# jonnylaw/ComposableStateSpaceModels

Measured on AMD Instinct MI355X. Metric: particle-steps/sec (N x T) bootstrap filter, higher is better.
Workload: dtype f64

## Files before the change

composablestatespacemodels_amd/csrc/cssm_device.hip.h:

```cpp
#pragma once

#if !defined(__HIPCC_RTC__)
#include <hip/hip_runtime.h>
#include <stdint.h>
#endif

#include "cssm_records.h"

#define CSSM_BLOCK 256
#ifndef CSSM_PROP_IT_MID
#define CSSM_PROP_IT_MID 2
#endif
#define CSSM_ITEMS 4
#define CSSM_TILE (CSSM_BLOCK * CSSM_ITEMS)

#define CSSM_MAXSLOTS 64
#define CSSM_SLOT_STRIDE 16
#define CSSM_MAXSETS 3
#define CSSM_GRP_UNITS 32
#define CSSM_GRP_MAX 64
#define CSSM_GRP_SMALL 32
#define CSSM_GRP_LIMB 56
#define CSSM_GRP_MAX_UNIT (1u << 15)
struct Scalars {
  unsigned long long maxslot[CSSM_MAXSETS * CSSM_MAXSLOTS * CSSM_SLOT_STRIDE];
  unsigned long long grp[CSSM_MAXSETS * 2 * CSSM_GRP_MAX * CSSM_SLOT_STRIDE];
  unsigned long long grp2[CSSM_MAXSETS * 2 * CSSM_GRP_MAX * CSSM_SLOT_STRIDE];
  uint32_t err;
  int32_t ess;
  uint32_t fail_step;
  uint32_t pad_;
  double gmax;
  double ref;
  double next_ref;
  double ll;
  cssm_u128 S_local, S2_local;
  cssm_u128 S_off;
  cssm_u128 S_tot, S2_tot;
  uint32_t pend, pend_buf, pend_n, pend_idx, pend_gen;
  uint32_t wait_code;
  cssm_u128 pend_S;
  unsigned long long peer_wait_ticks;
  unsigned long long t_first;
  unsigned long long t_last;
  unsigned long long hdr_wait_ticks, xhdr_wait_ticks, rows_wait_ticks, xwaits;
};

struct ChainBase {
  double* state[2]; double* logw; uint32_t* anc; cssm_u128* tileS; cssm_u128* tileS2; Scalars* sc; StepRec* recs;
  cssm_u128* s2buf; double* ll_t; int32_t* ess_t; double* path; const double* m0; const double* sd0;
  Scalars* host_sc; double* host_ll_t; int32_t* host_ess_t; uint32_t* host_done;
  uint64_t seed; uint32_t gen, done_seq;
};


#define CSSM_DPP_ROW_SHR(n) (0x110 + (n))
#define CSSM_DPP_BCAST15 0x142
#define CSSM_DPP_BCAST31 0x143
template <int CTRL, int ROW_MASK>
__device__ __forceinline__ uint32_t dpp0(uint32_t v) {
  return (uint32_t)__builtin_amdgcn_update_dpp(0, (int)v, CTRL, ROW_MASK, 0xf, false);
}
template <int CTRL, int ROW_MASK>
__device__ __forceinline__ uint64_t dpp0_u64(uint64_t v) {
  return (uint64_t)dpp0<CTRL, ROW_MASK>((uint32_t)v) | ((uint64_t)dpp0<CTRL, ROW_MASK>((uint32_t)(v >> 32)) << 32);
}
template <int CTRL, int ROW_MASK>
__device__ __forceinline__ cssm_u128 dpp0_u128(cssm_u128 v) {
  cssm_u128 r;
  r.lo = dpp0_u64<CTRL, ROW_MASK>(v.lo);
  r.hi = dpp0_u64<CTRL, ROW_MASK>(v.hi);
  return r;
}
__device__ __forceinline__ uint64_t readlane_u64(uint64_t v, int lane) {
  return (uint64_t)(uint32_t)__builtin_amdgcn_readlane((int)(uint32_t)v, lane) |
         ((uint64_t)(uint32_t)__builtin_amdgcn_readlane((int)(uint32_t)(v >> 32), lane) << 32);
}

#define CSSM_SCAN_STEP(CTRL)                                  \
  "v_add_co_u32_dpp %0, vcc, %0, %0 " CTRL "\n\t"              \
  "v_addc_co_u32_dpp %1, vcc, %1, %1, vcc " CTRL "\n\t"        \
  "v_addc_co_u32_dpp %2, vcc, %2, %2, vcc " CTRL "\n\t"        \
  "v_addc_co_u32_dpp %3, vcc, %3, %3, vcc " CTRL "\n\t"
__device__ __forceinline__ cssm_u128 wave_scan_u128(cssm_u128 v, int lane) {
  (void)lane;
  uint32_t a0 = (uint32_t)v.lo, a1 = (uint32_t)(v.lo >> 32), a2 = (uint32_t)v.hi, a3 = (uint32_t)(v.hi >> 32);
  asm volatile("s_nop 1\n\t"
               CSSM_SCAN_STEP("row_shr:1 row_mask:0xf bank_mask:0xf bound_ctrl:0")
               CSSM_SCAN_STEP("row_shr:2 row_mask:0xf bank_mask:0xf bound_ctrl:0")
               CSSM_SCAN_STEP("row_shr:4 row_mask:0xf bank_mask:0xf bound_ctrl:0")
               CSSM_SCAN_STEP("row_shr:8 row_mask:0xf bank_mask:0xf bound_ctrl:0")
               CSSM_SCAN_STEP("row_bcast:15 row_mask:0xa bank_mask:0xf")
               CSSM_SCAN_STEP("row_bcast:31 row_mask:0xc bank_mask:0xf")
               "s_nop 0"
               : "+v"(a0), "+v"(a1), "+v"(a2), "+v"(a3) : : "vcc");
  cssm_u128 r;
  r.lo = (uint64_t)a0 | ((uint64_t)a1 << 32);
  r.hi = (uint64_t)a2 | ((uint64_t)a3 << 32);
  return r;
}
__device__ __forceinline__ cssm_u128 wave_excl_add_u128(cssm_u128 inc, cssm_u128 off) {
  uint32_t a0 = (uint32_t)inc.lo, a1 = (uint32_t)(inc.lo >> 32), a2 = (uint32_t)inc.hi, a3 = (uint32_t)(inc.hi >> 32);
  const uint32_t b0 = (uint32_t)off.lo, b1 = (uint32_t)(off.lo >> 32), b2 = (uint32_t)off.hi, b3 = (uint32_t)(off.hi >> 32);
  uint32_t r0, r1, r2, r3;
  asm volatile("s_nop 1\n\t"
               "v_add_co_u32_dpp %0, vcc, %4, %8 wave_shr:1 row_mask:0xf bank_mask:0xf bound_ctrl:0\n\t"
               "v_addc_co_u32_dpp %1, vcc, %5, %9, vcc wave_shr:1 row_mask:0xf bank_mask:0xf bound_ctrl:0\n\t"
               "v_addc_co_u32_dpp %2, vcc, %6, %10, vcc wave_shr:1 row_mask:0xf bank_mask:0xf bound_ctrl:0\n\t"
               "v_addc_co_u32_dpp %3, vcc, %7, %11, vcc wave_shr:1 row_mask:0xf bank_mask:0xf bound_ctrl:0"
               : "=&v"(r0), "=&v"(r1), "=&v"(r2), "=&v"(r3)
               : "v"(a0), "v"(a1), "v"(a2), "v"(a3), "v"(b0), "v"(b1), "v"(b2), "v"(b3) : "vcc");
  cssm_u128 r;
  r.lo = (uint64_t)r0 | ((uint64_t)r1 << 32);
  r.hi = (uint64_t)r2 | ((uint64_t)r3 << 32);
  return r;
}
__device__ __forceinline__ unsigned long long ld_sys_u64(const unsigned long long* p) { return __hip_atomic_load(p, __ATOMIC_RELAXED, __HIP_MEMORY_SCOPE_SYSTEM); }
__device__ __forceinline__ double ld_sys_f64(const double* p) { return cssm_u2d(ld_sys_u64(reinterpret_cast<const unsigned long long*>(p))); }

__device__ __forceinline__ double uniform_f64(double x) {
  const uint64_t b = cssm_d2u(x);
  const uint32_t lo = (uint32_t)__builtin_amdgcn_readfirstlane((int)(uint32_t)b), hi = (uint32_t)__builtin_amdgcn_readfirstlane((int)(uint32_t)(b >> 32));
  return cssm_u2d((uint64_t)lo | ((uint64_t)hi << 32));
}
__device__ __forceinline__ cssm_u128 uniform_u128(cssm_u128 v) {
  cssm_u128 r;
  r.lo = (uint64_t)(uint32_t)__builtin_amdgcn_readfirstlane((int)(uint32_t)v.lo) | ((uint64_t)(uint32_t)__builtin_amdgcn_readfirstlane((int)(uint32_t)(v.lo >> 32)) << 32);
  r.hi = (uint64_t)(uint32_t)__builtin_amdgcn_readfirstlane((int)(uint32_t)v.hi) | ((uint64_t)(uint32_t)__builtin_amdgcn_readfirstlane((int)(uint32_t)(v.hi >> 32)) << 32);
  return r;
}
__device__ __forceinline__ double cssm_fract_pos(double x) { return __builtin_amdgcn_fract(x); }
__device__ __forceinline__ cssm_u128 wave_sum_u128(cssm_u128 v) {
  v = wave_scan_u128(v, 0);
  cssm_u128 r;
  r.lo = readlane_u64(v.lo, 63);
  r.hi = readlane_u64(v.hi, 63);
  return r;
}
__device__ __forceinline__ uint32_t wave_max_u32(uint32_t v) {
#define CSSM_MAX_STEP(CTRL, RM) { const uint32_t o = dpp0<CTRL, RM>(v); v = (o > v) ? o : v; }
  CSSM_MAX_STEP(CSSM_DPP_ROW_SHR(1), 0xf) CSSM_MAX_STEP(CSSM_DPP_ROW_SHR(2), 0xf) CSSM_MAX_STEP(CSSM_DPP_ROW_SHR(4), 0xf)
  CSSM_MAX_STEP(CSSM_DPP_ROW_SHR(8), 0xf) CSSM_MAX_STEP(CSSM_DPP_BCAST15, 0xa) CSSM_MAX_STEP(CSSM_DPP_BCAST31, 0xc)
#undef CSSM_MAX_STEP
  return (uint32_t)__builtin_amdgcn_readlane((int)v, 63);
}
__device__ __forceinline__ uint64_t wave_max_u64(uint64_t k) {
  const uint32_t hi = (uint32_t)(k >> 32);
  const uint32_t mh = wave_max_u32(hi);
  const uint32_t ml = wave_max_u32((hi == mh) ? (uint32_t)k : 0u);
  return ((uint64_t)mh << 32) | (uint64_t)ml;
}
__device__ __forceinline__ double wave_max(double v) { return cssm_order_unkey(wave_max_u64(cssm_order_key(v))); }

__device__ __forceinline__ const double* stage_log_table(const double* __restrict__ tab_global) {
  __shared__ double s_logtab[CSSM_TAB_SIZE];
  for (int i = threadIdx.x; i < CSSM_TAB_SIZE; i += blockDim.x) s_logtab[i] = tab_global[i];
  __syncthreads();
  return s_logtab;
}
__device__ __forceinline__ const double* stage_log_table_finish(double v, double v1, double v2) {
  static_assert(CSSM_TAB_SIZE == 3 * 256, "three table entries per thread of a 256-thread block");
  __shared__ double s_logtab2[CSSM_TAB_SIZE];
  s_logtab2[threadIdx.x] = v; s_logtab2[256 + threadIdx.x] = v1; s_logtab2[512 + threadIdx.x] = v2;
  __syncthreads();
  return s_logtab2;
}

template <int NP>
__device__ __forceinline__ void stream_normals(uint64_t seed, uint64_t stream, uint32_t step, uint32_t tag, uint32_t b0, const double* tab,
                                               double (&E)[2 * NP]) {
#pragma unroll
  for (int B = 0; B < (NP + 1) / 2; ++B) {
    const cssm_u32x4 blk = cssm_philox_draw(seed, stream, step, tag, b0 + (uint32_t)B);
    cssm_normal_pair64(blk.v[0], blk.v[1], tab, &E[(4 * B) % (2 * NP)], &E[(4 * B + 1) % (2 * NP)]);
    if (2 * B + 1 < NP) cssm_normal_pair64(blk.v[2], blk.v[3], tab, &E[(4 * B + 2) % (2 * NP)], &E[(4 * B + 3) % (2 * NP)]);
// ... 332 lines not shown
```

composablestatespacemodels_amd/csrc/cssm_host.h:

```cpp
#pragma once

#include <hip/hip_runtime.h>
#include <stdint.h>

#include "cssm_device.hip.h"

struct PropLaunch {
  int grid;
  hipStream_t stream;
  int lgcp;
  int obs;
  int sums;
  const double* src; size_t src_stride; const uint32_t* anc;
  double* dst; size_t dst_stride; double* logw; uint64_t n; uint64_t gid0; uint64_t seed;
  const StepRec* rec; ModelK mk; Scalars* sc; int slot_set;
  const double* src2; size_t src2_stride; uint32_t n_split; const double* logtab;
  uint64_t chunk; int do_sums; cssm_u128* subS; cssm_u128* subS2; double* pick_out; uint32_t pick_slot;
  const double* fsub;
  int sharded;
  int shard_slim;
  uint32_t step;
  int one;
  int specialise;
  const void* chains;
  int nchains;
  int cur, anc_valid, want_pick; uint32_t rec_idx;
  int obs_kind;
};

bool cssm_rtc_launch(const PropLaunch& a, int kind, int D, int IT, int onev);

#define CSSM_PROP_LAUNCHED_GRP 1
#define CSSM_PROP_LAUNCHED_WS 2
#define CSSM_DECL_PROP(D) int cssm_prop_launch_d##D(const PropLaunch& a);
CSSM_DECL_PROP(1) CSSM_DECL_PROP(2) CSSM_DECL_PROP(3) CSSM_DECL_PROP(4) CSSM_DECL_PROP(5) CSSM_DECL_PROP(6) CSSM_DECL_PROP(7) CSSM_DECL_PROP(8)
CSSM_DECL_PROP(9) CSSM_DECL_PROP(10) CSSM_DECL_PROP(11) CSSM_DECL_PROP(12) CSSM_DECL_PROP(13) CSSM_DECL_PROP(14) CSSM_DECL_PROP(15) CSSM_DECL_PROP(16)
#undef CSSM_DECL_PROP
```

composablestatespacemodels_amd/csrc/cssm_internal.h:

```cpp
#pragma once

#include <hip/hip_runtime.h>

#include <cstddef>
#include <cstring>
#include <string>
#include <vector>

#include "cssm_host.h"

#define fail cssm_fail
#define HIP_TRY(expr)                                                                         \
  do {                                                                                        \
    hipError_t e__ = (expr);                                                                  \
    if (e__ != hipSuccess) return fail(CSSM_EHIP, "%s: %s (%s:%d)", #expr, hipGetErrorString(e__), __FILE__, __LINE__); \
  } while (0)

#define CSSM_NKERNELS CSSM_PROFILE_NKERNELS


struct cssm_pf : HostModel {
  int device = 0;
  int n_cus = 256;
  hipStream_t stream = nullptr;
  bool own_stream = true;
  uint64_t first = 0, n = 0;
  size_t stride = 0;
  uint32_t ntiles = 0;
  uint32_t sup = 1, nunits = 0;
  uint32_t split = 1;
  bool safe_sums = false;
  bool last_optimistic = false;
  bool wmode = false;
  bool have_level = false;
  bool sums_ready = false;
  cssm_u128* s2buf = nullptr;
  uint32_t s2_stride = 0;
  int s2_par = 0;
  uint32_t gen = 0;
  int32_t ess_host = 0;
  void* last_comm = nullptr;
  std::vector<double> h_fsub;
  double* d_fsub = nullptr; size_t fsub_cap = 0;
  bool sharded = false;
  double* state[2] = {nullptr, nullptr};
  int cur = 0;
  const double* src = nullptr;
  size_t src_stride = 0;
  const double* src2 = nullptr;
  size_t src2_stride = 0;
  uint32_t n_split = 0;
  double* logw = nullptr;
  uint32_t* endslot = nullptr;
  uint32_t* anc = nullptr;
  bool anc_valid = false;
  int wparity = 0;
  int opt_exact = 0;
  int opt_fused = 0;
  cssm_u128 *fineS = nullptr, *fineS2 = nullptr;
  size_t fine_cap = 0;
  int opt_whole = 0;
  int opt_grp = 1;
  uint32_t grp_min_units = 2u * CSSM_GRP_UNITS;
  int opt_spec = 1;
  bool last_grp = false;
  int grp_layout = 0;
  bool last_ws = false;
  int opt_wave = 1;
  cssm_u128* tileW = nullptr;
  int resampler = CSSM_RESAMPLE_SYSTEMATIC;
  double* cum = nullptr;
  const long long *send_first_dev = nullptr, *send_count_dev = nullptr;
  cssm_u128 *tileS = nullptr, *tileS2 = nullptr, *tileP = nullptr;
  cssm_u128* unitPre = nullptr;
  bool spec_pre = false;
  Scalars* sc = nullptr;
  double *d_m0 = nullptr, *d_sd0 = nullptr, *d_logtab = nullptr;
  StepRec* d_recs = nullptr;
  size_t recs_cap = 0;
  double* d_ll_t = nullptr;
  int32_t* d_ess_t = nullptr;
  double* h_ll_t = nullptr; double* hd_ll_t = nullptr;
  int32_t* h_ess_t = nullptr; int32_t* hd_ess_t = nullptr;
  Scalars* hd_sc = nullptr;
  double* d_path = nullptr;
  size_t path_cap = 0;
  double* cand = nullptr;
  size_t cand_cap = 0;
  uint32_t *cand_end = nullptr, *cand_idx = nullptr;
  size_t cidx_cap = 0;
  int64_t* d_bounds = nullptr;
  int64_t* d_xch = nullptr;
  uint32_t* d_need = nullptr;
  size_t need_cap = 0;
  bool series = false;
  unsigned long long* sm_keys = nullptr; double* sm_partial = nullptr; void* sm_st = nullptr; StepRec* sm_rec = nullptr;
  size_t sm_cap = 0; int sm_blocks = 0; double sm_time = 0.0;
  void* peer = nullptr; void* peer_tab = nullptr; unsigned int* peer_tickets = nullptr;
  unsigned long long peer_wait_ticks = 3000000000ull;
  uint32_t peer_seq = 0;
  uint32_t peer_probe_plain_bad = 0;
  bool peer_packed = false;
  bool peer_rows_packed = false;
  bool peer_all_rows = false;
  long long peer_eager = 4096;
  bool want_path = false;
  uint32_t rec_base = 0;
  struct Snap { int cur; const double* src; size_t src_stride; const double* src2; size_t src2_stride; uint32_t n_split; bool anc_valid, last_optimistic; uint32_t step; double t; bool have_level;
                int wparity; bool last_grp; };
  std::vector<Snap> snaps;
  std::vector<Snap> pre_snaps;
  StepRec* h_recs = nullptr;
  StepRec* h_recs_dev = nullptr;
  size_t h_recs_cap = 0;
  Scalars* h_sc = nullptr;
  double t = 0.0;
  uint32_t step = 0;
  uint32_t h_step_for_resample = 0;
  bool initialised = false;
  hipEvent_t ev0 = nullptr, ev1 = nullptr;
  float last_ms = -1.f;
  int opt_events = 0;
  bool have_events = false;
  bool profile = false;
  uint32_t* h_done = nullptr; uint32_t* hd_done = nullptr; uint32_t done_seq = 0;
  std::vector<hipEvent_t> prof_ev;
  std::vector<int> prof_kind;
  size_t prof_used = 0;
  double prof_ms[CSSM_NKERNELS] = {0};
  uint64_t prof_cnt[CSSM_NKERNELS] = {0};
  int obs_has_scale = 0;
  double obs_scale = 0.0;
  size_t forecast_cap = 0;
  double forecast_ms[2] = {-1.0, -1.0};
};

static inline void prof_begin(cssm_pf* pf, int kind) {
  if (!pf->profile) return;
  if (pf->prof_used * 2 + 2 > pf->prof_ev.size()) {
    hipEvent_t a, b;
    if (hipEventCreate(&a) != hipSuccess || hipEventCreate(&b) != hipSuccess) { pf->profile = false; return; }
    pf->prof_ev.push_back(a); pf->prof_ev.push_back(b);
  }
  if (pf->prof_kind.size() <= pf->prof_used) pf->prof_kind.resize(pf->prof_used + 1);
  pf->prof_kind[pf->prof_used] = kind;
  (void)hipEventRecord(pf->prof_ev[pf->prof_used * 2], pf->stream);
}
static inline void prof_end(cssm_pf* pf) {
  if (!pf->profile) return;
  (void)hipEventRecord(pf->prof_ev[pf->prof_used * 2 + 1], pf->stream);
  pf->prof_used++;
}
static inline void prof_collect(cssm_pf* pf) {
  for (size_t i = 0; i < pf->prof_used; ++i) {
    float ms = 0.f;
    if (hipEventElapsedTime(&ms, pf->prof_ev[2 * i], pf->prof_ev[2 * i + 1]) == hipSuccess) {
      pf->prof_ms[pf->prof_kind[i]] += ms;
      pf->prof_cnt[pf->prof_kind[i]]++;
    }
  }
  pf->prof_used = 0;
}

static inline int grid_for(uint64_t n, int block, int cap) {
  uint64_t g = (n + block - 1) / block;
  if (g > (uint64_t)cap) g = cap;
  if (g < 1) g = 1;
  return (int)g;
}

#define CSSM_SC_TAIL_OFF offsetof(Scalars, err)
#define CSSM_SC_TAIL_ARGS(hp, scp) reinterpret_cast<char*>(hp) + CSSM_SC_TAIL_OFF, reinterpret_cast<const char*>(scp) + CSSM_SC_TAIL_OFF, sizeof(Scalars) - CSSM_SC_TAIL_OFF

static const int kGridCap = 4096;

#define DISPATCH_D(d, ...)                                                         \
  switch (d) {                                                                      \
    case 1: { constexpr int D = 1; __VA_ARGS__; } break;   case 2: { constexpr int D = 2; __VA_ARGS__; } break;   \
    case 3: { constexpr int D = 3; __VA_ARGS__; } break;   case 4: { constexpr int D = 4; __VA_ARGS__; } break;   \
    case 5: { constexpr int D = 5; __VA_ARGS__; } break;   case 6: { constexpr int D = 6; __VA_ARGS__; } break;   \
    case 7: { constexpr int D = 7; __VA_ARGS__; } break;   case 8: { constexpr int D = 8; __VA_ARGS__; } break;   \
    case 9: { constexpr int D = 9; __VA_ARGS__; } break;   case 10: { constexpr int D = 10; __VA_ARGS__; } break; \
    case 11: { constexpr int D = 11; __VA_ARGS__; } break; case 12: { constexpr int D = 12; __VA_ARGS__; } break; \
    case 13: { constexpr int D = 13; __VA_ARGS__; } break; case 14: { constexpr int D = 14; __VA_ARGS__; } break; \
    case 15: { constexpr int D = 15; __VA_ARGS__; } break; default: { constexpr int D = 16; __VA_ARGS__; } break; \
  }

int cssm_build_fsub(cssm_pf* pf, size_t first, size_t count, bool reset);
int cssm_ensure_recs(cssm_pf* pf, size_t T);
int cssm_upload_recs(cssm_pf* pf, size_t first, size_t count, bool chain);
int cssm_launch_init(cssm_pf* pf, double t0);
struct CssmBatchLaunch { const void* chains; int nchains; uint32_t rec_idx; int want_pick; };
int cssm_launch_propagate(cssm_pf* pf, const StepRec* d_rec, double* pick_out = nullptr, uint32_t pick_slot = 0, const CssmBatchLaunch* batch = nullptr);
int cssm_pf_create_on_stream(const cssm_model_desc* desc, uint64_t n_particles, uint64_t seed, int device, hipStream_t stream, cssm_pf** out);
void cssm_batch_fresh(cssm_pf* pf, double t0);
int cssm_batch_ok(const cssm_pf* pf);
int cssm_check_device_err(cssm_pf* pf, const Scalars& h);
int cssm_prop_items(int d);
double cssm_eta_of_mean(const cssm_pf* pf, const StepRec& rec, const double* mean);
void cssm_peer_free(cssm_pf* pf);
```

composablestatespacemodels_amd/csrc/cssm_offspring.hip.h:

```cpp
#pragma once

#include "cssm_device.hip.h"


#define CSSM_RUN_DIRECT 8

#ifndef CSSM_OFF_WAVES
#define CSSM_OFF_WAVES 4
#endif
#ifndef CSSM_OFF_UPRE
#define CSSM_OFF_UPRE 4
#endif
#ifndef CSSM_OFF_SC1
#define CSSM_OFF_SC1 1
#endif
__device__ __forceinline__ cssm_u128 block_sum_u128(cssm_u128 v, cssm_u128* s_red) {
  v = wave_sum_u128(v);
  __syncthreads();
  if ((threadIdx.x & 63) == 0) s_red[threadIdx.x >> 6] = v;
  __syncthreads();
  cssm_u128 t = s_red[0];
#pragma unroll
  for (int w = 1; w < CSSM_BLOCK / 64; ++w) t = cssm_u128_add(t, s_red[w]);
  return t;
}

#ifndef CSSM_OFF_SELF_WAVES
#define CSSM_OFF_SELF_WAVES 5
#endif
__device__ __forceinline__ void offspring_exact_counts(cssm_u128 run0, const double (&w)[4], uint32_t mask, double totd, double u, uint64_t n_global,
                                                       uint32_t (&e)[4], bool host_weights = false) {
  const bool pow2 = (n_global & (n_global - 1)) == 0;
  const double inv_n = 1.0 / (double)n_global;
  cssm_u128 run = run0;
#pragma unroll 1
  for (int k = 0; k < 4; ++k) {
    const double wk = (k == 0) ? w[0] : ((k == 1) ? w[1] : ((k == 2) ? w[2] : w[3]));
    run = cssm_u128_add(run, host_weights ? cssm_fix_from_double(wk) : cssm_fix_from_unit(wk));
    if ((mask >> k) & 1u) {
      const double C = cssm_u128_to_double(run) / totd;
      const uint32_t c = (uint32_t)(pow2 ? cssm_sys_count_pow2(C, u, n_global, inv_n) : cssm_sys_count(C, u, n_global));
      e[0] = (k == 0) ? c : e[0]; e[1] = (k == 1) ? c : e[1]; e[2] = (k == 2) ? c : e[2]; e[3] = (k == 3) ? c : e[3];
    }
  }
}

#ifdef CSSM_OFF_STAMPS
#define CSSM_STAMP(k) do { if (SELF && threadIdx.x == 0 && cum_out) reinterpret_cast<unsigned long long*>(cum_out)[(size_t)(is_pub ? gridDim.x - 1u : ublk) * 8 + (k)] = __builtin_amdgcn_s_memrealtime(); } while (0)
#else
#define CSSM_STAMP(k) do { } while (0)
#endif
template <bool SELF> struct TotExact {
  const cssm_u128* waves; double totd;
  __device__ __forceinline__ double operator()() const {
    if (!SELF) return totd;
    cssm_u128 t = waves[0];
#pragma unroll
    for (int w = 1; w < CSSM_BLOCK / 64; ++w) t = cssm_u128_add(t, waves[w]);
    return cssm_u128_to_double(t);
  }
};
template <bool SELF, int RS>
__device__ __forceinline__ void tile_end_slots(cssm_u128 run, const double (&w1)[CSSM_ITEMS], const int raw,
                                               const double u, const uint64_t n_global, const bool pow2, const int force_exact, const TotExact<SELF> totd_exact,
                                               const uint64_t seed, const uint32_t rec_step, const uint64_t base, const uint64_t n,
                                               double* __restrict__ cum_out, uint32_t (&e)[CSSM_ITEMS],
                                               const double scale, const double eps, const double one_minus_eps, const double one_minus_u) {
  constexpr int resampler = RS;
  auto fixw = [&](double w) { return (raw == 1) ? cssm_fix_from_double(w) : cssm_fix_from_unit(w); };
  constexpr bool OUTLINED = RS == CSSM_RESAMPLE_SYSTEMATIC && CSSM_ITEMS == 4;
  uint32_t unsafe = 0u;
  const cssm_u128 run0 = run;
  double sd = cssm_fma((double)run.hi, 0x1.0p64, (double)run.lo);
#pragma unroll
  for (int r = 0; r < CSSM_ITEMS; ++r) {
    if (raw == 1) {
      run = cssm_u128_add(run, fixw(w1[r]));
      sd = cssm_fma((double)run.hi, 0x1.0p64, (double)run.lo);
    } else {
      sd = cssm_fma(w1[r], 0x1.0p96, sd);
    }
    const double pp1 = cssm_fma(sd, scale, one_minus_u);
    const double fr = cssm_fract_pos(pp1);
    const bool safe = (fr > eps) && (fr < one_minus_eps) && (OUTLINED || !force_exact) && resampler == CSSM_RESAMPLE_SYSTEMATIC;
    if (safe) {
      const uint32_t c32 = (uint32_t)pp1;
      e[r] = (c32 > (uint32_t)n_global) ? (uint32_t)n_global : c32;
    } else if constexpr (OUTLINED) {
      e[r] = 0u;
      unsafe |= 1u << r;
    } else {
      if (raw != 1) {
        run = run0;
#pragma unroll
        for (int k = 0; k < CSSM_ITEMS; ++k) if (k <= r) run = cssm_u128_add(run, fixw(w1[k]));
      }
      const double C = cssm_u128_to_double(run) / totd_exact();
      if (resampler == CSSM_RESAMPLE_SYSTEMATIC) {
        e[r] = (uint32_t)(pow2 ? cssm_sys_count_pow2(C, u, n_global, 1.0 / (double)n_global) : cssm_sys_count(C, u, n_global));
      } else if (resampler == CSSM_RESAMPLE_STRATIFIED) {
        e[r] = (uint32_t)cssm_strat_count(C, seed, rec_step, n_global);
      } else {
        const uint64_t ii = base + (uint64_t)threadIdx.x * CSSM_ITEMS + r;
        if (ii < n) cum_out[ii] = C;
        e[r] = 0;
      }
    }
  }
  if constexpr (OUTLINED) {
    if (force_exact) {
      uint32_t fm = 0xfu;
      if (force_exact == 2) {
        const uint32_t j0 = (uint32_t)base + threadIdx.x * CSSM_ITEMS;
        fm = ((j0 % 3u == 0u) ? 1u : 0u) | (((j0 + 1u) % 3u == 0u) ? 2u : 0u) | (((j0 + 2u) % 3u == 0u) ? 4u : 0u) | (((j0 + 3u) % 3u == 0u) ? 8u : 0u);
      }
      unsafe |= fm;
    }
    if (unsafe) offspring_exact_counts(run0, w1, unsafe, totd_exact(), u, n_global, e, raw == 1);
  }
}

template <bool SELF, int RS>
__device__ __forceinline__ uint32_t end_slot_of_prefix(const cssm_u128 toff, const double scale, const double eps, const double one_minus_eps,
                                                       const double one_minus_u, const double u, const uint64_t n_global, const bool pow2,
                                                       const int force_exact, const TotExact<SELF> totd_exact, const uint64_t seed, const uint32_t rec_step) {
  constexpr int resampler = RS;
  constexpr bool OUTLINED = RS == CSSM_RESAMPLE_SYSTEMATIC && CSSM_ITEMS == 4;
  const double sdp = cssm_fma((double)toff.hi, 0x1.0p64, (double)toff.lo);
  const double ppp = cssm_fma(sdp, scale, one_minus_u);
  const double frp = cssm_fract_pos(ppp);
  if ((frp > eps) && (frp < one_minus_eps) && !force_exact && resampler == CSSM_RESAMPLE_SYSTEMATIC) {
    const uint32_t c32 = (uint32_t)ppp;
    return (c32 > (uint32_t)n_global) ? (uint32_t)n_global : c32;
  } else if constexpr (OUTLINED) {
    const double z4[4] = {0.0, 0.0, 0.0, 0.0};
    uint32_t p4[4] = {0u, 0u, 0u, 0u};
    offspring_exact_counts(toff, z4, 1u, totd_exact(), u, n_global, p4);
    return p4[0];
  } else {
    const double Cp = cssm_u128_to_double(toff) / totd_exact();
    return (resampler == CSSM_RESAMPLE_STRATIFIED)
               ? (uint32_t)cssm_strat_count(Cp, seed, rec_step, n_global)
               : (uint32_t)(pow2 ? cssm_sys_count_pow2(Cp, u, n_global, 1.0 / (double)n_global) : cssm_sys_count(Cp, u, n_global));
  }
}

__device__ __forceinline__ void publish_observation(Scalars* __restrict__ sc, const StepRec* __restrict__ rec, const double gmax_dec, const double gmax,
                                                    const cssm_u128 tot, const cssm_u128 tot2, const bool p_pend, const cssm_u128 ptot2,
                                                    const int s2_par, const uint32_t nunits, const uint32_t rec_idx, const uint32_t gen,
                                                    double* __restrict__ ll_t, int32_t* __restrict__ ess_t, const uint64_t n_global, const int slot_set) {
  if (threadIdx.x == 0) {
    if (p_pend) {
      const int32_t pe = cssm_ess_of(sc->pend_S, ptot2);
      sc->ess = pe;
      if (ess_t && sc->pend_gen == gen) ess_t[sc->pend_idx] = pe;
    }
    sc->gmax = gmax_dec; sc->ref = gmax; sc->S_off = cssm_u128_zero(); sc->S_local = tot; sc->S_tot = tot;
    publish_next_level(sc, rec, gmax_dec);
    if (s2_par < 0) {
      sc->S2_local = tot2; sc->S2_tot = tot2; sc->pend = 0u;
      finish_step(sc, n_global);
      if (ll_t) { ll_t[rec_idx] = sc->ll; ess_t[rec_idx] = sc->ess; }
    } else {
      sc->pend = 1u; sc->pend_buf = (uint32_t)s2_par; sc->pend_n = nunits; sc->pend_idx = rec_idx; sc->pend_gen = gen;
      sc->pend_S = tot;
      (void)finish_ll(sc, n_global);
      if (ll_t) ll_t[rec_idx] = sc->ll;
    }
  }
  if (threadIdx.x < 2 * 2 * CSSM_GRP_MAX) {
    const uint32_t tq2 = threadIdx.x;
    sc->grp[((size_t)((slot_set + 1 + (int)(tq2 / (2 * CSSM_GRP_MAX))) % CSSM_MAXSETS) * 2 * CSSM_GRP_MAX + tq2 % (2 * CSSM_GRP_MAX)) * CSSM_SLOT_STRIDE] = 0ull;
  }
  if (threadIdx.x < 2 * CSSM_MAXSLOTS)
    sc->maxslot[((size_t)((slot_set + 1 + (int)(threadIdx.x / CSSM_MAXSLOTS)) % CSSM_MAXSETS) * CSSM_MAXSLOTS + threadIdx.x % CSSM_MAXSLOTS) * CSSM_SLOT_STRIDE] = 0ull;
}

struct SpecTotals { cssm_u128 S_off, tot, tot2; double gmax; };
struct NoMid { __device__ __forceinline__ bool operator()(SpecTotals&) const { return true; } };
template <bool FUSE, bool SELF, int RS, int RAWC = -1, int GRPL = 0, class Mid = NoMid>
__device__ __forceinline__ void offspring_body(const double* __restrict__ logw, uint64_t n,
                                                          Scalars* __restrict__ sc,
                                                          const cssm_u128* __restrict__ unitP, const cssm_u128* __restrict__ unitS2,
                                                          const StepRec* __restrict__ rec, uint64_t n_global,
                                                          uint32_t* __restrict__ endslot, uint32_t* __restrict__ anc,
                                                          uint32_t ntiles, uint32_t sup, uint32_t nunits, int raw_arg, int slot_set,
                                                          double* __restrict__ ll_t, int32_t* __restrict__ ess_t, uint32_t rec_idx,
                                                          int force_exact, const unsigned long long* __restrict__ all5, int rank, int world,
                                                          int split, uint64_t seed, double* __restrict__ cum_out,
                                                          const double* __restrict__ logtab, int optimistic,
                                                          unsigned long long* __restrict__ flag_out,
                                                          uint32_t slot_lo, uint32_t slot_hi, uint32_t all5_stride,
                                                          cssm_u128* __restrict__ s2buf = nullptr, uint32_t s2_stride = 0, int s2_par_arg = -1,
                                                          uint32_t gen = 0, const cssm_u128* __restrict__ unit_pre = nullptr, const uint32_t blk0 = 0u,
                                                          const double* pre_in = nullptr, const SpecTotals* tt = nullptr, Mid* mid = nullptr) {
  const uint32_t bidx = blockIdx.x - blk0, nblk = gridDim.x - blk0;
  constexpr bool GRP = GRPL != 0;
  constexpr bool BIG = GRPL == 2;
  static_assert(!BIG || SELF, "layout 2: the single-GPU launch");
  constexpr bool grp_on = GRP;
  constexpr bool EARLY = GRP && RAWC == 2;
  static_assert(!GRP || RAWC == 2 || (SELF && RAWC == 0), "group sums: a launch behind a fused-sums propagate (the single GPU's, or a shard's exchange kernel)");
  constexpr bool SHARD_GRP = GRP && !SELF;
  const int raw = (RAWC >= 0) ? RAWC : raw_arg;
  const int s2_par = (RAWC == 0) ? -1 : s2_par_arg;
  constexpr int resampler = RS;
  const double* tab = nullptr; (void)logtab;
  __shared__ cssm_u128 s_w[CSSM_BLOCK / 64];
  __shared__ __attribute__((aligned(16))) uint32_t s_slot[FUSE ? (CSSM_BLOCK / 64) * CSSM_WAVE_CHUNK : 4];
  __shared__ cssm_u128 s_r[3][CSSM_BLOCK / 64];
  __shared__ cssm_u128 s_pre[2];
  __shared__ double s_scale;
  constexpr bool PUB_FIRST = SELF && RS == CSSM_RESAMPLE_SYSTEMATIC && RAWC == 2;
  const uint32_t ublk = PUB_FIRST ? bidx - 1u : bidx;
  const bool is_pub = SELF && (PUB_FIRST ? bidx == 0u : bidx == nunits);
  CSSM_STAMP(0);
  const uint32_t held = SELF ? sc->err : 0u;
  double pre_v[CSSM_ITEMS];
  if (pre_in != nullptr) {
#pragma unroll
    for (int r = 0; r < CSSM_ITEMS; ++r) pre_v[r] = pre_in[r];
  } else if (ublk < nunits) load_tile_raw(logw, (uint64_t)ublk * sup * CSSM_TILE, n, raw, pre_v);
  constexpr int UPRE = CSSM_OFF_UPRE;
  cssm_u128 upre[UPRE];
  const uint32_t nsub = SELF ? nunits * (uint32_t)split : 0u;
  const uint32_t E = (nsub + CSSM_BLOCK - 1) / CSSM_BLOCK;
  const uint32_t wsum = (bidx + 1u) & 3u;
  const uint32_t wsum2 = (bidx + 2u) & 3u;
  const uint32_t grp_unit = is_pub ? 0u : ublk;
  if (grp_on && BIG) {
#pragma unroll
    for (int k = 0; k < UPRE; ++k) upre[k] = cssm_u128_zero();
    const uint32_t l = threadIdx.x & 63u;
    if ((threadIdx.x >> 6) == wsum) {
      const unsigned long long* g = &sc->grp[((size_t)slot_set * 2 * CSSM_GRP_MAX + l) * CSSM_SLOT_STRIDE];
      upre[0].lo = g[0]; upre[0].hi = g[(size_t)CSSM_GRP_MAX * CSSM_SLOT_STRIDE];
    } else if ((threadIdx.x >> 6) == wsum2) {
      const uint32_t q = (grp_unit / 64u) * 64u + l;
      if (q < nunits) upre[0] = unitP[q];
    }
  } else if (grp_on) {
#pragma unroll
    for (int k = 0; k < UPRE; ++k) upre[k] = cssm_u128_zero();
    if ((threadIdx.x >> 6) == wsum) {
      const uint32_t l = threadIdx.x & 63u;
      if (l < (uint32_t)CSSM_GRP_SMALL) {
        const unsigned long long* g = &sc->grp[((size_t)slot_set * 2 * CSSM_GRP_MAX + l) * CSSM_SLOT_STRIDE];
        upre[0].lo = g[0]; upre[0].hi = g[(size_t)CSSM_GRP_MAX * CSSM_SLOT_STRIDE];
      } else {
        const uint32_t q = (grp_unit / CSSM_GRP_UNITS) * CSSM_GRP_UNITS + (l - (uint32_t)CSSM_GRP_SMALL);
        if (q < nunits) {
          upre[0] = unitP[(size_t)q * (uint32_t)split];
          if (!SELF) for (uint32_t sb = 1; sb < (uint32_t)split; ++sb) upre[0] = cssm_u128_add(upre[0], unitP[(size_t)q * (uint32_t)split + sb]);
        }
      }
    }
  } else if (SELF) {
    if (nsub == UPRE * CSSM_BLOCK) {
#pragma unroll
      for (int k = 0; k < UPRE; ++k) upre[k] = unitP[threadIdx.x * UPRE + (uint32_t)k];
    } else {
#pragma unroll
      for (int k = 0; k < UPRE; ++k) {
        const uint32_t q = threadIdx.x * E + (uint32_t)k;
        upre[k] = ((uint32_t)k < E && q < nsub) ? unitP[q] : cssm_u128_zero();
      }
    }
  }
  const double rec_ref = rec->ref, u = rec->u;
  const uint32_t rec_step = rec->step;
  __shared__ unsigned long long s_key;
  double gmax_dec = 0.0, gmax = 0.0;
  auto level_known = [&]() -> bool {
    gmax = (raw == 1) ? gmax_dec : cssm_ref_choose(rec_ref, gmax_dec);
    if (raw != 1 && optimistic && !(gmax == rec_ref)) {
      if (SELF) {
        if (bidx == 0 && threadIdx.x == 0) { sc->gmax = gmax_dec; atomicMin(&sc->fail_step, rec_step); atomicOr(&sc->err, 64u); }
      } else if (bidx == 0 && threadIdx.x == 0) {
        if (flag_out) *flag_out = 1ull;
        if (optimistic == 2) { atomicMin(&sc->fail_step, rec_step); atomicOr(&sc->err, 4u); }
      }
      return false;
    }
    return true;
  };
  if (SELF) {
    if ((threadIdx.x >> 6) == (bidx & (CSSM_BLOCK / 64 - 1))) {
      const uint32_t l = threadIdx.x & 63u;
      unsigned long long k = (l < CSSM_MAXSLOTS) ? sc->maxslot[((size_t)slot_set * CSSM_MAXSLOTS + l) * CSSM_SLOT_STRIDE] : 0ull;
      k = wave_max_u64(k);
      if (l == 0u) s_key = k;
    }
    if (held & 64u) return;
  } else if (!SHARD_GRP) {
    if (tt != nullptr) {
      gmax_dec = tt->gmax;
    } else if (all5) {
      unsigned long long key = 0ull;
      for (int r = 0; r < world; ++r) { const unsigned long long k = ld_sys_u64(all5 + (size_t)all5_stride * r + 4); key = (k > key) ? k : key; }
      gmax_dec = cssm_order_unkey(key);
    } else {
      gmax_dec = sc->gmax;
    }
    if (!level_known()) return;
  }
  if (!SELF && !SHARD_GRP && flag_out && bidx == 0 && threadIdx.x == 0) *flag_out = 0ull;
  const bool pow2 = (n_global & (n_global - 1)) == 0;
  const int lane = threadIdx.x & 63, wid = threadIdx.x >> 6;
  double totd = 0.0;
  cssm_u128 S_off = cssm_u128_zero();
  auto shard_totals = [&](const SpecTotals* t) {
    cssm_u128 tot = cssm_u128_zero(), tot2 = cssm_u128_zero();
    if (t != nullptr) {
      S_off = t->S_off; tot = t->tot; tot2 = t->tot2;
    } else
    for (int r = 0; r < world; ++r) {
      cssm_u128 a, b;
      const unsigned long long* w5 = all5 + (size_t)all5_stride * r;
      a.lo = ld_sys_u64(w5); a.hi = ld_sys_u64(w5 + 1); b.lo = ld_sys_u64(w5 + 2); b.hi = ld_sys_u64(w5 + 3);
      if (r < rank) S_off = cssm_u128_add(S_off, a);
      tot = cssm_u128_add(tot, a); tot2 = cssm_u128_add(tot2, b);
    }
    totd = cssm_u128_to_double(tot);
    if (bidx == 0 && threadIdx.x == 0) {
      sc->gmax = gmax_dec; sc->ref = gmax;
      sc->S_off = S_off; sc->S_tot = tot; sc->S2_tot = tot2;
      finish_step(sc, n_global);
      publish_next_level(sc, rec, gmax_dec);
    }
  };
  if (!SELF && !SHARD_GRP) {
    if (all5) {
      shard_totals(tt);
    } else {
      totd = cssm_u128_to_double(sc->S_tot);
      S_off = sc->S_off;
    }
  }
  uint32_t unit = ublk;
  cssm_u128 toff_self = cssm_u128_zero();
  double scale_self = 0.0;
  cssm_u128 acc2 = cssm_u128_zero();
  auto fixw = [&](double w) { return (raw == 1) ? cssm_fix_from_double(w) : cssm_fix_from_unit(w); };
  auto tile_front = [&](uint32_t tile, bool first, double (&w1)[CSSM_ITEMS], bool s2_now) __attribute__((always_inline)) -> cssm_u128 {
    if (first) weights_from_raw(pre_v, gmax, raw, w1, tab);
    else load_tile_weights(logw, (uint64_t)tile * CSSM_TILE, n, gmax, raw, w1, tab);
    cssm_u128 tsum = cssm_u128_zero();
#pragma unroll
    for (int r = 0; r < CSSM_ITEMS; ++r) {
      tsum = cssm_u128_add(tsum, fixw(w1[r]));
      if (SELF && s2_par >= 0) acc2 = cssm_u128_add(acc2, cssm_fix_from_unit(w1[r] * w1[r]));
    }
    const cssm_u128 inc = wave_scan_u128(tsum, lane);
    if (lane == 63) s_w[wid] = inc;
    CSSM_STAMP(2);
    if (s2_now) {
      const cssm_u128 w2 = wave_scan_u128(acc2, lane);
      if (lane == 63) s_r[2][wid] = w2;
    }
    return inc;
  };
  double w1_first[CSSM_ITEMS];
  cssm_u128 inc_first = cssm_u128_zero();
  if (SELF || SHARD_GRP) {
    const uint32_t qlim = (is_pub ? 0u : unit) * (uint32_t)split;
    const uint32_t Ed = E ? E : 1u;
    const uint32_t tq = ((Ed & (Ed - 1u)) == 0u) ? (qlim >> (31 - __builtin_clz(Ed))) : qlim / Ed, rq = qlim - tq * Ed;
    auto scan_units = [&](cssm_u128& tot, cssm_u128& pre) {
      if (grp_on && BIG) {
        if (wid == wsum) {
          cssm_u128 x, y;
          x.lo = upre[0].lo; x.hi = 0ull;
          y.lo = upre[0].hi << CSSM_GRP_LIMB; y.hi = upre[0].hi >> (64 - CSSM_GRP_LIMB);
          const cssm_u128 inc = wave_scan_u128(cssm_u128_add(x, y), lane);
          const uint32_t G = grp_unit / 64u;
          cssm_u128 t, pg = cssm_u128_zero();
          t.lo = readlane_u64(inc.lo, 63); t.hi = readlane_u64(inc.hi, 63);
          if (G > 0u) { pg.lo = readlane_u64(inc.lo, (int)G - 1); pg.hi = readlane_u64(inc.hi, (int)G - 1); }
          if (lane == 0u) {
            s_r[1][0] = t;
#pragma unroll
            for (int w = 1; w < CSSM_BLOCK / 64; ++w) s_r[1][w] = cssm_u128_zero();
            s_pre[0] = pg;
            const double tf = cssm_fma((double)t.hi, 0x1.0p64, (double)t.lo);
            double rinv = __builtin_amdgcn_rcp(tf);
            rinv = cssm_fma(cssm_fma(-tf, rinv, 1.0), rinv, rinv);
            rinv = cssm_fma(cssm_fma(-tf, rinv, 1.0), rinv, rinv);
            s_scale = (double)n_global * rinv;
          }
        } else if (wid == wsum2) {
          const cssm_u128 inc = wave_scan_u128(upre[0], lane);
          const uint32_t r = grp_unit % 64u;
          cssm_u128 pu = cssm_u128_zero();
          if (r > 0u) { pu.lo = readlane_u64(inc.lo, (int)r - 1); pu.hi = readlane_u64(inc.hi, (int)r - 1); }
          if (lane == 0u) s_pre[1] = pu;
        }
        __syncthreads();
        tot.lo = s_r[1][0].lo; tot.hi = s_r[1][0].hi;
        { cssm_u128 p0, p1; p0.lo = s_pre[0].lo; p0.hi = s_pre[0].hi; p1.lo = s_pre[1].lo; p1.hi = s_pre[1].hi; pre = cssm_u128_add(p0, p1); }
        return;
      }
      if (grp_on) {
        static_assert(CSSM_GRP_SMALL == 32 && CSSM_GRP_UNITS == 32, "one wave holds the groups and one group's units");
        if (wid == wsum) {
          cssm_u128 v = upre[0];
          if (lane < 32u) {
            cssm_u128 x, y;
            x.lo = upre[0].lo; x.hi = 0ull;
            y.lo = upre[0].hi << CSSM_GRP_LIMB; y.hi = upre[0].hi >> (64 - CSSM_GRP_LIMB);
            v = cssm_u128_add(x, y);
          }
          const cssm_u128 inc = wave_scan_u128(v, lane);
          const uint32_t G = grp_unit / CSSM_GRP_UNITS, r = grp_unit % CSSM_GRP_UNITS;
          cssm_u128 t, pg = cssm_u128_zero(), pu = cssm_u128_zero();
          t.lo = readlane_u64(inc.lo, 31); t.hi = readlane_u64(inc.hi, 31);
          if (G > 0u) { pg.lo = readlane_u64(inc.lo, (int)G - 1); pg.hi = readlane_u64(inc.hi, (int)G - 1); }
          if (r > 0u) {
            cssm_u128 e; e.lo = readlane_u64(inc.lo, 31 + (int)r); e.hi = readlane_u64(inc.hi, 31 + (int)r);
            pu.lo = e.lo - t.lo; pu.hi = e.hi - t.hi - (e.lo < t.lo ? 1ull : 0ull);
          }
          if (lane == 0u) {
            s_r[1][0] = t;
#pragma unroll
            for (int w = 1; w < CSSM_BLOCK / 64; ++w) s_r[1][w] = cssm_u128_zero();
            s_pre[0] = cssm_u128_add(pg, pu);
            if (SELF) {
              const double tf = cssm_fma((double)t.hi, 0x1.0p64, (double)t.lo);
              double rinv = __builtin_amdgcn_rcp(tf);
              rinv = cssm_fma(cssm_fma(-tf, rinv, 1.0), rinv, rinv);
              rinv = cssm_fma(cssm_fma(-tf, rinv, 1.0), rinv, rinv);
              s_scale = (double)n_global * rinv;
            }
          }
        }
        __syncthreads();
        tot.lo = s_r[1][0].lo; tot.hi = s_r[1][0].hi;
        pre.lo = s_pre[0].lo; pre.hi = s_pre[0].hi;
        return;
      }
      cssm_u128 own = cssm_u128_zero(), part = cssm_u128_zero();
#pragma unroll
      for (int k = 0; k < UPRE; ++k) {
        if ((uint32_t)k == rq && rq < (uint32_t)UPRE) part = own;
        own = cssm_u128_add(own, upre[k]);
      }
      if (rq == (uint32_t)UPRE) part = own;
      for (uint32_t k = UPRE; k < E; ++k) {
        const uint32_t q = threadIdx.x * E + k;
        if (q < nsub) own = cssm_u128_add(own, unitP[q]);
        if (k + 1u == rq) part = own;
      }
      const cssm_u128 inc = wave_scan_u128(own, lane);
      if (lane == 63) s_r[1][wid] = inc;
      if (threadIdx.x + 1u == tq) s_pre[0] = inc;
      if (threadIdx.x == tq) s_pre[1] = part;
      __syncthreads();
      tot = s_r[1][0];
#pragma unroll
      for (int w = 1; w < CSSM_BLOCK / 64; ++w) tot = cssm_u128_add(tot, s_r[1][w]);
      pre = (rq > 0u) ? s_pre[1] : cssm_u128_zero();
      if (tq > 0u) {
        pre = cssm_u128_add(pre, s_pre[0]);
        const uint32_t wq = (tq - 1u) >> 6;
#pragma unroll
        for (int w = 0; w < CSSM_BLOCK / 64 - 1; ++w) if ((uint32_t)w < wq) pre = cssm_u128_add(pre, s_r[1][w]);
      }
    };
    if (is_pub) {
      cssm_u128 tot2 = cssm_u128_zero(), pt2 = cssm_u128_zero();
      const uint32_t hint_buf = (s2_par >= 0) ? (uint32_t)(s2_par ^ 1) : 0u;
      {
        const cssm_u128* hb = s2buf + (size_t)hint_buf * s2_stride;
        for (uint32_t q = threadIdx.x; q < nunits; q += CSSM_BLOCK) pt2 = cssm_u128_add(pt2, hb[q]);
      }
      if (s2_par < 0) {
        cssm_u128 t2 = cssm_u128_zero();
        for (uint32_t q = threadIdx.x; q < nsub; q += CSSM_BLOCK) t2 = cssm_u128_add(t2, unitS2[q]);
        tot2 = block_sum_u128(t2, s_r[2]);
      }
      const uint32_t p_pend = sc->pend, p_buf = sc->pend_buf, p_n = sc->pend_n;
      if (p_pend && (p_buf != hint_buf || p_n != nunits)) {
        pt2 = cssm_u128_zero();
        const cssm_u128* pb = s2buf + (size_t)p_buf * s2_stride;
        for (uint32_t q = threadIdx.x; q < p_n; q += CSSM_BLOCK) pt2 = cssm_u128_add(pt2, pb[q]);
      }
      cssm_u128 tot, pre_unused;
      scan_units(tot, pre_unused);
      CSSM_STAMP(1);
      gmax_dec = cssm_order_unkey(s_key);
      if (!level_known()) return;
      cssm_u128 ptot2 = cssm_u128_zero();
      if (p_pend) ptot2 = block_sum_u128(pt2, s_r[2]);
      publish_observation(sc, rec, gmax_dec, gmax, tot, tot2, p_pend != 0u, ptot2, s2_par, nunits, rec_idx, gen, ll_t, ess_t, n_global, slot_set);
      CSSM_STAMP(7);
      return;
    }
    if constexpr (EARLY) {
      const uint32_t t0h = ublk * sup;
      inc_first = tile_front(t0h, true, w1_first, SELF && s2_par >= 0 && t0h + 1u == ((t0h + sup < ntiles) ? t0h + sup : ntiles));
    }
    cssm_u128 tot;
    scan_units(tot, toff_self);
    CSSM_STAMP(1);
    if constexpr (SHARD_GRP) {
      SpecTotals t2;
      if (!(*mid)(t2)) return;
      gmax_dec = t2.gmax; gmax = rec_ref;
      shard_totals(&t2);
    } else {
    gmax_dec = cssm_order_unkey(s_key);
    if (!level_known()) return;
    if constexpr (GRP) {
      scale_self = uniform_f64(s_scale);
    } else {
      const double tf = cssm_fma((double)tot.hi, 0x1.0p64, (double)tot.lo);
      double rinv = __builtin_amdgcn_rcp(tf);
      rinv = cssm_fma(cssm_fma(-tf, rinv, 1.0), rinv, rinv);
      rinv = cssm_fma(cssm_fma(-tf, rinv, 1.0), rinv, rinv);
      scale_self = uniform_f64((double)n_global * rinv);
    }
    }
  }
  if (unit < nunits) do {
    const uint32_t t0 = unit * sup;
    const uint32_t t1 = (t0 + sup < ntiles) ? t0 + sup : ntiles;
    cssm_u128 toff;
    if constexpr (SHARD_GRP) {
      toff = cssm_u128_add(S_off, toff_self);
    } else
    if (!SELF && all5 && unit_pre != nullptr) {
      cssm_u128 up; const unsigned long long* upw = reinterpret_cast<const unsigned long long*>(unit_pre + (size_t)unit * split);
      up.lo = ld_sys_u64(upw); up.hi = ld_sys_u64(upw + 1);
      toff = cssm_u128_add(S_off, up);
    } else if (!SELF && all5) {
      cssm_u128 pre = cssm_u128_zero();
      const uint32_t qlim = unit * (uint32_t)split;
      for (uint32_t q = threadIdx.x; q < qlim; q += CSSM_BLOCK) pre = cssm_u128_add(pre, unitP[q]);
      pre = block_sum_u128(pre, s_r[0]);
      toff = cssm_u128_add(S_off, pre);
      __syncthreads();
    } else if (SELF) {
      toff = uniform_u128(toff_self);
    } else {
      toff = cssm_u128_add(S_off, unitP[(size_t)unit * split]);
    }
    for (uint32_t tile = t0; tile < t1; ++tile) {
      const uint64_t base = (uint64_t)tile * CSSM_TILE;
      double w1[CSSM_ITEMS];
      cssm_u128 inc;
      const bool s2_now = SELF && s2_par >= 0 && tile + 1 == t1;
      if constexpr (EARLY) {
        if (tile == t0) {
#pragma unroll
          for (int r = 0; r < CSSM_ITEMS; ++r) w1[r] = w1_first[r];
          inc = inc_first;
        } else {
          inc = tile_front(tile, false, w1, s2_now);
          __syncthreads();
        }
      } else {
        if (unit == ublk && tile == t0) weights_from_raw(pre_v, gmax, raw, w1, tab);
        else load_tile_weights(logw, base, n, gmax, raw, w1, tab);
        cssm_u128 tsum = cssm_u128_zero();
#pragma unroll
        for (int r = 0; r < CSSM_ITEMS; ++r) {
          tsum = cssm_u128_add(tsum, fixw(w1[r]));
          if (SELF && s2_par >= 0) acc2 = cssm_u128_add(acc2, cssm_fix_from_unit(w1[r] * w1[r]));
        }
        inc = wave_scan_u128(tsum, lane);
        if (lane == 63) s_w[wid] = inc;
        CSSM_STAMP(2);
        if (s2_now) {
          const cssm_u128 w2 = wave_scan_u128(acc2, lane);
          if (lane == 63) s_r[2][wid] = w2;
        }
        __syncthreads();
      }
      if (s2_now && threadIdx.x == 0) {
        cssm_u128 b2 = s_r[2][0];
#pragma unroll
        for (int w = 1; w < CSSM_BLOCK / 64; ++w) b2 = cssm_u128_add(b2, s_r[2][w]);
        s2buf[(size_t)s2_par * s2_stride + ublk] = b2;
      }
      CSSM_STAMP(3);
      cssm_u128 off = toff;
      for (int w = 0; w < wid; ++w) off = cssm_u128_add(off, s_w[w]);
      cssm_u128 run = wave_excl_add_u128(inc, off);
      const double nd = (double)n_global;
      const double scale = SELF ? scale_self : nd / totd;
      const double eps = SELF ? uniform_f64(nd * 0x1.0p-44) : nd * 0x1.0p-44;
      const double one_minus_eps = SELF ? uniform_f64(1.0 - eps) : 1.0 - eps;
      const double one_minus_u = 1.0 - u;
      uint32_t e[CSSM_ITEMS];
      tile_end_slots<SELF, RS>(run, w1, raw, u, n_global, pow2, force_exact, TotExact<SELF>{s_r[1], totd}, seed, rec_step, base, n, cum_out, e,
                               scale, eps, one_minus_eps, one_minus_u);
      const uint64_t i0 = base + (uint64_t)threadIdx.x * CSSM_ITEMS;
      constexpr bool CLIP = !SELF;
      if ((!FUSE || (CLIP && all5 != nullptr)) && endslot != nullptr) {
        if (i0 + CSSM_ITEMS <= n) {
          *reinterpret_cast<uint4*>(endslot + i0) = make_uint4(e[0], e[1], e[2], e[3]);
        } else {
#pragma unroll
          for (int r = 0; r < CSSM_ITEMS; ++r) if (i0 + r < n) endslot[i0 + r] = e[r];
        }
      }
      CSSM_STAMP(4);
      if (FUSE && resampler != CSSM_RESAMPLE_MULTINOMIAL) {
        uint32_t prev = dpp0<0x138 , 0xf>(e[CSSM_ITEMS - 1]);
        if (lane == 0) {
          if (tile == 0 && wid == 0 && (SELF || all5 == nullptr || rank == 0)) prev = 0u;
          else prev = end_slot_of_prefix<SELF, RS>(off, scale, eps, one_minus_eps, one_minus_u, u, n_global, pow2, force_exact, TotExact<SELF>{s_r[1], totd}, seed, rec_step);
        }
        uint32_t wb = (uint32_t)__builtin_amdgcn_readfirstlane((int)prev);
        uint32_t we = (uint32_t)__builtin_amdgcn_readlane((int)e[CSSM_ITEMS - 1], 63);
        if (CLIP) { wb = (wb < slot_lo) ? slot_lo : wb; we = (we > slot_hi) ? slot_hi : we; }
        we = (we > (uint32_t)n_global) ? (uint32_t)n_global : we;
        wb = (wb > we) ? we : wb;
        fill_runs_wave<CSSM_OFF_SC1 != 0, CLIP>(prev, e, (uint32_t)i0, wb, we, anc, CLIP ? slot_lo : 0u, (uint32_t)(n - 1),
                                                s_slot + wid * CSSM_WAVE_CHUNK);
      }
      CSSM_STAMP(5);
      if (!SELF || tile + 1 < t1) {
        cssm_u128 ttot = s_w[0];
#pragma unroll
        for (int w = 1; w < CSSM_BLOCK / 64; ++w) ttot = cssm_u128_add(ttot, s_w[w]);
        toff = SELF ? uniform_u128(cssm_u128_add(toff, ttot)) : cssm_u128_add(toff, ttot);
        __syncthreads();
      }
    }
  } while (!SELF && !SHARD_GRP && (unit += nblk) < nunits);
}

#define CSSM_OFFSPRING_PARAMS                                                                                              \
  const double* __restrict__ logw, uint64_t n, Scalars* __restrict__ sc, const cssm_u128* __restrict__ unitP,              \
  const cssm_u128* __restrict__ unitS2, const StepRec* __restrict__ rec, uint64_t n_global, uint32_t* __restrict__ endslot, \
  uint32_t* __restrict__ anc, uint32_t ntiles, uint32_t sup, uint32_t nunits, int raw, int slot_set,                        \
  double* __restrict__ ll_t, int32_t* __restrict__ ess_t, uint32_t rec_idx, int force_exact,                                \
  const unsigned long long* __restrict__ all5, int rank, int world, int split, uint64_t seed, double* __restrict__ cum_out, \
  const double* __restrict__ logtab, int optimistic, unsigned long long* __restrict__ flag_out, uint32_t slot_lo, uint32_t slot_hi
#define CSSM_OFFSPRING_FWD                                                                                                   \
  logw, n, sc, unitP, unitS2, rec, n_global, endslot, anc, ntiles, sup, nunits, raw, slot_set, ll_t, ess_t, rec_idx,       \
  force_exact, all5, rank, world, split, seed, cum_out, logtab, optimistic, flag_out, slot_lo, slot_hi

template <bool FUSE, bool SELF, int RS>
__global__ __launch_bounds__(CSSM_BLOCK, CSSM_OFF_WAVES) void k_offspring(CSSM_OFFSPRING_PARAMS, uint32_t all5_stride = 5) {
  offspring_body<FUSE, SELF, RS>(CSSM_OFFSPRING_FWD, all5_stride);
}

template <int RS, int RAWC, int GRP = 0>
__global__ __attribute__((amdgpu_flat_work_group_size(CSSM_BLOCK, CSSM_BLOCK),
                          amdgpu_waves_per_eu((RS == CSSM_RESAMPLE_SYSTEMATIC && RAWC == 2) ? CSSM_OFF_SELF_WAVES : CSSM_OFF_WAVES, 8))) void k_offspring_self(
    const double* __restrict__ logw, uint64_t n, Scalars* __restrict__ sc, const cssm_u128* __restrict__ unitP,
    const cssm_u128* __restrict__ unitS2, const StepRec* __restrict__ rec, uint32_t* __restrict__ anc, uint32_t ntiles, uint32_t sup,
    uint32_t nunits, int slot_set, double* __restrict__ ll_t, int32_t* __restrict__ ess_t, uint32_t rec_idx, int force_exact, int split,
    uint64_t seed, double* __restrict__ cum_out, cssm_u128* __restrict__ s2buf, uint32_t s2_stride, int s2_par, uint32_t gen) {
  offspring_body<true, true, RS, RAWC, GRP>(logw, n, sc, unitP, unitS2, rec, n, nullptr, anc, ntiles, sup, nunits, RAWC, slot_set, ll_t, ess_t, rec_idx,
                                            force_exact, nullptr, 0, 1, split, seed, cum_out, nullptr, RAWC == 2 ? 1 : 0, nullptr, 0u, (uint32_t)n, 5u,
                                            s2buf, s2_stride, s2_par, gen);
}
```

composablestatespacemodels_amd/csrc/cssm_pf.hip:

```cpp
#include <hip/hip_runtime.h>

#include <algorithm>
#include <chrono>
#include <cmath>
#include <cstdio>
#include <cstdlib>

#include "cssm_internal.h"
#include "cssm_kernels.hip.h"
#include "cssm_offspring_wave.hip.h"

static int upload_init_params(cssm_pf* pf) {
  double m0[CSSM_MAX_DIM], sd0[CSSM_MAX_DIM];
  for (int k = 0; k < pf->d; ++k) { m0[k] = pf->comp[k].m0; sd0[k] = std::sqrt(pf->comp[k].c0); }
  HIP_TRY(hipMemcpyAsync(pf->d_m0, m0, pf->d * 8, hipMemcpyHostToDevice, pf->stream));
  HIP_TRY(hipMemcpyAsync(pf->d_sd0, sd0, pf->d * 8, hipMemcpyHostToDevice, pf->stream));
  HIP_TRY(hipStreamSynchronize(pf->stream));
  return CSSM_OK;
}

int cssm_build_fsub(cssm_pf* pf, size_t first, size_t count, bool reset) {
  if (!pf->lgcp_tdep) return CSSM_OK;
  if (reset) pf->h_fsub.clear();
  int rc = cssm_build_fsub_table(pf, pf->h_recs, first, count, pf->h_fsub);
  if (rc) return rc;
  if (pf->h_fsub.empty()) return CSSM_OK;
  if (pf->fsub_cap < pf->h_fsub.size()) {
    HIP_TRY(hipStreamSynchronize(pf->stream));
    if (pf->d_fsub) (void)hipFree(pf->d_fsub);
    pf->d_fsub = nullptr; pf->fsub_cap = 0;
    const size_t cap = pf->h_fsub.size() + pf->h_fsub.size() / 2 + 1024;
    HIP_TRY(hipMalloc(&pf->d_fsub, cap * 8));
    pf->fsub_cap = cap;
  }
  HIP_TRY(hipStreamSynchronize(pf->stream));
  HIP_TRY(hipMemcpy(pf->d_fsub, pf->h_fsub.data(), pf->h_fsub.size() * 8, hipMemcpyHostToDevice));
  return CSSM_OK;
}


#ifndef CSSM_PROP_IT_LO
#define CSSM_PROP_IT_LO 2
#endif
#ifndef CSSM_SPLIT_MAX_N
#define CSSM_SPLIT_MAX_N (1u << 20)
#endif
int cssm_prop_items(int d) { return d <= 2 ? CSSM_PROP_IT_LO : (d <= 8 ? CSSM_PROP_IT_MID : 1); }

static uint32_t auto_split(const cssm_pf* pf) {
  if (pf->sharded) {
    if (pf->obs_kind != CSSM_OBS_LGCP || pf->sup < 2) return 1u;
    uint32_t want = 2u;
    if (const char* e = getenv("CSSM_SHARD_LGCP_SPLIT")) { const int v = atoi(e); if (v == 1 || v == 2 || v == 4) want = (uint32_t)v; }
    while (want > 1u && ((uint64_t)pf->sup * CSSM_TILE / want) % (uint64_t)CSSM_TILE != 0) want >>= 1;
    const uint64_t unit_particles = (uint64_t)pf->sup * CSSM_TILE;
    if (!(pf->opt_grp && pf->nunits >= pf->grp_min_units && pf->nunits <= (uint32_t)(CSSM_GRP_SMALL * CSSM_GRP_UNITS) && unit_particles <= CSSM_GRP_MAX_UNIT)) want = 1u;
    return want;
  }
  if (pf->sup != 1 || pf->n >= CSSM_SPLIT_MAX_N) return 1u;
  return cssm_prop_items(pf->d) == 1 ? 4u : 2u;
}

static int alloc_handle(cssm_pf* pf) {
  HIP_TRY(hipSetDevice(pf->device));
  if (pf->own_stream) HIP_TRY(hipStreamCreateWithFlags(&pf->stream, hipStreamNonBlocking));
  HIP_TRY(hipEventCreate(&pf->ev0));
  HIP_TRY(hipEventCreate(&pf->ev1));
  { const char* e = getenv("CSSM_LOOP_EVENTS"); pf->opt_events = (e && e[0] == '1') ? 1 : 0; }
  { const char* e = getenv("CSSM_PEER_TIMEOUT_MS"); if (e && atof(e) > 0.0) pf->peer_wait_ticks = (unsigned long long)(atof(e) * 1e5); }
  { const char* e = getenv("CSSM_PEER_ALL_ROWS"); pf->peer_all_rows = e && e[0] == '1'; }
  { const char* e = getenv("CSSM_PEER_EAGER_ROWS"); if (e && atoll(e) >= 1) pf->peer_eager = atoll(e); }
  { const char* e = getenv("CSSM_WAVE_SUMS"); if (e) pf->opt_wave = atoi(e) == 2 ? 2 : (atoi(e) ? 1 : 0); }
  { const char* e = getenv("CSSM_GRP_MIN_UNITS"); if (e && atoi(e) >= 1) pf->grp_min_units = (uint32_t)atoi(e); }
  HIP_TRY(hipDeviceGetAttribute(&pf->n_cus, hipDeviceAttributeMultiprocessorCount, pf->device));
  pf->stride = (size_t)((pf->n + CSSM_TILE - 1) / CSSM_TILE) * CSSM_TILE;
  pf->ntiles = (uint32_t)((pf->n + CSSM_TILE - 1) / CSSM_TILE);
  pf->sup = (pf->ntiles + 1023u) / 1024u;
  if (!pf->sharded && pf->sup > 4u) {
    uint32_t want = 4u;
    if (const char* e = getenv("CSSM_UNIT_MAX_TILES")) want = (uint32_t)atoi(e);
    if (want >= 1u) {
      const uint32_t least = (pf->ntiles + (uint32_t)(CSSM_GRP_MAX * 64) - 1u) / (uint32_t)(CSSM_GRP_MAX * 64);
      const uint32_t sup2 = want > least ? want : least;
      if (sup2 < pf->sup) pf->sup = sup2;
    }
  }
  pf->nunits = (pf->ntiles + pf->sup - 1) / pf->sup;
  {
    pf->split = auto_split(pf);
  }
  const size_t nsums = (size_t)(pf->ntiles > 4 * pf->nunits ? pf->ntiles : 4 * pf->nunits);
  const size_t row = pf->stride * 8;
  for (int b = 0; b < 2; ++b) {
    if (hipMalloc(&pf->state[b], row * pf->d + 64) != hipSuccess)
      return fail(CSSM_ENOMEM, "hipMalloc of %zu bytes failed", row * pf->d);
    HIP_TRY(hipMemsetAsync(pf->state[b], 0, row * pf->d, pf->stream));
  }
  if (hipMalloc(&pf->logw, row) != hipSuccess) return fail(CSSM_ENOMEM, "hipMalloc logw");
  if (hipMalloc(&pf->endslot, pf->stride * 4) != hipSuccess) return fail(CSSM_ENOMEM, "hipMalloc endslot");
  if (hipMalloc(&pf->anc, pf->stride * 4) != hipSuccess) return fail(CSSM_ENOMEM, "hipMalloc anc");
  HIP_TRY(hipMalloc(&pf->tileS, nsums * sizeof(cssm_u128)));
  HIP_TRY(hipMalloc(&pf->tileS2, nsums * sizeof(cssm_u128)));
  HIP_TRY(hipMalloc(&pf->tileP, nsums * sizeof(cssm_u128)));
  HIP_TRY(hipMalloc(&pf->unitPre, nsums * sizeof(cssm_u128)));
  HIP_TRY(hipMalloc(&pf->tileW, nsums * sizeof(cssm_u128)));
  HIP_TRY(hipMemsetAsync(pf->tileW, 0, nsums * sizeof(cssm_u128), pf->stream));
  pf->s2_stride = (uint32_t)nsums;
  HIP_TRY(hipMalloc(&pf->s2buf, 2 * nsums * sizeof(cssm_u128)));
  HIP_TRY(hipMemsetAsync(pf->s2buf, 0, 2 * nsums * sizeof(cssm_u128), pf->stream));
  HIP_TRY(hipHostMalloc((void**)&pf->h_sc, sizeof(Scalars), hipHostMallocMapped));
  memset(pf->h_sc, 0, sizeof(Scalars));
  HIP_TRY(hipHostGetDevicePointer((void**)&pf->hd_sc, pf->h_sc, 0));
  HIP_TRY(hipHostMalloc((void**)&pf->h_done, 64, hipHostMallocMapped));
  memset(pf->h_done, 0, 64);
  HIP_TRY(hipHostGetDevicePointer((void**)&pf->hd_done, pf->h_done, 0));
  HIP_TRY(hipMemsetAsync(pf->tileS, 0, nsums * sizeof(cssm_u128), pf->stream));
  HIP_TRY(hipMemsetAsync(pf->tileS2, 0, nsums * sizeof(cssm_u128), pf->stream));
  HIP_TRY(hipMemsetAsync(pf->tileP, 0, nsums * sizeof(cssm_u128), pf->stream));
  HIP_TRY(hipMalloc(&pf->sc, sizeof(Scalars)));
  HIP_TRY(hipMemsetAsync(pf->sc, 0, sizeof(Scalars), pf->stream));
  HIP_TRY(hipMalloc(&pf->d_m0, CSSM_MAX_DIM * 8));
  HIP_TRY(hipMalloc(&pf->d_sd0, CSSM_MAX_DIM * 8));
  HIP_TRY(hipMalloc(&pf->d_bounds, 64 * 8));
  HIP_TRY(hipMalloc(&pf->d_xch, 136 * 8));
  HIP_TRY(hipMemsetAsync(pf->d_xch, 0, 136 * 8, pf->stream));
  HIP_TRY(hipMemsetAsync(pf->anc, 0, pf->stride * 4, pf->stream));
  HIP_TRY(hipMalloc(&pf->d_logtab, sizeof(CSSM_TAB)));
  HIP_TRY(hipMemcpyAsync(pf->d_logtab, CSSM_TAB, sizeof(CSSM_TAB), hipMemcpyHostToDevice, pf->stream));
  return upload_init_params(pf);
}

static int create_common(const cssm_model_desc* desc, uint64_t n_global, uint64_t first, uint64_t n_local,
                         uint64_t seed, int device, void* stream, bool sharded, cssm_pf** out) {
  if (!out) return fail(CSSM_EINVAL_ARG, "out is null");
  *out = nullptr;
  if (n_global < 1 || n_global > 0xffff0000ull) return fail(CSSM_EINVAL_ARG, "n_particles must be in [1, 2^32 - 2^16]");
  if (n_local < 1 || first + n_local > n_global) return fail(CSSM_ESHARD, "shard [%llu, +%llu) outside [0, %llu)",
                                                              (unsigned long long)first, (unsigned long long)n_local, (unsigned long long)n_global);
  int ndev = 0;
  if (hipGetDeviceCount(&ndev) != hipSuccess || ndev < 1) return fail(CSSM_EHIP, "no HIP device available (this library has no CPU path)");
  if (device < 0 || device >= ndev) return fail(CSSM_EINVAL_ARG, "device %d out of range (%d devices)", device, ndev);
  cssm_pf* pf = new cssm_pf();
  pf->device = device;
  pf->n_global = n_global; pf->first = first; pf->n = n_local; pf->seed = seed; pf->sharded = sharded;
  if (sharded || stream != nullptr) { pf->stream = (hipStream_t)stream; pf->own_stream = false; }
  pf->opt_fused = 1;
  int rc = cssm_build_model(pf, desc, false);
  if (rc == CSSM_OK) { pf->obs_has_scale = desc->leaves[0].has_scale; pf->obs_scale = desc->leaves[0].scale; }
  if (rc == CSSM_OK) rc = alloc_handle(pf);
  if (rc != CSSM_OK) { const std::string keep = cssm_last_error(); cssm_pf_destroy(pf); return fail(rc, "%s", keep.c_str()); }
  *out = pf;
  return CSSM_OK;
}

int cssm_pf_create_on_stream(const cssm_model_desc* desc, uint64_t n_particles, uint64_t seed, int device, hipStream_t stream, cssm_pf** out) {
  return create_common(desc, n_particles, 0, n_particles, seed, device, stream, false, out);
}

extern "C" int cssm_pf_create(const cssm_model_desc* desc, uint64_t n_particles, uint64_t seed, int device, cssm_pf** out) {
  return create_common(desc, n_particles, 0, n_particles, seed, device, nullptr, false, out);
}

extern "C" int cssm_pf_create_shard(const cssm_model_desc* desc, uint64_t n_global, uint64_t first, uint64_t n_local,
                                    uint64_t seed, int device, void* hip_stream, cssm_pf** out) {
  return create_common(desc, n_global, first, n_local, seed, device, hip_stream, true, out);
}

extern "C" void cssm_pf_destroy(cssm_pf* pf) {
  if (!pf) return;
  (void)hipSetDevice(pf->device);
  if (pf->stream) (void)hipStreamSynchronize(pf->stream);
  cssm_peer_free(pf);
  void* ptrs[] = {pf->sm_keys, pf->sm_partial, pf->sm_st, pf->sm_rec, pf->s2buf, pf->fineS, pf->fineS2, pf->state[0], pf->state[1], pf->logw, pf->endslot, pf->anc, pf->tileS, pf->tileS2, pf->tileP, pf->unitPre, pf->tileW, pf->sc,
                  pf->d_m0, pf->d_sd0, pf->d_logtab, pf->d_fsub, pf->cum, pf->d_recs, pf->d_ll_t, pf->d_ess_t, pf->d_path, pf->cand, pf->cand_end, pf->cand_idx, pf->d_bounds, pf->d_xch, pf->d_need};
  for (void* p : ptrs) if (p) (void)hipFree(p);
  if (pf->h_recs) (void)hipHostFree(pf->h_recs);
  if (pf->h_sc) (void)hipHostFree(pf->h_sc);
  if (pf->h_done) (void)hipHostFree(pf->h_done);
  if (pf->h_ll_t) (void)hipHostFree(pf->h_ll_t);
  if (pf->h_ess_t) (void)hipHostFree(pf->h_ess_t);
  for (hipEvent_t e : pf->prof_ev) (void)hipEventDestroy(e);
  if (pf->ev0) (void)hipEventDestroy(pf->ev0);
  if (pf->ev1) (void)hipEventDestroy(pf->ev1);
  if (pf->own_stream && pf->stream) (void)hipStreamDestroy(pf->stream);
  delete pf;
}

extern "C" int cssm_pf_set_params(cssm_pf* pf, const cssm_model_desc* desc) {
  if (!pf) return fail(CSSM_EINVAL_ARG, "null handle");
  HIP_TRY(hipSetDevice(pf->device));
  int rc = cssm_build_model(pf, desc, true);
  if (rc) return rc;
  pf->obs_has_scale = desc->leaves[0].has_scale; pf->obs_scale = desc->leaves[0].scale;
  return upload_init_params(pf);
}

extern "C" int cssm_pf_reseed(cssm_pf* pf, uint64_t seed) {
  if (!pf) return fail(CSSM_EINVAL_ARG, "null handle");
  pf->seed = seed;
  return CSSM_OK;
}

extern "C" uint64_t cssm_pf_run_key(uint64_t seed, uint64_t run) { return cssm_derive_key(seed, run); }

extern "C" uint64_t cssm_pf_num_particles(const cssm_pf* pf) { return pf ? pf->n : 0; }
extern "C" int32_t cssm_pf_dim(const cssm_pf* pf) { return pf ? pf->d : 0; }

static int reset_scalars(cssm_pf* pf) {
  Scalars h;
  memset(&h, 0, sizeof h);
  h.ess = (int32_t)(pf->n_global < 2147483647ull ? pf->n_global : 2147483647ull);
  h.fail_step = 0xffffffffu;
  h.next_ref = cssm_nan();
  h.peer_wait_ticks = pf->peer_wait_ticks;
  HIP_TRY(hipMemsetAsync(pf->sc, 0, offsetof(Scalars, err), pf->stream));
  HIP_TRY(hipMemcpyAsync(reinterpret_cast<char*>(pf->sc) + CSSM_SC_TAIL_OFF, reinterpret_cast<const char*>(&h) + CSSM_SC_TAIL_OFF, sizeof(Scalars) - CSSM_SC_TAIL_OFF,
                         hipMemcpyHostToDevice, pf->stream));
  return CSSM_OK;
}

static void fresh_host_state(cssm_pf* pf, double t0) {
  pf->cur = 0; pf->src = pf->state[0]; pf->src_stride = pf->stride; pf->src2 = nullptr; pf->anc_valid = false;
  pf->t = t0; pf->step = 0; pf->initialised = true; pf->wparity = 0;
  pf->wmode = false; pf->sums_ready = false; pf->last_optimistic = false; pf->last_grp = false; pf->have_level = false;
  pf->ess_host = (int32_t)(pf->n_global < 2147483647ull ? pf->n_global : 2147483647ull);
}

int cssm_launch_init(cssm_pf* pf, double t0) {
  HIP_TRY(hipSetDevice(pf->device));
  const int grid = grid_for(pf->n, CSSM_BLOCK, kGridCap);
  DISPATCH_D(pf->d, k_init<D><<<dim3(grid), dim3(CSSM_BLOCK), 0, pf->stream>>>(pf->state[0], pf->stride, pf->n, pf->first,
                                                                              pf->seed, pf->d_m0, pf->d_sd0, pf->d_logtab));
  HIP_TRY(hipGetLastError());
  int rc = reset_scalars(pf);
  if (rc) return rc;
  fresh_host_state(pf, t0);
  return CSSM_OK;
}


static bool uses_sums_kernel(const cssm_pf* pf) {
  return pf->opt_fused && !pf->safe_sums && (pf->obs_kind != CSSM_OBS_LGCP || pf->have_level) && pf->resampler != CSSM_RESAMPLE_MULTINOMIAL;
}
static bool may_use_sums_kernel(const cssm_pf* pf) {
  return pf->opt_fused && !pf->safe_sums && pf->resampler != CSSM_RESAMPLE_MULTINOMIAL;
}

__global__ __launch_bounds__(128) void k_fetch_recs(const StepRec* __restrict__ host, StepRec* __restrict__ dev, Scalars* __restrict__ sc) {
  static_assert(sizeof(StepRec) % 8 == 0, "records are copied in 8-byte words");
  if (sc != nullptr && blockIdx.x == 0 && threadIdx.x == 0) sc->t_first = __builtin_amdgcn_s_memrealtime();
  const unsigned long long* s = reinterpret_cast<const unsigned long long*>(host + blockIdx.x);
  unsigned long long* d = reinterpret_cast<unsigned long long*>(dev + blockIdx.x);
  for (uint32_t i = threadIdx.x; i < sizeof(StepRec) / 8; i += 128) d[i] = s[i];
}
__global__ __launch_bounds__(128) void k_put_rec(StepRec r, StepRec* __restrict__ dev, Scalars* __restrict__ sc) {
  static_assert(offsetof(StepRec, step) < sizeof(StepRec), "");
  if (sc != nullptr && threadIdx.x == 0) sc->t_first = __builtin_amdgcn_s_memrealtime();
  const unsigned long long* s = (const unsigned long long*)__builtin_amdgcn_kernarg_segment_ptr();
  unsigned long long* d = reinterpret_cast<unsigned long long*>(dev);
  if (threadIdx.x < sizeof(StepRec) / 8) d[threadIdx.x] = s[threadIdx.x];
  (void)r;
}
int cssm_upload_recs(cssm_pf* pf, size_t first, size_t count, bool chain) {
  Scalars* stamp = first == 0 ? pf->sc : nullptr;
  static const bool by_copy = getenv("CSSM_UPLOAD_MEMCPY") != nullptr;
  static const bool no_kernarg = getenv("CSSM_UPLOAD_NO_KERNARG") != nullptr;
  if (count == 0) return CSSM_OK;
  if (count == 1 && !by_copy && !no_kernarg) {
    static_assert(sizeof(StepRec) / 8 <= 128 && sizeof(StepRec) <= 3072, "one record fits a kernel's argument segment and one block copies it");
    hipLaunchKernelGGL(k_put_rec, dim3(1), dim3(128), 0, pf->stream, pf->h_recs[first], pf->d_recs + first, stamp);
    HIP_TRY(hipGetLastError());
  } else if (by_copy || !pf->h_recs_dev || count > 0x7fffffffu) {
    if (stamp) HIP_TRY(hipMemsetAsync(&stamp->t_first, 0, sizeof(stamp->t_first), pf->stream));
    HIP_TRY(hipMemcpyAsync(pf->d_recs + first, pf->h_recs + first, count * sizeof(StepRec), hipMemcpyHostToDevice, pf->stream));
  } else {
    hipLaunchKernelGGL(k_fetch_recs, dim3((uint32_t)count), dim3(128), 0, pf->stream, (const StepRec*)(pf->h_recs_dev + first), pf->d_recs + first, stamp);
    HIP_TRY(hipGetLastError());
  }
  if (chain && pf->obs_kind == CSSM_OBS_LGCP) {
    hipLaunchKernelGGL(k_chain_level, dim3(1), dim3(1), 0, pf->stream, pf->d_recs + first, (const Scalars*)pf->sc);
    HIP_TRY(hipGetLastError());
  }
  return CSSM_OK;
}

#ifndef CSSM_FINE_MIN_D
#define CSSM_FINE_MIN_D 4
#endif
#ifndef CSSM_LOOP_MAX_TILES
#define CSSM_LOOP_MAX_TILES 8
#endif
enum { GEO_PIPE = 0, GEO_LOOP = 1, GEO_FINE = 2 };
static int large_geometry(const cssm_pf* pf) {
  if (pf->sharded || pf->split != 1 || pf->first != 0 || pf->n != pf->n_global || pf->resampler == CSSM_RESAMPLE_MULTINOMIAL) return GEO_PIPE;
  if (pf->opt_whole == 1) return GEO_LOOP;
  if (pf->opt_whole == 2) return GEO_PIPE;
  if (pf->opt_whole == 3) return GEO_FINE;
  const uint32_t tiles = pf->sup * (uint32_t)CSSM_TILE / (uint32_t)(CSSM_BLOCK * cssm_prop_items(pf->d));
  if (tiles <= CSSM_LOOP_MAX_TILES) return GEO_LOOP;
  return pf->d >= CSSM_FINE_MIN_D ? GEO_FINE : GEO_PIPE;
}

void cssm_batch_fresh(cssm_pf* pf, double t0) { fresh_host_state(pf, t0); pf->gen++; pf->done_seq++; }
int cssm_batch_ok(const cssm_pf* pf) {
  return pf->opt_fused && !pf->safe_sums && pf->obs_kind != CSSM_OBS_LGCP && pf->resampler == CSSM_RESAMPLE_SYSTEMATIC && !pf->sharded &&
         large_geometry(pf) != GEO_FINE;
}

int cssm_launch_propagate(cssm_pf* pf, const StepRec* d_rec, double* pick_out, uint32_t pick_slot, const CssmBatchLaunch* batch) {
  if (!pf->h_recs || d_rec < pf->d_recs || d_rec >= pf->d_recs + std::min(pf->h_recs_cap, pf->recs_cap))
    return fail(CSSM_ESTATE, "propagate launched on a record outside the handle's record buffer");
  const uint32_t rec_step = pf->h_recs[d_rec - pf->d_recs].step;
  uint64_t chunk = (uint64_t)pf->sup * CSSM_TILE / pf->split;
  double* dst = pf->state[pf->cur ^ 1];
  const uint32_t* anc = pf->anc_valid ? pf->anc : nullptr;
  const int do_sums = uses_sums_kernel(pf) ? 1 : 0;
  pf->last_optimistic = do_sums != 0;
  const int geo = do_sums ? large_geometry(pf) : GEO_PIPE;
  const bool fine = geo == GEO_FINE;
  const uint64_t unit_particles = (uint64_t)pf->sup * CSSM_TILE;
  if (fine) chunk = (uint64_t)CSSM_BLOCK * cssm_prop_items(pf->d);
  const int grid = (int)((pf->n + chunk - 1) / chunk);
  if (fine && pf->fine_cap < (size_t)grid) {
    HIP_TRY(hipStreamSynchronize(pf->stream));
    if (pf->fineS) (void)hipFree(pf->fineS);
    if (pf->fineS2) (void)hipFree(pf->fineS2);
    pf->fineS = pf->fineS2 = nullptr; pf->fine_cap = 0;
    if (hipMalloc(&pf->fineS, (size_t)grid * sizeof(cssm_u128)) != hipSuccess || hipMalloc(&pf->fineS2, (size_t)grid * sizeof(cssm_u128)) != hipSuccess)
      return fail(CSSM_ENOMEM, "hipMalloc of the per-block sums (%d blocks)", grid);
    pf->fine_cap = (size_t)grid;
  }
  prof_begin(pf, CSSM_K_PROPAGATE);
  PropLaunch a;
  a.chains = nullptr; a.nchains = 0; a.cur = pf->cur; a.anc_valid = pf->anc_valid ? 1 : 0; a.want_pick = 0; a.rec_idx = 0;
  if (batch) { a.chains = batch->chains; a.nchains = batch->nchains; a.want_pick = batch->want_pick; a.rec_idx = batch->rec_idx; }
  a.grid = grid; a.stream = pf->stream;
  a.lgcp = pf->obs_kind == CSSM_OBS_LGCP;
  a.sharded = pf->sharded ? 1 : 0;
  a.obs = (pf->obs_kind == CSSM_OBS_POISSON || pf->obs_kind == CSSM_OBS_GAUSSIAN) ? pf->obs_kind : -1;
  a.sums = do_sums;
  a.src = pf->src; a.src_stride = pf->src_stride; a.anc = anc; a.dst = dst; a.dst_stride = pf->stride; a.logw = pf->logw;
  a.n = pf->n; a.gid0 = pf->first; a.seed = pf->seed; a.rec = d_rec; a.mk = pf->mk; a.sc = pf->sc;
  a.slot_set = pf->sharded ? 0 : pf->wparity;
  const bool big = pf->nunits > (uint32_t)(CSSM_GRP_SMALL * CSSM_GRP_UNITS);
  pf->last_grp = do_sums && !fine && chunk * pf->split == unit_particles && (pf->sharded ? pf->split <= 4u : (pf->split == 1 && pf->first == 0 && pf->n == pf->n_global)) &&
                 pf->nunits >= pf->grp_min_units && (big ? (!pf->sharded && batch == nullptr && pf->nunits <= (uint32_t)(CSSM_GRP_MAX * 64)) : true) &&
                 unit_particles <= CSSM_GRP_MAX_UNIT && pf->opt_grp;
  pf->grp_layout = pf->last_grp ? (big ? 2 : 1) : 0;
  const bool want_grp = pf->last_grp;
  if (want_grp) a.slot_set |= 0x100 | (pf->wparity << 9) | ((big ? 1 : (pf->split == 4u ? 2 : (pf->split == 2u ? 1 : 0))) << 11);
  const bool want_ws = want_grp && geo == GEO_LOOP && !pf->sharded && batch == nullptr && pf->resampler == CSSM_RESAMPLE_SYSTEMATIC &&
                       pf->obs_kind != CSSM_OBS_LGCP && pick_out == nullptr && 4 * (size_t)pf->nunits <= (size_t)pf->s2_stride &&
                       (pf->opt_wave == 2 || (pf->opt_wave != 0 && pf->sup >= 2u && pf->d <= 2));
  if (want_ws) a.slot_set |= 0x2000;
  a.src2 = anc ? pf->src2 : nullptr; a.src2_stride = pf->src2_stride; a.n_split = pf->n_split; a.logtab = pf->d_logtab;
  a.chunk = chunk; a.do_sums = do_sums; a.subS = fine ? pf->fineS : pf->tileS; a.subS2 = want_ws ? pf->tileW : (fine ? pf->fineS2 : pf->tileS2);
  a.pick_out = pick_out; a.pick_slot = pick_slot;
  a.step = rec_step;
  a.fsub = pf->lgcp_tdep ? pf->d_fsub : nullptr;
  a.one = (chunk == (uint64_t)CSSM_BLOCK * cssm_prop_items(pf->d)) ? 1 : (geo == GEO_LOOP ? 2 : 0);
  a.specialise = pf->opt_spec; a.obs_kind = pf->obs_kind;
  a.shard_slim = pf->sharded && do_sums && !a.lgcp && (a.src2 == nullptr || a.src2_stride == 0) && a.fsub == nullptr && pick_out == nullptr &&
                 ((pf->first & 1ull) == 0ull || cssm_prop_items(pf->d) == 1) && (a.slot_set & 0xff) == 0;
  if (a.shard_slim && pf->sup * (uint32_t)CSSM_TILE / (uint32_t)(CSSM_BLOCK * cssm_prop_items(pf->d)) <= CSSM_LOOP_MAX_TILES) a.one = 2;
  int launched = 0;
  switch (pf->d) {
#define CSSM_CASE_PROP(D) case D: launched = cssm_prop_launch_d##D(a); break;
    CSSM_CASE_PROP(1) CSSM_CASE_PROP(2) CSSM_CASE_PROP(3) CSSM_CASE_PROP(4) CSSM_CASE_PROP(5) CSSM_CASE_PROP(6) CSSM_CASE_PROP(7) CSSM_CASE_PROP(8)
    CSSM_CASE_PROP(9) CSSM_CASE_PROP(10) CSSM_CASE_PROP(11) CSSM_CASE_PROP(12) CSSM_CASE_PROP(13) CSSM_CASE_PROP(14) CSSM_CASE_PROP(15)
    default: launched = cssm_prop_launch_d16(a); break;
#undef CSSM_CASE_PROP
  }
  pf->last_grp = want_grp && (launched & CSSM_PROP_LAUNCHED_GRP) != 0;
  pf->last_ws = pf->last_grp && want_ws && (launched & CSSM_PROP_LAUNCHED_WS) != 0;
  prof_end(pf);
  if (fine) {
    prof_begin(pf, CSSM_K_REDUCE);
    hipLaunchKernelGGL(k_reduce_units, dim3((pf->nunits + CSSM_BLOCK / 64 - 1) / (CSSM_BLOCK / 64)), dim3(CSSM_BLOCK), 0, pf->stream,
                       (const cssm_u128*)pf->fineS, (const cssm_u128*)nullptr, (uint32_t)grid, (uint32_t)(unit_particles / chunk), pf->nunits,
                       pf->tileS, pf->tileS2, (const Scalars*)pf->sc, d_rec);
    prof_end(pf);
  }
  HIP_TRY(hipGetLastError());
  pf->cur ^= 1;
  pf->src = pf->state[pf->cur]; pf->src_stride = pf->stride; pf->anc_valid = false; pf->src2 = nullptr;
  return CSSM_OK;
}

static int launch_resample(cssm_pf* pf, const StepRec* d_rec, double* ll_t = nullptr, int32_t* ess_t = nullptr, uint32_t rec_idx = 0, bool allow_grp = true) {
#ifdef CSSM_OFF_STAMPS
  if (!pf->cum) { HIP_TRY(hipMalloc(&pf->cum, pf->stride * 8 + (1u << 20))); HIP_TRY(hipMemsetAsync(pf->cum, 0, 1u << 20, pf->stream)); }
#endif
  if (pf->resampler == CSSM_RESAMPLE_MULTINOMIAL && !pf->cum) {
    if (hipMalloc(&pf->cum, pf->stride * 8) != hipSuccess) return fail(CSSM_ENOMEM, "hipMalloc cumulative weights");
  }
  const bool optimistic = pf->last_optimistic;
  const int tgrid = (int)pf->nunits;
  const int split = optimistic ? (int)pf->split : 1;
  int lean_layout = 0;
  if (!optimistic && allow_grp && !pf->sharded && pf->opt_grp && pf->resampler == CSSM_RESAMPLE_SYSTEMATIC && pf->first == 0 && pf->n == pf->n_global &&
      pf->nunits >= pf->grp_min_units && pf->nunits <= (uint32_t)(CSSM_GRP_MAX * 64) && (uint64_t)pf->sup * CSSM_TILE <= CSSM_GRP_MAX_UNIT)
    lean_layout = pf->nunits > (uint32_t)(CSSM_GRP_SMALL * CSSM_GRP_UNITS) ? 2 : 1;
  if (!optimistic) {
    prof_begin(pf, CSSM_K_TILE_SUMS);
    hipLaunchKernelGGL(k_tile_sums, dim3(tgrid), dim3(CSSM_BLOCK), 0, pf->stream, pf->logw, pf->n, pf->sc, pf->tileS, pf->tileS2, pf->ntiles,
                       pf->sup, pf->nunits, 0, pf->wparity, (const double*)nullptr, pf->d_logtab, d_rec, 0u, (const unsigned long long*)nullptr, 0,
                       lean_layout ? (0x100 | (pf->wparity << 9) | ((lean_layout == 2 ? 1 : 0) << 11)) : 0);
    prof_end(pf);
  }
  const int s2_par = optimistic ? pf->s2_par : -1;
  prof_begin(pf, CSSM_K_OFFSPRING);
#define OFF_ARGS pf->logw, pf->n, pf->sc, (const cssm_u128*)pf->tileS, (const cssm_u128*)pf->tileS2, d_rec, pf->anc, pf->ntiles, pf->sup, pf->nunits, \
                 pf->wparity, ll_t, ess_t, rec_idx, pf->opt_exact, split, pf->seed, pf->cum, pf->s2buf, pf->s2_stride, s2_par, pf->gen
  const int ogrid = tgrid + 1;
#define OFF_WAVE_ARGS pf->logw, pf->n, pf->sc, (const cssm_u128*)pf->tileS, (const cssm_u128*)pf->tileW, d_rec, pf->anc, pf->sup, pf->nunits, pf->wparity, \
                      ll_t, ess_t, rec_idx, pf->opt_exact, pf->s2buf, pf->s2_stride, s2_par, pf->gen
  static const bool no_offw = getenv("CSSM_NO_OFFW") != nullptr;
#define OFF_GO(RS) do { if (optimistic && pf->last_grp && pf->last_ws && !no_offw && RS == CSSM_RESAMPLE_SYSTEMATIC) { \
                          if (pf->grp_layout == 2) hipLaunchKernelGGL((k_offspring_wave<2>), dim3(ogrid), dim3(CSSM_BLOCK), 0, pf->stream, OFF_WAVE_ARGS); \
                          else hipLaunchKernelGGL((k_offspring_wave<1>), dim3(ogrid), dim3(CSSM_BLOCK), 0, pf->stream, OFF_WAVE_ARGS); \
                        } else if (optimistic && pf->last_grp && pf->grp_layout == 2 && RS == CSSM_RESAMPLE_SYSTEMATIC) \
                          hipLaunchKernelGGL((k_offspring_self<CSSM_RESAMPLE_SYSTEMATIC, 2, 2>), dim3(ogrid), dim3(CSSM_BLOCK), 0, pf->stream, OFF_ARGS); \
                        else if (optimistic && pf->last_grp && RS == CSSM_RESAMPLE_SYSTEMATIC) \
                          hipLaunchKernelGGL((k_offspring_self<CSSM_RESAMPLE_SYSTEMATIC, 2, 1>), dim3(ogrid), dim3(CSSM_BLOCK), 0, pf->stream, OFF_ARGS); \
                        else if (optimistic) hipLaunchKernelGGL((k_offspring_self<RS, 2>), dim3(ogrid), dim3(CSSM_BLOCK), 0, pf->stream, OFF_ARGS); \
                        else if (lean_layout == 2 && RS == CSSM_RESAMPLE_SYSTEMATIC) \
                          hipLaunchKernelGGL((k_offspring_self<CSSM_RESAMPLE_SYSTEMATIC, 0, 2>), dim3(ogrid), dim3(CSSM_BLOCK), 0, pf->stream, OFF_ARGS); \
                        else if (lean_layout == 1 && RS == CSSM_RESAMPLE_SYSTEMATIC) \
                          hipLaunchKernelGGL((k_offspring_self<CSSM_RESAMPLE_SYSTEMATIC, 0, 1>), dim3(ogrid), dim3(CSSM_BLOCK), 0, pf->stream, OFF_ARGS); \
                        else hipLaunchKernelGGL((k_offspring_self<RS, 0>), dim3(ogrid), dim3(CSSM_BLOCK), 0, pf->stream, OFF_ARGS); } while (0)
  if (pf->resampler == CSSM_RESAMPLE_STRATIFIED) OFF_GO(CSSM_RESAMPLE_STRATIFIED);
  else if (pf->resampler == CSSM_RESAMPLE_MULTINOMIAL) OFF_GO(CSSM_RESAMPLE_MULTINOMIAL);
  else OFF_GO(CSSM_RESAMPLE_SYSTEMATIC);
#undef OFF_GO
#undef OFF_ARGS
#undef OFF_WAVE_ARGS
  if (pf->resampler == CSSM_RESAMPLE_MULTINOMIAL)
    hipLaunchKernelGGL(k_multinomial, dim3(grid_for(pf->n, 256, kGridCap)), dim3(256), 0, pf->stream, pf->cum, pf->n, pf->seed,
                       pf->h_step_for_resample, pf->anc);
  prof_end(pf);
  pf->wparity = (pf->wparity + 1) % CSSM_MAXSETS;
  HIP_TRY(hipGetLastError());
  pf->anc_valid = true;
  pf->wmode = optimistic;
  pf->have_level = true;
  if (optimistic) pf->s2_par ^= 1;
  return CSSM_OK;
}
static int launch_step(cssm_pf* pf, const StepRec* d_rec, int weighted, uint32_t step_index, double* ll_t = nullptr, int32_t* ess_t = nullptr,
                       uint32_t rec_idx = 0, double* pick_out = nullptr, uint32_t pick_slot = 0) {
  pf->h_step_for_resample = step_index;
  int rc = cssm_launch_propagate(pf, d_rec, pick_out, pick_slot);
  if (rc) return rc;
  if (weighted) rc = launch_resample(pf, d_rec, ll_t, ess_t, rec_idx);
  else if (ll_t) hipLaunchKernelGGL(k_record, dim3(1), dim3(1), 0, pf->stream, pf->sc, ll_t, ess_t, rec_idx);
  return rc;
}

int cssm_check_device_err(cssm_pf* pf, const Scalars& h) {
  if (h.err & 1u) return fail(CSSM_ENONFINITE, "a log-weight is NaN (the reference's breeze distribution constructor would throw)");
  if (h.err & 2u) return fail(CSSM_ENONFINITE, "all particle weights are zero or the maximum log-weight is not finite");
  if (h.err & 16u) return fail(CSSM_ESHARD, "peer-written exchange: a rank's segment did not arrive within the wait bound");
  (void)pf;
  return CSSM_OK;
}
static int read_scalars(cssm_pf* pf, uint32_t T = 0, bool want_ll_t = false, bool want_ess_t = false, bool poll = false) {
  const uint32_t seq = ++pf->done_seq;
  hipLaunchKernelGGL(k_finish, dim3(1), dim3(CSSM_BLOCK), 0, pf->stream, pf->sc, (const cssm_u128*)pf->s2buf, pf->s2_stride, pf->d_ll_t, pf->d_ess_t, T,
                     pf->gen, pf->hd_sc, want_ll_t ? pf->hd_ll_t : (double*)nullptr, want_ess_t ? pf->hd_ess_t : (int32_t*)nullptr,
                     pf->hd_done, seq);
  HIP_TRY(hipGetLastError());
  static const bool no_poll = getenv("CSSM_NO_POLL") != nullptr;
  if (poll && !no_poll && !pf->profile) {
    volatile uint32_t* flag = pf->h_done;
    for (uint64_t spins = 1;; ++spins) {
      if (__atomic_load_n(flag, __ATOMIC_ACQUIRE) == seq) break;
      if ((spins & 0x3fffu) == 0u) {
        const hipError_t q = hipStreamQuery(pf->stream);
        if (q == hipSuccess) {
          if (__atomic_load_n(flag, __ATOMIC_ACQUIRE) == seq) break;
          return fail(CSSM_EHIP, "the stream drained without k_finish's completion word");
        }
        if (q != hipErrorNotReady) return fail(CSSM_EHIP, "HIP error while waiting for the series: %s", hipGetErrorString(q));
      }
    }
  } else {
    HIP_TRY(hipStreamSynchronize(pf->stream));
  }
  pf->ess_host = pf->h_sc->ess;
  return CSSM_OK;
}

struct PreState { int cur; const double* src; size_t src_stride; bool anc_valid; int wparity; };
static inline PreState pre_state(const cssm_pf* pf) { return {pf->cur, pf->src, pf->src_stride, pf->anc_valid, pf->wparity}; }
static int redo_observation(cssm_pf* pf, const PreState& q, const StepRec* d_rec, double* ll_t, int32_t* ess_t, uint32_t rec_idx) {
  pf->cur = q.cur; pf->src = q.src; pf->src_stride = q.src_stride; pf->src2 = nullptr; pf->anc_valid = q.anc_valid; pf->wparity = q.wparity;
  pf->safe_sums = true;
  int rc = cssm_launch_propagate(pf, d_rec, nullptr, 0);
  pf->safe_sums = false;
  if (rc) return rc;
  return launch_resample(pf, d_rec, ll_t, ess_t, rec_idx, false);
}


int cssm_ensure_recs(cssm_pf* pf, size_t T) {
  if (T < 1024) T = 1024;
  if (pf->h_recs_cap < T) {
    if (pf->h_recs) (void)hipHostFree(pf->h_recs);
    pf->h_recs = nullptr;
    HIP_TRY(hipHostMalloc((void**)&pf->h_recs, T * sizeof(StepRec), hipHostMallocDefault));
    pf->h_recs_cap = T;
    pf->h_recs_dev = nullptr;
    if (hipHostGetDevicePointer((void**)&pf->h_recs_dev, pf->h_recs, 0) != hipSuccess) { (void)hipGetLastError(); pf->h_recs_dev = nullptr; }
  }
  if (pf->recs_cap < T) {
    if (pf->d_recs) (void)hipFree(pf->d_recs);
    if (pf->d_ll_t) (void)hipFree(pf->d_ll_t);
    if (pf->d_ess_t) (void)hipFree(pf->d_ess_t);
    if (pf->h_ll_t) (void)hipHostFree(pf->h_ll_t);
    if (pf->h_ess_t) (void)hipHostFree(pf->h_ess_t);
    pf->d_recs = nullptr; pf->d_ll_t = nullptr; pf->d_ess_t = nullptr; pf->h_ll_t = pf->hd_ll_t = nullptr; pf->h_ess_t = pf->hd_ess_t = nullptr;
    HIP_TRY(hipMalloc(&pf->d_recs, (T + 1) * sizeof(StepRec)));
    HIP_TRY(hipMalloc(&pf->d_ll_t, T * 8));
    HIP_TRY(hipMalloc(&pf->d_ess_t, T * 4));
    HIP_TRY(hipHostMalloc((void**)&pf->h_ll_t, T * 8, hipHostMallocMapped));
    HIP_TRY(hipHostMalloc((void**)&pf->h_ess_t, T * 4, hipHostMallocMapped));
    HIP_TRY(hipHostGetDevicePointer((void**)&pf->hd_ll_t, pf->h_ll_t, 0));
    HIP_TRY(hipHostGetDevicePointer((void**)&pf->hd_ess_t, pf->h_ess_t, 0));
    pf->recs_cap = T;
  }
  return CSSM_OK;
}

extern "C" int cssm_pf_init(cssm_pf* pf, double t0) {
  if (!pf) return fail(CSSM_EINVAL_ARG, "null handle");
  int rc = cssm_launch_init(pf, t0);
  if (rc) return rc;
  HIP_TRY(hipStreamSynchronize(pf->stream));
  return CSSM_OK;
}

extern "C" int cssm_pf_init_from(cssm_pf* pf, double t0, const double* state_d) {
  if (!pf || !state_d) return fail(CSSM_EINVAL_ARG, "null argument");
  HIP_TRY(hipSetDevice(pf->device));
  HIP_TRY(hipMemcpyAsync(pf->d_m0, state_d, pf->d * 8, hipMemcpyHostToDevice, pf->stream));
  hipLaunchKernelGGL(k_init_from, dim3(grid_for(pf->n, 256, kGridCap)), dim3(256), 0, pf->stream, pf->state[0], pf->stride, pf->n, pf->d, pf->d_m0);
  HIP_TRY(hipGetLastError());
  int rc = reset_scalars(pf);
  if (rc) return rc;
  HIP_TRY(hipStreamSynchronize(pf->stream));
  rc = upload_init_params(pf);
  if (rc) return rc;
  fresh_host_state(pf, t0);
  return CSSM_OK;
}

extern "C" int cssm_pf_step(cssm_pf* pf, double t, double obs, int has_obs, double* ll_out, int32_t* ess_out) {
  if (!pf) return fail(CSSM_EINVAL_ARG, "null handle");
  if (!pf->initialised) return fail(CSSM_ESTATE, "cssm_pf_step before cssm_pf_init");
  if (pf->sharded) return fail(CSSM_ESTATE, "a sharded handle is driven through the cssm_pf_shard_* stages");
  HIP_TRY(hipSetDevice(pf->device));
  int rc = cssm_ensure_recs(pf, 1);
  if (rc) return rc;
  cssm_build_rec(pf, pf->t, t, obs, has_obs, pf->step, &pf->h_recs[0]);
  rc = cssm_build_fsub(pf, 0, 1, true);
  if (rc) return rc;
  rc = cssm_upload_recs(pf, 0, 1, true);
  if (rc) return rc;
  const int weighted = pf->h_recs[0].has_obs;
  const PreState before = pre_state(pf);
  pf->gen++;
  rc = launch_step(pf, pf->d_recs, weighted, pf->step);
  if (rc) return rc;
  Scalars& h = *pf->h_sc;
  rc = read_scalars(pf, 0, false, false, true);
  if (rc) return rc;
  if ((h.err & 64u) && !(h.err & 3u)) {
    const uint32_t cleared = h.err & ~64u, none = 0xffffffffu;
    HIP_TRY(hipMemcpyAsync(&pf->sc->err, &cleared, sizeof(uint32_t), hipMemcpyHostToDevice, pf->stream));
    HIP_TRY(hipMemcpyAsync(&pf->sc->fail_step, &none, sizeof(uint32_t), hipMemcpyHostToDevice, pf->stream));
    rc = redo_observation(pf, before, pf->d_recs, nullptr, nullptr, 0);
    if (rc) return rc;
    rc = read_scalars(pf);
    if (rc) return rc;
  }
  pf->t = t; pf->step++;
  if (ll_out) *ll_out = h.ll;
  if (ess_out) *ess_out = h.ess;
  return cssm_check_device_err(pf, h);
}
extern "C" int cssm_pf_propagate(cssm_pf* pf, double t, double obs, int has_obs) {
  if (!pf) return fail(CSSM_EINVAL_ARG, "null handle");
  if (!pf->initialised) return fail(CSSM_ESTATE, "cssm_pf_propagate before cssm_pf_init");
  if (pf->sharded) return fail(CSSM_ESTATE, "a sharded handle is driven through the cssm_pf_shard_* stages");
  HIP_TRY(hipSetDevice(pf->device));
  int rc = cssm_ensure_recs(pf, 1);
  if (rc) return rc;
  cssm_build_rec(pf, pf->t, t, obs, has_obs, pf->step, &pf->h_recs[0]);
  rc = cssm_build_fsub(pf, 0, 1, true);
  if (rc) return rc;
  rc = cssm_upload_recs(pf, 0, 1, false);
  if (rc) return rc;
  pf->safe_sums = true;
  rc = cssm_launch_propagate(pf, pf->d_recs);
  pf->safe_sums = false;
  if (rc) return rc;
  if (pf->obs_kind == CSSM_OBS_LGCP || pf->h_recs[0].has_obs) pf->wmode = false;
  static_assert(offsetof(Scalars, maxslot) == 0 && offsetof(Scalars, grp) == sizeof(Scalars::maxslot), "maxslot and grp are contiguous at the head of Scalars");
  HIP_TRY(hipMemsetAsync(pf->sc, 0, offsetof(Scalars, err), pf->stream));
  static const double kNoLevel = cssm_nan();
  HIP_TRY(hipMemcpyAsync(&pf->sc->next_ref, &kNoLevel, sizeof(double), hipMemcpyHostToDevice, pf->stream));
  pf->have_level = false;
  Scalars h;
  HIP_TRY(hipMemcpyAsync(CSSM_SC_TAIL_ARGS(&h, pf->sc), hipMemcpyDeviceToHost, pf->stream));
  HIP_TRY(hipStreamSynchronize(pf->stream));
  pf->wparity = 0;
  pf->t = t; pf->step++;
  return cssm_check_device_err(pf, h);
}

extern "C" int cssm_pf_adopt(cssm_pf* pf, const double* state_dN, double ll, int32_t ess) {
  if (!pf || !state_dN) return fail(CSSM_EINVAL_ARG, "null argument");
  if (!pf->initialised) return fail(CSSM_ESTATE, "cssm_pf_adopt before cssm_pf_init");
  if (pf->sharded) return fail(CSSM_ESTATE, "a sharded handle is driven through the cssm_pf_shard_* stages");
  HIP_TRY(hipSetDevice(pf->device));
  HIP_TRY(hipMemcpy2DAsync(pf->state[pf->cur], pf->stride * 8, state_dN, pf->n * 8, pf->n * 8, pf->d, hipMemcpyHostToDevice, pf->stream));
  HIP_TRY(hipMemcpyAsync(&pf->sc->ll, &ll, sizeof(double), hipMemcpyHostToDevice, pf->stream));
  HIP_TRY(hipMemcpyAsync(&pf->sc->ess, &ess, sizeof(int32_t), hipMemcpyHostToDevice, pf->stream));
  const uint32_t no_pend = 0u;
  HIP_TRY(hipMemcpyAsync(&pf->sc->pend, &no_pend, sizeof(uint32_t), hipMemcpyHostToDevice, pf->stream));
  pf->ess_host = ess;
  HIP_TRY(hipStreamSynchronize(pf->stream));
  pf->src = pf->state[pf->cur]; pf->src_stride = pf->stride; pf->src2 = nullptr; pf->anc_valid = false;
  return CSSM_OK;
}

static int run_filter_once(cssm_pf* pf, const double* t, const double* y, const uint8_t* has, size_t T, double* ll_out,
                           double* ll_t, int32_t* ess_t, double* path, bool* retry, bool cont = false);

static int run_filter(cssm_pf* pf, const double* t, const double* y, const uint8_t* has, size_t T, double* ll_out,
                      double* ll_t, int32_t* ess_t, double* path) {
  bool retry = false;
  int rc = run_filter_once(pf, t, y, has, T, ll_out, ll_t, ess_t, path, &retry);
  if (rc == CSSM_OK && retry) {
    pf->safe_sums = true;
    rc = run_filter_once(pf, t, y, has, T, ll_out, ll_t, ess_t, path, &retry);
    pf->safe_sums = false;
  }
  return rc;
}

static int run_filter_once(cssm_pf* pf, const double* t, const double* y, const uint8_t* has, size_t T, double* ll_out,
                           double* ll_t, int32_t* ess_t, double* path, bool* retry, bool cont) {
  *retry = false;
  if (!pf || !t || !y) return fail(CSSM_EINVAL_ARG, "null argument");
  if (T < 1) return fail(CSSM_EINVAL_ARG, "empty data (the reference's minBy throws on an empty Vector)");
  static const bool timing = getenv("CSSM_CALL_TIMING") != nullptr;
  const auto tp0 = std::chrono::steady_clock::now();
  auto since = [&](std::chrono::steady_clock::time_point a) { return std::chrono::duration<double, std::micro>(std::chrono::steady_clock::now() - a).count(); };
  double ph_rec = 0, ph_up = 0, ph_enq = 0;
  if (pf->sharded) return fail(CSSM_ESTATE, "a sharded handle is driven through the cssm_pf_shard_* stages");
  HIP_TRY(hipSetDevice(pf->device));
  int rc = cssm_ensure_recs(pf, T);
  if (rc) return rc;
  if (cont && (!pf->initialised || path)) return fail(CSSM_ESTATE, "continuing a filter needs an initialised handle (and records no path)");
  double t0 = t[0];
  for (size_t s = 1; s < T; ++s) if (t[s] < t0) t0 = t[s];
  const uint32_t base = cont ? pf->step : 0u;
  double tp = cont ? pf->t : t0;
  const bool head_first = cont && T > 1 && pf->obs_kind != CSSM_OBS_LGCP;
  size_t built = 0;
  if (head_first) {
    cssm_build_rec(pf, tp, t[0], y[0], has ? has[0] : 1, base, &pf->h_recs[0]); tp = t[0]; built = 1;
    rc = cssm_upload_recs(pf, 0, 1, cont);
    if (rc) return rc;
  }
  bool rest_pending = head_first;
  auto build_rest = [&]() -> int {
    for (size_t s = built; s < T; ++s) { cssm_build_rec(pf, tp, t[s], y[s], has ? has[s] : 1, base + (uint32_t)s, &pf->h_recs[s]); tp = t[s]; }
    int r = cssm_build_fsub(pf, 0, T, true);
    if (r) return r;
    ph_rec = since(tp0);
    r = cssm_upload_recs(pf, built, T - built, cont && built == 0);
    ph_up = since(tp0);
    rest_pending = false;
    return r;
  };
  if (!head_first) { rc = build_rest(); if (rc) return rc; }
  if (!cont) {
    rc = cssm_launch_init(pf, t0);
    if (rc) return rc;
  }
  const int cur0 = pf->cur, wpar0 = pf->wparity;
  const bool anc_valid0 = pf->anc_valid;
  const int32_t ess0 = pf->ess_host;
  pf->gen++;
  const int d = pf->d;
  if (path) {
    if (pf->path_cap < (T + 1) * (size_t)d) {
      if (pf->d_path) (void)hipFree(pf->d_path);
      pf->d_path = nullptr;
      HIP_TRY(hipMalloc(&pf->d_path, (T + 1) * (size_t)d * 8));
      pf->path_cap = (T + 1) * (size_t)d;
    }
    const int32_t pr = (int32_t)cssm_philox_draw(pf->seed, 0, 0, CSSM_STREAM_PICK, 0).v[0];
    const uint32_t pa = pr < 0 ? (uint32_t)0 - (uint32_t)pr : (uint32_t)pr;
    hipLaunchKernelGGL(k_pick, dim3(1), dim3(64), 0, pf->stream, pf->src, pf->src_stride, (const uint32_t*)nullptr,
                       (uint64_t)pa % pf->n, d, pf->d_path);
  }
  if (pf->opt_events) HIP_TRY(hipEventRecord(pf->ev0, pf->stream));
  bool folded = false;
  size_t s_from = 0;
  for (;;) {
    const bool may_hold = may_use_sums_kernel(pf);
    for (size_t s = s_from; s < T; ++s) {
      const int weighted = pf->h_recs[s].has_obs;
      double* pick_out = (folded && s >= 1) ? pf->d_path + s * (size_t)d : nullptr;
      const uint32_t pick_slot = s >= 1 ? pf->h_recs[s - 1].pick : 0u;
      pf->h_step_for_resample = base + (uint32_t)s;
      rc = cssm_launch_propagate(pf, pf->d_recs + s, pick_out, pick_slot);
      if (!rc) {
        if (weighted) rc = launch_resample(pf, pf->d_recs + s, pf->d_ll_t, pf->d_ess_t, (uint32_t)s);
        else hipLaunchKernelGGL(k_record, dim3(1), dim3(1), 0, pf->stream, pf->sc, pf->d_ll_t, pf->d_ess_t, (uint32_t)s);
      }
      if (rc) return rc;
      if (rest_pending) { rc = build_rest(); if (rc) return rc; }
      folded = path && s + 1 < T && uses_sums_kernel(pf);
      if (path && !folded)
        hipLaunchKernelGGL(k_pick, dim3(1), dim3(64), 0, pf->stream, pf->src, pf->src_stride,
                           (const uint32_t*)(pf->anc_valid ? pf->anc : nullptr), (uint64_t)pf->h_recs[s].pick, d,
                           pf->d_path + (s + 1) * (size_t)d);
    }
    ph_enq = since(tp0);
    if (pf->opt_events) HIP_TRY(hipEventRecord(pf->ev1, pf->stream));
    HIP_TRY(hipGetLastError());
    if (path) HIP_TRY(hipMemcpyAsync(path, pf->d_path, (T + 1) * (size_t)d * 8, hipMemcpyDeviceToHost, pf->stream));
    rc = read_scalars(pf, (uint32_t)T, ll_t != nullptr, ess_t != nullptr, path == nullptr);
    if (rc) return rc;
    const Scalars& hh = *pf->h_sc;
    if (!may_hold || !(hh.err & 64u) || (hh.err & 3u)) break;
    const size_t sf = (size_t)hh.fail_step - base;
    if (hh.fail_step < base || sf >= T) return fail(CSSM_ESTATE, "held series reports observation %u; this call holds %u .. %zu", hh.fail_step, base, base + T - 1);
    const uint32_t cleared = hh.err & ~64u, none = 0xffffffffu;
    HIP_TRY(hipMemcpyAsync(&pf->sc->err, &cleared, sizeof(uint32_t), hipMemcpyHostToDevice, pf->stream));
    HIP_TRY(hipMemcpyAsync(&pf->sc->fail_step, &none, sizeof(uint32_t), hipMemcpyHostToDevice, pf->stream));
    PreState before;
    before.cur = (int)(((size_t)cur0 + sf) & 1);
    before.src = pf->state[before.cur]; before.src_stride = pf->stride;
    before.anc_valid = sf == 0 ? anc_valid0 : (pf->h_recs[sf - 1].has_obs != 0);
    int wp = wpar0;
    for (size_t q = 0; q < sf; ++q) wp = (wp + (pf->h_recs[q].has_obs ? 1 : 0)) % CSSM_MAXSETS;
    before.wparity = wp;
    pf->h_step_for_resample = base + (uint32_t)sf;
    rc = redo_observation(pf, before, pf->d_recs + sf, pf->d_ll_t, pf->d_ess_t, (uint32_t)sf);
    if (rc) return rc;
    folded = path && sf + 1 < T && uses_sums_kernel(pf);
    if (path && !folded)
      hipLaunchKernelGGL(k_pick, dim3(1), dim3(64), 0, pf->stream, pf->src, pf->src_stride, (const uint32_t*)pf->anc,
                         (uint64_t)pf->h_recs[sf].pick, d, pf->d_path + (sf + 1) * (size_t)d);
    s_from = sf + 1;
  }
  Scalars& h = *pf->h_sc;
  if (ll_t) memcpy(ll_t, pf->h_ll_t, T * 8);
  if (ess_t) {
    memcpy(ess_t, pf->h_ess_t, T * 4);
    for (size_t s = 0; s < T; ++s) if (!pf->h_recs[s].has_obs) ess_t[s] = s ? ess_t[s - 1] : ess0;
  }
  pf->last_ms = -1.f;
  pf->have_events = pf->opt_events != 0;
  if (timing && pf->have_events) { HIP_TRY(hipEventSynchronize(pf->ev1)); HIP_TRY(hipEventElapsedTime(&pf->last_ms, pf->ev0, pf->ev1)); }
  prof_collect(pf);
  if (timing) fprintf(stderr, "cssm call T=%zu: records built %.1f us, upload enqueued %.1f, %zu steps enqueued %.1f, results back %.1f (device loop %.1f us)\n",
                      T, ph_rec, ph_up, T, ph_enq, since(tp0), pf->last_ms * 1e3);
  pf->t = t[T - 1]; pf->step = base + (uint32_t)T;
  if ((h.err & 4u) && !(h.err & 1u) && !pf->safe_sums) { *retry = true; return CSSM_OK; }
  if (ll_out) *ll_out = h.ll;
  return cssm_check_device_err(pf, h);
}

extern "C" int cssm_pf_ll_filter(cssm_pf* pf, const double* t, const double* y, const uint8_t* has_obs, size_t T,
                                 double* ll_out, double* ll_t, int32_t* ess_t) {
  return run_filter(pf, t, y, has_obs, T, ll_out, ll_t, ess_t, nullptr);
}

extern "C" int cssm_pf_ll_filter_more(cssm_pf* pf, const double* t, const double* y, const uint8_t* has_obs, size_t T,
                                      double* ll_out, double* ll_t, int32_t* ess_t) {
  bool retry = false;
  int rc = run_filter_once(pf, t, y, has_obs, T, ll_out, ll_t, ess_t, nullptr, &retry, true);
  if (rc == CSSM_OK && retry) return fail(CSSM_ESTATE, "a continued series cannot be repeated from its start");
  return rc;
}

extern "C" int cssm_pf_filter(cssm_pf* pf, const double* t, const double* y, const uint8_t* has_obs, size_t T,
                              double* ll_out, double* ll_t, int32_t* ess_t, double* path) {
  if (!path) return fail(CSSM_EINVAL_ARG, "path is null (use cssm_pf_ll_filter)");
  return run_filter(pf, t, y, has_obs, T, ll_out, ll_t, ess_t, path);
}

__global__ void k_contract_eval(int fn, const double* __restrict__ x, size_t n, double* __restrict__ out, const double* __restrict__ logtab) {
  const double* tab = stage_log_table(logtab);
  for (size_t i = (size_t)blockIdx.x * blockDim.x + threadIdx.x; i < n; i += (size_t)gridDim.x * blockDim.x) {
    const double v = x[i];
    if (fn == CSSM_FN_EXP) out[i] = cssm_exp(v);
    else if (fn == CSSM_FN_LOG) out[i] = cssm_log(v);
    else if (fn == CSSM_FN_LOG_UNIT) out[i] = cssm_log_unit(v, tab);
    else if (fn == CSSM_FN_SINCOS2PI) { double sn, cs; cssm_sincos2pi(v, &sn, &cs); out[2 * i] = sn; out[2 * i + 1] = cs; }
    else if (fn == CSSM_FN_SINCOS_U24) { double sn, cs; cssm_sincos_u24((uint32_t)v, tab, &sn, &cs); out[2 * i] = sn; out[2 * i + 1] = cs; }
    else if (fn == CSSM_FN_SQRT_RADIUS) out[i] = cssm_sqrt_radius(v);
    else { const cssm_u128 q = cssm_fix_from_double(v); out[2 * i] = cssm_u2d(q.lo); out[2 * i + 1] = cssm_u2d(q.hi); }
  }
}
template <int D>
__global__ void k_contract_normals(uint64_t seed, uint64_t first, uint32_t step, uint32_t tag, size_t n, double* __restrict__ out,
                                   const double* __restrict__ logtab) {
  const double* tab = stage_log_table(logtab);
  for (size_t i = (size_t)blockIdx.x * blockDim.x + threadIdx.x; i < n; i += (size_t)gridDim.x * blockDim.x) {
    double z[D];
    draw_normals<D>(seed, first + i, step, tag, tab, z);
#pragma unroll
    for (int k = 0; k < D; ++k) out[i * D + k] = z[k];
  }
}

extern "C" int cssm_contract_eval(int device, int fn, const double* x, size_t n, double* out, size_t n_out) {
  if (!x || !out || n < 1) return fail(CSSM_EINVAL_ARG, "null argument");
  int ndev = 0;
  if (hipGetDeviceCount(&ndev) != hipSuccess || ndev < 1) return fail(CSSM_EHIP, "no HIP device available (this library has no CPU path)");
  if (device < 0 || device >= ndev) return fail(CSSM_EINVAL_ARG, "device %d out of range", device);
  HIP_TRY(hipSetDevice(device));
  size_t need = n, d = 0, np = 0;
  if (fn == CSSM_FN_SINCOS2PI || fn == CSSM_FN_FIX || fn == CSSM_FN_SINCOS_U24) need = 2 * n;
  else if (fn == CSSM_FN_PAIRED_NORMALS) {
    if (n < 5) return fail(CSSM_EINVAL_ARG, "paired normals take {seed, first, step, tag, d}");
    d = (size_t)x[4];
    if (d < 1 || d > CSSM_MAX_DIM) return fail(CSSM_EINVAL_ARG, "d out of range");
    np = n_out / d; need = np * d;
    if (np < 1) return fail(CSSM_EINVAL_ARG, "out is too small");
  } else if ((fn < CSSM_FN_EXP || fn > CSSM_FN_FIX) && fn != CSSM_FN_SINCOS_U24 && fn != CSSM_FN_SQRT_RADIUS) return fail(CSSM_EINVAL_ARG, "unknown contract function %d", fn);
  if (n_out < need) return fail(CSSM_EINVAL_ARG, "out holds %zu doubles, %zu needed", n_out, need);
  double *dx = nullptr, *dout = nullptr, *dtab = nullptr;
  int rc = CSSM_OK;
  if (hipMalloc(&dx, n * 8) != hipSuccess || hipMalloc(&dout, need * 8) != hipSuccess || hipMalloc(&dtab, sizeof(CSSM_TAB)) != hipSuccess)
    rc = fail(CSSM_ENOMEM, "hipMalloc");
  if (!rc && (hipMemcpy(dx, x, n * 8, hipMemcpyHostToDevice) != hipSuccess || hipMemcpy(dtab, CSSM_TAB, sizeof(CSSM_TAB), hipMemcpyHostToDevice) != hipSuccess))
    rc = fail(CSSM_EHIP, "upload");
  if (!rc) {
    if (fn == CSSM_FN_PAIRED_NORMALS) {
      const uint64_t seed = (uint64_t)x[0], first = (uint64_t)x[1];
      const uint32_t step = (uint32_t)x[2], tag = (uint32_t)x[3];
      DISPATCH_D((int)d, k_contract_normals<D><<<dim3(grid_for(np, 256, 1024)), dim3(256)>>>(seed, first, step, tag, np, dout, dtab));
    } else {
      hipLaunchKernelGGL(k_contract_eval, dim3(grid_for(n, 256, 1024)), dim3(256), 0, 0, fn, dx, n, dout, dtab);
    }
    if (hipGetLastError() != hipSuccess || hipDeviceSynchronize() != hipSuccess) rc = fail(CSSM_EHIP, "contract kernel");
  }
  if (!rc && hipMemcpy(out, dout, need * 8, hipMemcpyDeviceToHost) != hipSuccess) rc = fail(CSSM_EHIP, "download");
  if (dx) (void)hipFree(dx);
  if (dout) (void)hipFree(dout);
  if (dtab) (void)hipFree(dtab);
  return rc;
}

__global__ __launch_bounds__(256) void k_diag_copy(const uint4* __restrict__ src, uint4* __restrict__ dst, size_t n16) {
  for (size_t i = (size_t)blockIdx.x * 256 + threadIdx.x; i < n16; i += (size_t)gridDim.x * 256) dst[i] = src[i];
}
extern "C" int cssm_diag_copy_ceiling(int device, size_t bytes, int reps, double* gbps_out) {
  if (!gbps_out || bytes < (1u << 20) || reps < 1) return fail(CSSM_EINVAL_ARG, "bytes >= 1 MiB, reps >= 1 and an output pointer are required");
  int ndev = 0;
  if (hipGetDeviceCount(&ndev) != hipSuccess || ndev < 1) return fail(CSSM_EHIP, "no HIP device available (this library has no CPU path)");
  if (device < 0 || device >= ndev) return fail(CSSM_EINVAL_ARG, "device %d out of range", device);
  HIP_TRY(hipSetDevice(device));
  const size_t n16 = bytes / 16;
  uint4 *a = nullptr, *b = nullptr;
  hipEvent_t e0 = nullptr, e1 = nullptr;
  int rc = CSSM_OK;
  if (hipMalloc(&a, n16 * 16) != hipSuccess || hipMalloc(&b, n16 * 16) != hipSuccess) rc = fail(CSSM_ENOMEM, "hipMalloc of 2 x %zu bytes", n16 * 16);
  if (!rc && (hipMemset(a, 1, n16 * 16) != hipSuccess || hipEventCreate(&e0) != hipSuccess || hipEventCreate(&e1) != hipSuccess)) rc = fail(CSSM_EHIP, "setup");
  if (!rc) {
    const int grid = 65536;
    hipLaunchKernelGGL(k_diag_copy, dim3(grid), dim3(256), 0, 0, a, b, n16);
    (void)hipEventRecord(e0, 0);
    for (int r = 0; r < reps; ++r) hipLaunchKernelGGL(k_diag_copy, dim3(grid), dim3(256), 0, 0, (r & 1) ? b : a, (r & 1) ? a : b, n16);
    (void)hipEventRecord(e1, 0);
    float ms = 0.f;
    if (hipEventSynchronize(e1) != hipSuccess || hipEventElapsedTime(&ms, e0, e1) != hipSuccess || hipGetLastError() != hipSuccess) rc = fail(CSSM_EHIP, "copy kernel");
    else *gbps_out = 2.0 * (double)(n16 * 16) * reps / ((double)ms * 1e-3) / 1e9;
  }
  if (e0) (void)hipEventDestroy(e0);
  if (e1) (void)hipEventDestroy(e1);
  if (a) (void)hipFree(a);
  if (b) (void)hipFree(b);
  return rc;
}

extern "C" int cssm_pf_last_loop_ms(cssm_pf* pf, float* ms_out) {
  if (!pf || !ms_out) return fail(CSSM_EINVAL_ARG, "null argument");
  if (pf->last_ms < 0.f) {
    if (!pf->have_events) return fail(CSSM_ESTATE, "the last batch call recorded no events: set CSSM_OPT_LOOP_EVENTS = 1 before it");
    HIP_TRY(hipSetDevice(pf->device));
    HIP_TRY(hipEventSynchronize(pf->ev1));
    HIP_TRY(hipEventElapsedTime(&pf->last_ms, pf->ev0, pf->ev1));
  }
  *ms_out = pf->last_ms;
  return CSSM_OK;
}

extern "C" int cssm_pf_last_device_us(cssm_pf* pf, double* us_out) {
  if (!pf || !us_out) return fail(CSSM_EINVAL_ARG, "null argument");
  if (!pf->h_sc) return fail(CSSM_ESTATE, "no call has run");
  const unsigned long long a = pf->h_sc->t_first, b = pf->h_sc->t_last;
  if (a == 0ull || b < a) return fail(CSSM_ESTATE, "the last call left no pair of device stamps (it drew a new cloud, or none has run)");
  *us_out = (double)(b - a) * 1e-2;
  return CSSM_OK;
}

extern "C" int cssm_pf_stream_idle(cssm_pf* pf) {
  if (!pf) return fail(CSSM_EINVAL_ARG, "null handle");
  if (hipSetDevice(pf->device) != hipSuccess) return fail(CSSM_EHIP, "hipSetDevice(%d)", pf->device);
  const hipError_t q = hipStreamQuery(pf->stream);
  if (q == hipSuccess) return 1;
  if (q == hipErrorNotReady) { (void)hipGetLastError(); return 0; }
  return fail(CSSM_EHIP, "hipStreamQuery: %s", hipGetErrorString(q));
}

extern "C" int cssm_pf_set_option(cssm_pf* pf, int option, int value) {
  if (!pf) return fail(CSSM_EINVAL_ARG, "null handle");
  if (option == CSSM_OPT_EXACT_OFFSPRING) { pf->opt_exact = (value == 2) ? 2 : (value ? 1 : 0); return CSSM_OK; }
  if (option == CSSM_OPT_FUSED_SUMS) { pf->opt_fused = value ? 1 : 0; return CSSM_OK; }
  if (option == CSSM_OPT_GROUP_SUMS) { pf->opt_grp = value ? 1 : 0; return CSSM_OK; }
  if (option == CSSM_OPT_WAVE_SUMS) { pf->opt_wave = value == 2 ? 2 : (value ? 1 : 0); return CSSM_OK; }
  if (option == CSSM_OPT_LOOP_EVENTS) { pf->opt_events = value ? 1 : 0; return CSSM_OK; }
  if (option == CSSM_OPT_FORECAST_CAP) {
    if (value < 0) return fail(CSSM_EINVAL_ARG, "the forecast key-buffer cap is a number of KiB >= 0");
    pf->forecast_cap = (size_t)value * 1024;
    return CSSM_OK;
  }
  if (option == CSSM_OPT_SPECIALISE) { pf->opt_spec = (value == 2) ? 2 : (value ? 1 : 0); return CSSM_OK; }
  if (option == CSSM_OPT_WHOLE_TILES) {
    if (pf->sharded) return fail(CSSM_ESTATE, "sharded handles always run whole tiles");
    pf->opt_whole = value < 0 ? 0 : (value > 3 ? 3 : value);
    pf->split = value ? 1u : auto_split(pf);
    return CSSM_OK;
  }
  if (option == CSSM_OPT_RESAMPLER) {
    if (value < CSSM_RESAMPLE_SYSTEMATIC || value > CSSM_RESAMPLE_MULTINOMIAL) return fail(CSSM_EINVAL_ARG, "unknown resampler %d", value);
    if (pf->sharded && value == CSSM_RESAMPLE_MULTINOMIAL) return fail(CSSM_ESTATE, "sharded handles resample systematically or stratified");
    pf->resampler = value;
    return CSSM_OK;
  }
  return fail(CSSM_EINVAL_ARG, "unknown option %d", option);
}

extern "C" int cssm_pf_profile(cssm_pf* pf, int enable) {
  if (!pf) return fail(CSSM_EINVAL_ARG, "null handle");
  pf->profile = enable != 0;
  pf->prof_used = 0;
  for (int k = 0; k < CSSM_NKERNELS; ++k) { pf->prof_ms[k] = 0.0; pf->prof_cnt[k] = 0; }
  return CSSM_OK;
}

extern "C" int cssm_pf_profile_read(cssm_pf* pf, double* total_ms, uint64_t* launches) {
  if (!pf || !total_ms || !launches) return fail(CSSM_EINVAL_ARG, "null argument");
  for (int k = 0; k < CSSM_NKERNELS; ++k) { total_ms[k] = pf->prof_ms[k]; launches[k] = pf->prof_cnt[k]; }
  return CSSM_OK;
}


extern "C" int cssm_pf_get_particles(cssm_pf* pf, double* out) {
  if (!pf || !out) return fail(CSSM_EINVAL_ARG, "null argument");
  if (!pf->initialised) return fail(CSSM_ESTATE, "not initialised");
  HIP_TRY(hipSetDevice(pf->device));
  double* tmp = nullptr;
  if (hipMalloc(&tmp, pf->n * (size_t)pf->d * 8) != hipSuccess) return fail(CSSM_ENOMEM, "hipMalloc for the gathered cloud");
  hipLaunchKernelGGL(k_gather, dim3(grid_for(pf->n, 256, kGridCap)), dim3(256), 0, pf->stream, pf->src, pf->src_stride,
                     (const uint32_t*)(pf->anc_valid ? pf->anc : nullptr), tmp, (size_t)pf->n, pf->n, pf->d,
                     pf->anc_valid ? pf->src2 : nullptr, pf->src2_stride, pf->n_split);
  hipError_t e = hipMemcpyAsync(out, tmp, pf->n * (size_t)pf->d * 8, hipMemcpyDeviceToHost, pf->stream);
  if (e == hipSuccess) e = hipStreamSynchronize(pf->stream);
  (void)hipFree(tmp);
  if (e != hipSuccess) return fail(CSSM_EHIP, "get_particles: %s", hipGetErrorString(e));
  return CSSM_OK;
}

extern "C" int cssm_pf_get_proposed(cssm_pf* pf, double* out) {
  if (!pf || !out) return fail(CSSM_EINVAL_ARG, "null argument");
  if (!pf->initialised) return fail(CSSM_ESTATE, "not initialised");
  HIP_TRY(hipSetDevice(pf->device));
  HIP_TRY(hipMemcpy2DAsync(out, pf->n * 8, pf->state[pf->cur], pf->stride * 8, pf->n * 8, pf->d, hipMemcpyDeviceToHost, pf->stream));
  HIP_TRY(hipStreamSynchronize(pf->stream));
  return CSSM_OK;
}

extern "C" int cssm_pf_get_ancestors(cssm_pf* pf, uint32_t* out) {
  if (!pf || !out) return fail(CSSM_EINVAL_ARG, "null argument");
  HIP_TRY(hipSetDevice(pf->device));
  if (!pf->anc_valid) { for (uint64_t i = 0; i < pf->n; ++i) out[i] = (uint32_t)i; return CSSM_OK; }
  HIP_TRY(hipMemcpyAsync(out, pf->anc, pf->n * 4, hipMemcpyDeviceToHost, pf->stream));
  HIP_TRY(hipStreamSynchronize(pf->stream));
  return CSSM_OK;
}

extern "C" int cssm_pf_get_weights(cssm_pf* pf, double* out, double* level_out) {
  if (!pf || !out) return fail(CSSM_EINVAL_ARG, "null argument");
  if (!pf->wmode) return fail(CSSM_ESTATE, "the last weighted step kept log-weights (cssm_pf_get_logw), not weights");
  HIP_TRY(hipSetDevice(pf->device));
  Scalars h;
  HIP_TRY(hipMemcpyAsync(out, pf->logw, pf->n * 8, hipMemcpyDeviceToHost, pf->stream));
  HIP_TRY(hipMemcpyAsync(CSSM_SC_TAIL_ARGS(&h, pf->sc), hipMemcpyDeviceToHost, pf->stream));
  HIP_TRY(hipStreamSynchronize(pf->stream));
  if (level_out) *level_out = h.ref;
  return CSSM_OK;
}

extern "C" int cssm_pf_get_logw(cssm_pf* pf, double* out) {
  if (!pf || !out) return fail(CSSM_EINVAL_ARG, "null argument");
  if (pf->wmode) return fail(CSSM_ESTATE, "the fused kernel keeps the weights exp(w - c) in place of the log-weights (cssm_pf_get_weights); "
                                          "CSSM_OPT_FUSED_SUMS = 0 keeps log-weights");
  HIP_TRY(hipSetDevice(pf->device));
  HIP_TRY(hipMemcpyAsync(out, pf->logw, pf->n * 8, hipMemcpyDeviceToHost, pf->stream));
  HIP_TRY(hipStreamSynchronize(pf->stream));
  return CSSM_OK;
}

static double host_link(int obs_kind, double g) {
  switch (obs_kind) {
    case CSSM_OBS_POISSON: case CSSM_OBS_NEGBIN: case CSSM_OBS_ZIP: return cssm_exp(g);
    case CSSM_OBS_BERNOULLI: return (g > 6.0) ? 1.0 : ((g < -6.0) ? 0.0 : 1.0 / (1.0 + cssm_exp(-g)));
    case CSSM_OBS_BETA: return cssm_exp(-g);
    default: return g;
  }
}

double cssm_eta_of_mean(const cssm_pf* pf, const StepRec& rec, const double* mean) {
  double g = 0.0, acc = 0.0;
  for (int k = 0; k < pf->d; ++k) {
    const int fm = pf->mk.fmode(k);
    if (fm == FM_START) acc = rec.fco[k] * mean[k]; else if (fm == FM_ADD) acc = acc + rec.fco[k] * mean[k];
    if (pf->mk.leaf_end(k)) g = pf->mk.first_leaf(k) ? acc : g + acc;
  }
  return host_link(pf->obs_kind, g);
}

static int summary_impl(cssm_pf* pf, const double* src, size_t src_stride, const uint32_t* idx, const double* src2, size_t src2_stride,
                        uint32_t n_split, double time, double interval, double* state_mean, double* state_lower, double* state_upper,
                        double* eta_of_mean, double* eta_lower, double* eta_upper) {
  const int d = pf->d, rows = d + 1;
  const uint64_t n = pf->n;
  const int nblocks = grid_for(n, CSSM_BLOCK, 1024);
  unsigned long long* keys = nullptr; double* partial = nullptr; SelState* st = nullptr; uint32_t* hist = nullptr; double* out = nullptr;
  StepRec* drec = nullptr;
  std::vector<SelState> hst(rows);
  std::vector<double> hout(3 * rows);
  StepRec hrec;
  int rc = CSSM_OK;
  const long long idxr = (long long)std::floor(interval * (double)n);
  auto clampr = [&](long long r) { return (unsigned long long)std::min<long long>(std::max<long long>(r, 0), (long long)n - 1); };
  for (int k = 0; k < rows; ++k) {
    hst[k].prefix[0] = hst[k].prefix[1] = 0;
    hst[k].rank[0] = clampr(k < d ? (long long)n - idxr - 1 : (long long)n - idxr);
    hst[k].rank[1] = clampr(k < d ? idxr - 1 : idxr);
  }
  cssm_build_rec(pf, time, time, 0.0, 0, pf->step, &hrec);
#define SM_TRY(expr) do { hipError_t e__ = (expr); if (e__ != hipSuccess) { rc = fail(CSSM_EHIP, "%s: %s", #expr, hipGetErrorString(e__)); goto done; } } while (0)
  SM_TRY(hipMalloc(&keys, (size_t)rows * n * 8)); SM_TRY(hipMalloc(&partial, (size_t)nblocks * d * 8));
  SM_TRY(hipMalloc(&st, rows * sizeof(SelState))); SM_TRY(hipMalloc(&hist, (size_t)rows * 512 * 4)); SM_TRY(hipMalloc(&out, 3 * rows * 8));
  SM_TRY(hipMalloc(&drec, sizeof(StepRec)));
  SM_TRY(hipMemcpyAsync(st, hst.data(), rows * sizeof(SelState), hipMemcpyHostToDevice, pf->stream));
  SM_TRY(hipMemcpyAsync(drec, &hrec, sizeof hrec, hipMemcpyHostToDevice, pf->stream));
  SM_TRY(hipMemsetAsync(hist, 0, (size_t)rows * 512 * 4, pf->stream));
  {
    DISPATCH_D(d, k_summary_fill<D><<<dim3(nblocks), dim3(CSSM_BLOCK), 0, pf->stream>>>(
                      src, src_stride, idx, idx ? src2 : nullptr, src2_stride, n_split, n, drec, pf->mk, keys, (size_t)n, partial));
    for (int shift = 56; shift >= 0; shift -= 8) {
      hipLaunchKernelGGL(k_sel_hist, dim3(nblocks, rows), dim3(CSSM_BLOCK), 0, pf->stream, keys, (size_t)n, n, st, shift, hist);
      hipLaunchKernelGGL(k_sel_pick, dim3(rows), dim3(2), 0, pf->stream, st, shift, hist);
    }
    hipLaunchKernelGGL(k_summary_finish, dim3(1), dim3(64), 0, pf->stream, st, partial, nblocks, d, n, out);
  }
  SM_TRY(hipGetLastError());
  SM_TRY(hipMemcpyAsync(hout.data(), out, 3 * rows * 8, hipMemcpyDeviceToHost, pf->stream));
  SM_TRY(hipStreamSynchronize(pf->stream));
  for (int k = 0; k < d; ++k) {
    if (state_mean) state_mean[k] = hout[k];
    if (state_lower) state_lower[k] = hout[rows + k];
// ... 189 lines not shown
```

composablestatespacemodels_amd/csrc/cssm_propagate.hip.h:

```cpp
#pragma once

#if !defined(__HIPCC_RTC__)
#include <cstddef>
#endif

#include "cssm_device.hip.h"

#ifndef CSSM_PROP_IT_LO
#define CSSM_PROP_IT_LO 2
#endif
#ifndef CSSM_PROP_WR
#define CSSM_PROP_WR 1
#endif
template <int D> struct PropItems { static constexpr int value = (D <= 2) ? CSSM_PROP_IT_LO : (D <= 8 ? CSSM_PROP_IT_MID : 1); };


#ifndef CSSM_PROP_WAVES_LO
#define CSSM_PROP_WAVES_LO 4
#endif
#ifndef CSSM_PROP_WAVES_SUMS
#define CSSM_PROP_WAVES_SUMS 4
#endif
template <int D, int SUMS = 0> struct PropWaves { static constexpr int value = (D <= 4) ? (SUMS ? CSSM_PROP_WAVES_SUMS : CSSM_PROP_WAVES_LO) : 3; };

#ifdef CSSM_PROP_STAMPS
static __device__ unsigned long long g_prop_stamps[8192 * 8];
#define PSTAMP(k) do { if (threadIdx.x == 0 && blockIdx.x < 8192) g_prop_stamps[blockIdx.x * 8 + (k)] = __builtin_amdgcn_s_memrealtime(); } while (0)
#else
#define PSTAMP(k) do { } while (0)
#endif

template <int D, int IT> struct PropStage {
  static constexpr int ES = (IT * D <= 8) ? 16 : 8;
  static constexpr int wave_bytes = IT * D * 64 * ES;
  static constexpr int bytes = (CSSM_BLOCK / 64) * wave_bytes;
};

struct PropAcc {
  cssm_u128 S, S2;
  double tmax;
  bool bad;
};

template <int D, bool LGCP, int IT, int OBS, int SUMS, int ONE = 0, bool WR = false>
__device__ __forceinline__ void propagate_range(
    const double* __restrict__ src, size_t src_stride, const uint32_t* __restrict__ anc,
    double* __restrict__ dst, size_t dst_stride, double* __restrict__ logw, uint64_t gid0,
    uint64_t seed, const StepRec* __restrict__ rec, const ModelK& mk,
    const double* __restrict__ src2, size_t src2_stride, uint32_t n_split, const double* tab,
    const uint32_t range_lo, const uint32_t n, int do_sums_arg,
    double* __restrict__ pick_out, uint32_t pick_slot, unsigned char* s_stage, PropAcc& acc,
    const double* __restrict__ fsub = nullptr, const unsigned long long* pre_jp = nullptr, const cssm_u32x4* pre_blk = nullptr,
    const uint32_t step_now = 0u, const bool wr_on = false) {
  const uint32_t step = (pre_blk != nullptr) ? step_now : rec->step;
  const int has_obs = rec->has_obs;
  const double dt = rec->dt;
  const bool weighted = LGCP || has_obs;
  const bool pair_ok = (gid0 & 1ull) == 0ull;
  const bool do_sums = SUMS && do_sums_arg && weighted;
  const double cref = rec->ref;
  cssm_u128 accS = cssm_u128_zero(), accS2 = cssm_u128_zero();
  double tmax = -cssm_inf();
  bool bad = false;
  static_assert(!WR || ONE == 2, "wave ranges: the tile-after-tile instantiation");
  const bool wr = WR && wr_on;
  const uint32_t stride = (wr ? 64u : (uint32_t)CSSM_BLOCK) * IT;
  const uint32_t tl = wr ? (threadIdx.x & 63u) : threadIdx.x;
  constexpr bool STAGE = true;
  constexpr int ES = (IT * D <= 8) ? 16 : 8;
  constexpr int WAVE_STAGE = IT * D * 64 * ES;
  unsigned char* const wstage = s_stage + (size_t)(threadIdx.x >> 6) * WAVE_STAGE;
  const uint32_t wstage_lds = __builtin_amdgcn_readfirstlane((uint32_t)(size_t)(__attribute__((address_space(3))) void*)wstage);
  const uint32_t n_last = n - 1u;
  constexpr int NJ = (IT + 1) / 2;
  auto load_idx = [&](uint32_t base, unsigned long long (&jp)[NJ]) {
    const uint32_t i0 = base + tl * IT;
    if (anc) {
      if (IT == 4) {
        const ulonglong2 a = *reinterpret_cast<const ulonglong2*>(anc + i0);
        jp[0] = a.x; jp[NJ - 1] = a.y;
      } else if (IT == 2) {
        jp[0] = *reinterpret_cast<const unsigned long long*>(anc + i0);
      } else {
        jp[0] = anc[i0];
      }
    } else {
#pragma unroll
      for (int q = 0; q < NJ; ++q) jp[q] = (unsigned long long)(uint32_t)(i0 + 2 * q) | ((unsigned long long)(uint32_t)(i0 + 2 * q + 1) << 32);
    }
  };
  auto unpack_idx = [&](uint32_t base, const unsigned long long (&jp)[NJ], uint32_t (&j)[IT]) {
    const uint32_t i0 = base + tl * IT;
#pragma unroll
    for (int r = 0; r < IT; ++r) {
      const uint32_t v = (uint32_t)(jp[r / 2] >> (32 * (r & 1)));
      j[r] = (i0 + r < n) ? v : n_last;
    }
  };
  auto ptr_of = [&](uint32_t j, int k) -> const double* {
    if (src2 && j >= n_split)
      return (src2_stride == 0) ? src2 + (size_t)(j - n_split) * (size_t)(D + 1) + k : src2 + (size_t)k * src2_stride + (j - n_split);
    return src + (size_t)k * src_stride + j;
  };
  auto gather = [&](const uint32_t (&j)[IT], double (&x)[IT][D]) {
#pragma unroll
    for (int r = 0; r < IT; ++r)
#pragma unroll
      for (int k = 0; k < D; ++k) x[r][k] = (src2 && j[r] >= n_split) ? ld_sys_f64(ptr_of(j[r], k)) : *ptr_of(j[r], k);
  };
  auto stage_issue = [&](const uint32_t (&j)[IT]) {
    bool local_only = (src2 == nullptr);
    if (src2 != nullptr) {
      uint32_t jm = j[0];
#pragma unroll
      for (int r = 1; r < IT; ++r) jm = (j[r] > jm) ? j[r] : jm;
      local_only = !__any(jm >= n_split);
    }
#pragma unroll
    for (int r = 0; r < IT; ++r)
#pragma unroll
      for (int k = 0; k < D; ++k) {
        const double* g = local_only ? src + (size_t)k * src_stride + j[r] : ptr_of(j[r], k);
        const uint32_t slot = wstage_lds + (uint32_t)((r * D + k) * 64 * ES);
        if (!local_only && j[r] >= n_split) {
          const double v = ld_sys_f64(g);
          unsigned char* sl = wstage + (size_t)((r * D + k) * 64 * ES);
          const uint32_t lane = threadIdx.x & 63;
          if (ES == 16) {
            *reinterpret_cast<double*>(sl + lane * 16) = v;
          } else {
            *reinterpret_cast<uint32_t*>(sl + lane * 4) = (uint32_t)cssm_d2u(v);
            *reinterpret_cast<uint32_t*>(sl + 256 + lane * 4) = (uint32_t)(cssm_d2u(v) >> 32);
          }
        } else
        if (ES == 16) {
          lds_dma16(g, slot);
        } else {
          lds_dma4(g, slot);
          lds_dma4(reinterpret_cast<const unsigned char*>(g) + 4, slot + 256u);
        }
      }
  };
  auto stage_read = [&](double (&x)[IT][D]) {
    const uint32_t lane = threadIdx.x & 63;
#pragma unroll
    for (int r = 0; r < IT; ++r)
#pragma unroll
      for (int k = 0; k < D; ++k) {
        const unsigned char* slot = wstage + (r * D + k) * 64 * ES;
        if (ES == 16) {
          x[r][k] = *reinterpret_cast<const double*>(slot + lane * 16);
        } else {
          const uint32_t lo = *reinterpret_cast<const uint32_t*>(slot + lane * 4);
          const uint32_t hi = *reinterpret_cast<const uint32_t*>(slot + 256 + lane * 4);
          x[r][k] = cssm_u2d((uint64_t)lo | ((uint64_t)hi << 32));
        }
      }
  };
  uint32_t base = range_lo;
  unsigned long long jp[NJ];
  uint32_t jn[IT];
  double x[IT][D];
  static_assert(!ONE || (IT <= 2 && !LGCP), "ONE: one pair (d <= 8) or one particle (d >= 9) per thread, ordinary step");
  double zz[ONE ? IT * D : 1];
  if (base < n) {
    if (NJ == 1 && pre_jp != nullptr) jp[0] = *pre_jp; else load_idx(base, jp);
    if (ONE && IT == 2 && pre_jp == nullptr) {
      normals_pair_half<D, 0>(seed, gid0 + base + tl * IT, step, tab, zz);
#pragma unroll
      for (int q = 0; q < PairHalf<D>::n0; ++q) asm volatile("" : "+v"(zz[q % (ONE ? IT * D : 1)]), "+v"(jp[0]));
      if (PairHalf<D>::n0 == 0) asm volatile("" : "+v"(jp[0]));
    }
    unpack_idx(base, jp, jn);
    if (STAGE) {
      stage_issue(jn);
      if (!ONE && base + stride < n) load_idx(base + stride, jp);
      if (ONE && IT == 2) {
        if (pre_blk != nullptr) {
          normals_pair_from_blocks<D>(pre_blk, tab, zz);
        } else {
          if (pre_jp != nullptr) normals_pair_half<D, 0>(seed, gid0 + base + tl * IT, step, tab, zz);
          normals_pair_half<D, 1>(seed, gid0 + base + tl * IT, step, tab, zz);
        }
#pragma unroll
        for (int q = (pre_jp != nullptr) ? 0 : PairHalf<D>::n0; q < 2 * D; ++q) asm volatile("" : "+v"(zz[q % (ONE ? IT * D : 1)]));
      } else if (ONE) {
        double z1[D];
        draw_normals<D>(seed, gid0 + base + tl, step, CSSM_STREAM_STEP, tab, z1);
#pragma unroll
        for (int q = 0; q < D; ++q) { zz[q % (ONE ? IT * D : 1)] = z1[q]; asm volatile("" : "+v"(zz[q % (ONE ? IT * D : 1)])); }
      }
      if (ONE) PSTAMP(2);
      asm volatile("s_waitcnt vmcnt(0)" ::: "memory");
      stage_read(x);
      asm volatile("s_waitcnt lgkmcnt(0)" ::: "memory");
      if (ONE) PSTAMP(3);
      if (!ONE && base + stride < n) {
        unpack_idx(base + stride, jp, jn);
        stage_issue(jn);
        if (base + 2 * stride < n) load_idx(base + 2 * stride, jp);
      }
    } else {
      gather(jn, x);
    }
  }
  for (; base < n; base += stride) {
    const uint32_t i0 = base + tl * IT;
    const bool full = (i0 + IT <= n);
    if (ONE == 2 && base + stride < n) load_idx(base + stride, jp);
    if (SUMS && pick_out != nullptr) {
#pragma unroll
      for (int r = 0; r < IT; ++r)
        if (i0 + r == pick_slot) {
#pragma unroll
          for (int k = 0; k < D; ++k) pick_out[k] = x[r][k];
        }
    }
    double lw[IT];
    auto account = [&](int r) {
      if (weighted && i0 + r < n) {
        if (lw[r] != lw[r]) { bad = true; lw[r] = -cssm_inf(); }
        tmax = (lw[r] > tmax) ? lw[r] : tmax;
        if (SUMS && do_sums) {
          const double a = cssm_min_c(lw[r] - cref, CSSM_REF_BELOW);
          const double w1 = cssm_exp_le0(a);
          accS = cssm_u128_add(accS, cssm_fix_from_unit(w1));
          if (SUMS == 2) accS2 = cssm_u128_add(accS2, cssm_fix_from_unit(w1 * w1));
          lw[r] = w1;
        }
      }
    };
    if (LGCP) {
#pragma unroll
      for (int r = 0; r < IT; ++r) {
        double z[D];
        const uint64_t gid = gid0 + i0 + r;
        const int nsub = rec->n_sub;
        if (nsub == 0) {
          double g = gamma_of<D>(mk, rec, x[r]);
          lw[r] = g - g;
        } else {
          double haz = 0.0, carry = 0.0;
          uint32_t held_a = 0u, held_b = 0u;
          const double* fsub_obs = (fsub != nullptr) ? fsub + rec->fsub_off : nullptr;
          for (int s = 0; s < nsub; ++s) {
#pragma unroll
            for (int k = 0; k < D; ++k) {
              const uint32_t q = (uint32_t)s * D + k;
              if ((q & 1u) == 0u) {
                double z0, z1;
                if ((q & 2u) == 0u) {
                  const cssm_u32x4 blk = cssm_philox_draw(seed, gid, step, CSSM_STREAM_STEP, q >> 2);
                  held_a = blk.v[2]; held_b = blk.v[3];
                  cssm_normal_pair64(blk.v[0], blk.v[1], tab, &z0, &z1);
                } else {
                  cssm_normal_pair64(held_a, held_b, tab, &z0, &z1);
                }
                z[k] = z0; carry = z1;
              } else {
                z[k] = carry;
              }
            }
            transition<D>(mk, rec, dt, x[r], z);
            const double* fc = (fsub_obs != nullptr) ? fsub_obs + (size_t)s * D : rec->fco;
            haz = haz + cssm_exp(gamma_coef<D>(mk, fc, x[r])) * dt;
          }
          lw[r] = gamma_of<D>(mk, rec, x[r]) - haz;
        }
        account(r);
      }
    } else if (ONE) {
#pragma unroll
      for (int q = 0; q < IT * D; ++q) transition_one<D>(mk, rec, dt, q % D, x[(q / D) % IT][q % D], zz[q % (ONE ? IT * D : 1)]);
#pragma unroll
      for (int r = 0; r < IT; ++r) {
        lw[r] = has_obs ? logdens<OBS>(mk, rec, gamma_of<D>(mk, rec, x[r]), tab) : 0.0;
        account(r);
      }
    } else if (IT % 2 == 0 && pair_ok) {
#pragma unroll
      for (int r = 0; r + 1 < IT; r += 2) {
        propagate_pair<D>(mk, rec, dt, seed, gid0 + i0 + r, step, tab, x[r], x[(r + 1) % IT]);
        lw[r] = has_obs ? logdens<OBS>(mk, rec, gamma_of<D>(mk, rec, x[r]), tab) : 0.0;
        account(r);
        lw[(r + 1) % IT] = has_obs ? logdens<OBS>(mk, rec, gamma_of<D>(mk, rec, x[(r + 1) % IT]), tab) : 0.0;
        account((r + 1) % IT);
      }
    } else {
#pragma unroll
      for (int r = 0; r < IT; ++r) {
        propagate_one<D>(mk, rec, dt, seed, gid0 + i0 + r, step, tab, x[r]);
        lw[r] = has_obs ? logdens<OBS>(mk, rec, gamma_of<D>(mk, rec, x[r]), tab) : 0.0;
        account(r);
      }
    }
    if (STAGE) {
      asm volatile("s_waitcnt vmcnt(0)" ::: "memory");
#pragma unroll
      for (int q = 0; q < NJ; ++q) asm volatile("" : "+v"(jp[q]));
    }
    if (full && IT == 4) {
#pragma unroll
      for (int k = 0; k < D; ++k) {
        double* p = dst + (size_t)k * dst_stride + i0;
        *reinterpret_cast<double2*>(p) = make_double2(x[0][k], x[1 % IT][k]);
        *reinterpret_cast<double2*>(p + 2) = make_double2(x[2 % IT][k], x[3 % IT][k]);
      }
      if (weighted) {
        *reinterpret_cast<double2*>(logw + i0) = make_double2(lw[0], lw[1 % IT]);
        *reinterpret_cast<double2*>(logw + i0 + 2) = make_double2(lw[2 % IT], lw[3 % IT]);
      }
    } else if (full && IT == 2) {
#pragma unroll
      for (int k = 0; k < D; ++k)
        bulk_store2(dst + (size_t)k * dst_stride + i0, x[0][k], x[1 % IT][k]);
      if (weighted && logw) bulk_store2(logw + i0, lw[0], lw[1 % IT]);
    } else {
#pragma unroll
      for (int r = 0; r < IT; ++r) {
        if (i0 + r < n) {
#pragma unroll
          for (int k = 0; k < D; ++k) dst[(size_t)k * dst_stride + i0 + r] = x[r][k];
          if (weighted && logw) logw[i0 + r] = lw[r];
        }
      }
    }
    if (ONE && base == range_lo) PSTAMP(4);
    if (ONE == 1) break;
    if (ONE == 2) {
      const uint32_t nb = base + stride;
      if (nb < n) {
        unpack_idx(nb, jp, jn);
        stage_issue(jn);
        if (IT == 2) {
          normals_pair_half<D, 0>(seed, gid0 + nb + tl * IT, step, tab, zz);
          normals_pair_half<D, 1>(seed, gid0 + nb + tl * IT, step, tab, zz);
        } else {
          double z1[D];
          draw_normals<D>(seed, gid0 + nb + tl, step, CSSM_STREAM_STEP, tab, z1);
#pragma unroll
          for (int q = 0; q < D; ++q) zz[q % (ONE ? IT * D : 1)] = z1[q];
        }
#pragma unroll
        for (int q = 0; q < IT * D; ++q) asm volatile("" : "+v"(zz[q % (ONE ? IT * D : 1)]));
        asm volatile("s_waitcnt vmcnt(0)" ::: "memory");
        stage_read(x);
        asm volatile("s_waitcnt lgkmcnt(0)" ::: "memory");
        if (base == range_lo) PSTAMP(5);
      }
      continue;
    }
    if (STAGE) {
      if (base + stride < n) {
        stage_read(x);
        asm volatile("s_waitcnt lgkmcnt(0)" ::: "memory");
        if (base + 2 * stride < n) {
          unpack_idx(base + 2 * stride, jp, jn);
          stage_issue(jn);
          if (base + 3 * stride < n) load_idx(base + 3 * stride, jp);
        }
      }
    } else if (base + stride < n) {
      load_idx(base + stride, jp);
      unpack_idx(base + stride, jp, jn);
      gather(jn, x);
    }
  }
  acc.S = accS; acc.S2 = accS2; acc.tmax = tmax; acc.bad = bad;
}

template <int D, bool LGCP, int IT, int OBS, int SUMS, uint32_t MKW = 0u, uint32_t MKW1 = 0u, uint32_t MKW2 = 0u>
__global__ __launch_bounds__(CSSM_BLOCK, (PropWaves<D, SUMS>::value)) void k_propagate(
    const double* __restrict__ src, size_t src_stride, const uint32_t* __restrict__ anc,
    double* __restrict__ dst, size_t dst_stride, double* __restrict__ logw, uint64_t n_arg, uint64_t gid0,
    uint64_t seed, const StepRec* __restrict__ rec, ModelK mk, Scalars* __restrict__ sc, int slot_set_arg,
    const double* __restrict__ src2, size_t src2_stride, uint32_t n_split, const double* __restrict__ logtab,
    uint64_t chunk, int do_sums_arg, cssm_u128* __restrict__ subS, cssm_u128* __restrict__ subS2,
    double* __restrict__ pick_out, uint32_t pick_slot, const double* __restrict__ fsub) {
  __shared__ double s_max[CSSM_BLOCK / 64];
  if (MKW != 0u) { mk.comp[0] = MKW; mk.comp[1] = MKW1; mk.comp[2] = MKW2; }
  const int slot_set = slot_set_arg & 0xff;
  const bool grp_on = (slot_set_arg & 0x100) != 0;
  const int grp_set = (slot_set_arg >> 9) & 3;
  const int grp_shift = 5 + ((slot_set_arg >> 11) & 3);
  const uint32_t held = sc->err;
  const uint32_t range_lo = blockIdx.x * (uint32_t)chunk;
  uint32_t n;
  { const uint64_t range_hi = (uint64_t)range_lo + chunk; n = (uint32_t)((range_hi < n_arg) ? range_hi : n_arg); }
  constexpr bool EARLY_IDX = (IT == 2);
  unsigned long long jp_early = 0ull;
  if (EARLY_IDX && range_lo < n) {
    const uint32_t i0 = range_lo + threadIdx.x * IT;
    jp_early = anc ? *reinterpret_cast<const unsigned long long*>(anc + i0) : ((unsigned long long)i0 | ((unsigned long long)(i0 + 1u) << 32));
  }
  static_assert(CSSM_BLOCK == 256, "three table entries per thread");
  const double tv = logtab[threadIdx.x], tv1 = logtab[256 + threadIdx.x], tv2 = logtab[512 + threadIdx.x];
  const double* tab = stage_log_table_finish(tv, tv1, tv2);
  if (held & (4u | 8u | 16u | 64u)) return;
  __shared__ __attribute__((aligned(16))) unsigned char s_stage[PropStage<D, IT>::bytes];
  PropAcc acc;
  propagate_range<D, LGCP, IT, OBS, SUMS>(src, src_stride, anc, dst, dst_stride, logw, gid0, seed, rec, mk, src2, src2_stride,
                                          n_split, tab, range_lo, n, do_sums_arg, pick_out, pick_slot, s_stage, acc, LGCP ? fsub : nullptr,
                                          (EARLY_IDX && range_lo < n) ? &jp_early : nullptr);
  const bool weighted = LGCP || rec->has_obs;
  const bool do_sums = SUMS && do_sums_arg && weighted;
  cssm_u128 accS = acc.S, accS2 = acc.S2;
  double tmax = acc.tmax;
  const bool bad = acc.bad;
  if (!weighted) return;
  tmax = wave_max(tmax);
  if ((threadIdx.x & 63) == 0) s_max[threadIdx.x >> 6] = tmax;
  if (__any(bad) && (threadIdx.x & 63) == 0) atomicOr(&sc->err, 1u);
  if (SUMS && do_sums) {
    __shared__ cssm_u128 s_sa[CSSM_BLOCK / 64], s_sb[CSSM_BLOCK / 64];
    accS = wave_sum_u128(accS);
    if (SUMS == 2) accS2 = wave_sum_u128(accS2);
    if ((threadIdx.x & 63) == 0) { s_sa[threadIdx.x >> 6] = accS; if (SUMS == 2) s_sb[threadIdx.x >> 6] = accS2; }
    __syncthreads();
    if (threadIdx.x == 0) {
      cssm_u128 ta = s_sa[0], tb = (SUMS == 2) ? s_sb[0] : cssm_u128_zero();
#pragma unroll
      for (int w = 1; w < CSSM_BLOCK / 64; ++w) { ta = cssm_u128_add(ta, s_sa[w]); if (SUMS == 2) tb = cssm_u128_add(tb, s_sb[w]); }
      subS[blockIdx.x] = ta;
      if (SUMS == 2) subS2[blockIdx.x] = tb;
      if (grp_on) group_sums_add(sc, grp_set, blockIdx.x >> grp_shift, ta, tb, SUMS == 2);
    }
  } else {
    __syncthreads();
  }
  if (threadIdx.x == 0) {
    double m = s_max[0];
#pragma unroll
    for (int w = 1; w < CSSM_BLOCK / 64; ++w) m = (s_max[w] > m) ? s_max[w] : m;
    atomicMax(&sc->maxslot[((size_t)slot_set * CSSM_MAXSLOTS + blockIdx.x % CSSM_MAXSLOTS) * CSSM_SLOT_STRIDE],
              (unsigned long long)cssm_order_key(m));
  }
}

template <int D, int IT, int OBS, int SUMS, int ONE>
__device__ __forceinline__ void propagate_block(
    const double* __restrict__ src, size_t src_stride, const uint32_t* __restrict__ anc, double* __restrict__ dst, size_t dst_stride,
    double* __restrict__ logw, uint64_t n_arg, uint64_t seed, const StepRec* __restrict__ rec, const ModelK& mk, Scalars* __restrict__ sc,
    int slot_set_arg, const double* __restrict__ logtab, uint64_t chunk,
    cssm_u128* __restrict__ subS, cssm_u128* __restrict__ subS2, double* __restrict__ pick_out, uint32_t pick_slot,
    const uint64_t gid0, const double* __restrict__ src2, const uint32_t n_split, const uint32_t step_now) {
  const int slot_set = slot_set_arg & 0xff;
  const bool grp_on = (slot_set_arg & 0x100) != 0;
  const int grp_set = (slot_set_arg >> 9) & 3;
  const int grp_shift = 5 + ((slot_set_arg >> 11) & 3);
  __shared__ double s_max[CSSM_BLOCK / 64];
  uint32_t key_lo = (uint32_t)seed, key_hi = (uint32_t)(seed >> 32), step_k = step_now;
  if (ONE != 0 && IT == 2) asm volatile("" : "+s"(key_lo), "+s"(key_hi), "+s"(step_k));
  PSTAMP(0);
  const uint32_t held = sc->err;
  constexpr bool WR = CSSM_PROP_WR != 0 && (ONE == 2 && SUMS == 1);
  const bool wsum_on = WR && (slot_set_arg & 0x2000) != 0;
  uint32_t range_lo = blockIdx.x * (uint32_t)chunk;
  uint32_t n;
  { const uint64_t range_hi = (uint64_t)range_lo + chunk; n = (uint32_t)((range_hi < n_arg) ? range_hi : n_arg); }
  if (wsum_on) {
    const uint32_t qw = (uint32_t)(chunk >> 2);
    const uint32_t wlo = range_lo + (threadIdx.x >> 6) * qw;
    const uint32_t whi = ((uint64_t)wlo + qw < (uint64_t)n) ? wlo + qw : n;
    range_lo = (uint32_t)__builtin_amdgcn_readfirstlane((int)((wlo < n) ? wlo : n));
    n = (uint32_t)__builtin_amdgcn_readfirstlane((int)whi);
  }
  const uint32_t tl = wsum_on ? (threadIdx.x & 63u) : threadIdx.x;
  unsigned long long jp_early = 0ull;
  if (ONE) {
    const uint32_t i0 = range_lo + tl * IT;
    const bool in_buf = !wsum_on || range_lo < n;
    if (IT == 2) jp_early = (anc && in_buf) ? *reinterpret_cast<const unsigned long long*>(anc + i0) : ((unsigned long long)i0 | ((unsigned long long)(i0 + 1u) << 32));
    else jp_early = (anc && in_buf) ? (unsigned long long)anc[i0] : (unsigned long long)i0;
  }
  const double* tab;
  constexpr bool EARLY = ONE != 0 && IT == 2;
  cssm_u32x4 blk_early[EARLY ? PairHalf<D>::nblk : 1];
  if (ONE) {
    static_assert(CSSM_BLOCK == 256, "one table entry per thread");
// ... 111 lines not shown
```

include/cssm_pf.h:

```cpp
#ifndef CSSM_PF_H
#define CSSM_PF_H

#if !defined(__HIPCC_RTC__)
#include <stddef.h>
#include <stdint.h>
#endif

#ifdef __cplusplus
extern "C" {
#endif

#define CSSM_OK 0
#define CSSM_EINVAL_DESC (-1)
#define CSSM_EHIP (-2)
#define CSSM_ESHARD (-3)
#define CSSM_ENOMEM (-4)
#define CSSM_ENONFINITE (-5)
#define CSSM_EINVAL_ARG (-6)
#define CSSM_ESTATE (-7)
#define CSSM_ERCCL (-8)

#define CSSM_SDE_BROWNIAN 0
#define CSSM_SDE_GEN_BROWNIAN 1
#define CSSM_SDE_OU 2
#define CSSM_SDE_EULER_AFFINE 3

#define CSSM_F_FIRST 0
#define CSSM_F_SEASONAL 1

#define CSSM_OBS_POISSON 0
#define CSSM_OBS_GAUSSIAN 1
#define CSSM_OBS_LGCP 2
#define CSSM_OBS_NEGBIN 3
#define CSSM_OBS_ZIP 4
#define CSSM_OBS_BERNOULLI 5
#define CSSM_OBS_STUDENT_T 6
#define CSSM_OBS_BETA 7

#define CSSM_MAX_DIM 16
#define CSSM_MAX_LEAVES 16

typedef struct cssm_leaf_desc {
  int32_t sde_kind;
  int32_t dim;
  int32_t f_kind;
  int32_t period;
  int32_t harmonics;
  int32_t has_scale;
  double scale;
  int32_t n_m0, n_c0, n_mu, n_phi, n_sigma;
  int32_t reserved;
  const double* m0;
  const double* c0;
  const double* mu;
  const double* phi;
  const double* sigma;
} cssm_leaf_desc;

typedef struct cssm_model_desc {
  int32_t n_leaves;
  int32_t obs_kind;
  int32_t lgcp_precision;
  int32_t obs_df;
  const cssm_leaf_desc* leaves;
} cssm_model_desc;

typedef struct cssm_pf cssm_pf;


int cssm_pf_create(const cssm_model_desc* desc, uint64_t n_particles, uint64_t seed, int device,
                   cssm_pf** out);

int cssm_pf_create_shard(const cssm_model_desc* desc, uint64_t n_global, uint64_t first,
                         uint64_t n_local, uint64_t seed, int device, void* hip_stream,
                         cssm_pf** out);

void cssm_pf_destroy(cssm_pf* pf);

int cssm_pf_set_params(cssm_pf* pf, const cssm_model_desc* desc);

int cssm_pf_reseed(cssm_pf* pf, uint64_t seed);
uint64_t cssm_pf_run_key(uint64_t seed, uint64_t run);


int cssm_pf_init(cssm_pf* pf, double t0);

int cssm_pf_init_from(cssm_pf* pf, double t0, const double* state_d);

int cssm_pf_step(cssm_pf* pf, double t, double obs, int has_obs, double* ll_out, int32_t* ess_out);

int cssm_pf_propagate(cssm_pf* pf, double t, double obs, int has_obs);
int cssm_pf_adopt(cssm_pf* pf, const double* state_dN, double ll, int32_t ess);


int cssm_pf_ll_filter(cssm_pf* pf, const double* t, const double* y, const uint8_t* has_obs,
                      size_t T, double* ll_out, double* ll_t, int32_t* ess_t);
int cssm_pf_ll_filter_more(cssm_pf* pf, const double* t, const double* y, const uint8_t* has_obs, size_t T,
                           double* ll_out, double* ll_t, int32_t* ess_t);

int cssm_pf_filter(cssm_pf* pf, const double* t, const double* y, const uint8_t* has_obs, size_t T,
                   double* ll_out, double* ll_t, int32_t* ess_t, double* path);

int cssm_pf_last_loop_ms(cssm_pf* pf, float* ms_out);

int cssm_pf_last_device_us(cssm_pf* pf, double* us_out);

int cssm_pf_stream_idle(cssm_pf* pf);

#define CSSM_OPT_EXACT_OFFSPRING 1
#define CSSM_OPT_RESAMPLER 2
#define CSSM_RESAMPLE_SYSTEMATIC 0
#define CSSM_RESAMPLE_STRATIFIED 1
#define CSSM_RESAMPLE_MULTINOMIAL 2
#define CSSM_OPT_FUSED_SUMS 3
#define CSSM_OPT_WHOLE_TILES 6
#define CSSM_OPT_GROUP_SUMS 7
#define CSSM_OPT_SPECIALISE 8
#define CSSM_OPT_LOOP_EVENTS 9
#define CSSM_OPT_WAVE_SUMS 10
#define CSSM_OPT_FORECAST_CAP 11
int cssm_pf_set_option(cssm_pf* pf, int option, int value);
int cssm_rtc_info(uint64_t* out4);

#define CSSM_K_PROPAGATE 0
#define CSSM_K_TILE_SUMS 1
#define CSSM_K_OFFSPRING 2
#define CSSM_K_REDUCE 3
#define CSSM_K_PACK 4
#define CSSM_K_EXPAND 5
#define CSSM_K_COLLECTIVE 6
#define CSSM_PROFILE_NKERNELS 7
int cssm_pf_profile(cssm_pf* pf, int enable);
int cssm_pf_profile_read(cssm_pf* pf, double* total_ms, uint64_t* launches);

#define CSSM_FN_EXP 0
#define CSSM_FN_LOG 1
#define CSSM_FN_LOG_UNIT 2
#define CSSM_FN_SINCOS2PI 3
#define CSSM_FN_FIX 4
#define CSSM_FN_PAIRED_NORMALS 5
#define CSSM_FN_SINCOS_U24 6
#define CSSM_FN_SQRT_RADIUS 7
int cssm_contract_eval(int device, int fn, const double* x, size_t n, double* out, size_t n_out);

int cssm_diag_copy_ceiling(int device, size_t bytes, int reps, double* gbps_out);


uint64_t cssm_pf_num_particles(const cssm_pf* pf);
int32_t cssm_pf_dim(const cssm_pf* pf);

int cssm_pf_get_particles(cssm_pf* pf, double* out_dN);
int cssm_pf_get_ancestors(cssm_pf* pf, uint32_t* out_N);
int cssm_pf_get_logw(cssm_pf* pf, double* out_N);
int cssm_pf_get_weights(cssm_pf* pf, double* out_N, double* level_out);
int cssm_pf_get_proposed(cssm_pf* pf, double* out_dN);

int cssm_pf_summary(cssm_pf* pf, double interval, double* state_mean, double* state_lower, double* state_upper,
                    double* eta_of_mean, double* eta_lower, double* eta_upper);

int cssm_pf_forecast(cssm_pf* pf, const double* t, size_t H, uint64_t key, double interval, double* state_mean, double* state_lower,
                     double* state_upper, double* eta_mean, double* eta_lower, double* eta_upper, double* obs_mean, double* obs_lower,
                     double* obs_upper, double* samples);
int cssm_pf_forecast_posterior(cssm_pf* pf, const cssm_model_desc* desc, const double* theta, size_t n_theta, const double* x, size_t M,
                               double t0, const double* t, size_t H, const uint32_t* pick, uint64_t key, double interval,
                               double* state_mean, double* state_lower, double* state_upper, double* eta_mean, double* eta_lower,
                               double* eta_upper, double* obs_mean, double* obs_lower, double* obs_upper, double* samples, uint32_t* pick_out);
int cssm_pf_forecast_last_ms(cssm_pf* pf, double* ms2);
uint64_t cssm_pf_observation_index(const cssm_pf* pf);
int cssm_obs_draw(int obs_kind, const double* eta, size_t n, int has_scale, double scale, int df, uint64_t key, uint32_t step,
                  double* out, int device);

#define CSSM_INTERP_REFERENCE_PAIRING 1
int cssm_pf_interpolate(cssm_pf* pf, const double* t, const double* y, const uint8_t* has_obs, size_t T, double interval,
                        int flags, double* ll_out, double* state_mean, double* state_lower, double* state_upper,
                        double* eta_of_mean, double* eta_lower, double* eta_upper);


int cssm_resample_systematic(const double* w, size_t n, double u, uint32_t* anc, int device);
int cssm_resample(int kind, const double* w, size_t n, double u, uint64_t seed, uint32_t step, uint32_t* anc, int device);
int cssm_resample_residual(const double* w, size_t n, uint64_t seed, uint32_t step, uint32_t* anc, int device);

int cssm_pf_shard_init(cssm_pf* pf, double t0);
int cssm_pf_shard_propagate(cssm_pf* pf, double t, double obs, int has_obs, uint64_t* sums5_dev);
int cssm_pf_shard_sums(cssm_pf* pf, const uint64_t* all_sums5_dev, int world, uint64_t* sums5_dev);
int cssm_pf_shard_offspring(cssm_pf* pf, const uint64_t* all_sums5_dev, int rank, int world,
                            int64_t* send_first_dev, int64_t* send_count_dev, uint64_t* redo_flag_dev);
int cssm_pf_shard_pack(cssm_pf* pf, int world, const int64_t* send_first_host,
                       const int64_t* send_count_host, int skip_rank, double* send_buf_dev);
int cssm_pf_shard_adopt(cssm_pf* pf, const double* recv_buf_dev, int64_t n_low, int64_t n_high,
                        int64_t self_first, int64_t self_count);
int cssm_pf_shard_result(cssm_pf* pf, double* ll_out, int32_t* ess_out);

int cssm_pf_shard_begin(cssm_pf* pf, const double* t, const double* y, const uint8_t* has_obs, size_t T);
int cssm_pf_shard_wait_stats(cssm_pf* pf, uint64_t* out4);

int cssm_pf_shard_continue(cssm_pf* pf, const double* t, const double* y, const uint8_t* has_obs, size_t T);
int cssm_pf_shard_propagate_at(cssm_pf* pf, size_t s, uint64_t* sums5_dev);
int cssm_pf_shard_status(cssm_pf* pf, double* ll_out, int32_t* ess_out, uint32_t* bits_out, uint32_t* need, size_t T);
int cssm_pf_shard_want_path(cssm_pf* pf, int on);
int cssm_pf_shard_get_path(cssm_pf* pf, double* out_host, size_t T);

int cssm_pf_shard_summary_begin(cssm_pf* pf, double interval, double* sums_dev, uint32_t* hist_dev);
int cssm_pf_shard_summary_hist(cssm_pf* pf, int shift, uint32_t* hist_dev);
int cssm_pf_shard_summary_pick(cssm_pf* pf, int shift, uint32_t* hist_dev);
int cssm_pf_shard_summary_finish(cssm_pf* pf, const double* sums_global_dev, double* state_mean, double* state_lower, double* state_upper,
                                 double* eta_of_mean, double* eta_lower, double* eta_upper);

int64_t cssm_pf_shard_spec_segment(const cssm_pf* pf, int64_t cap);
int64_t cssm_pf_shard_unit(const cssm_pf* pf);
int cssm_pf_shard_boundary_pack(cssm_pf* pf, int rank, int world, int64_t cap, double* send_buf_dev);
int cssm_pf_shard_adopt_spec(cssm_pf* pf, const double* recv_buf_dev, int rank, int world, int64_t cap);
int cssm_pf_shard_resume(cssm_pf* pf, uint32_t* fail_step_out);
int cssm_pf_shard_resume_level(cssm_pf* pf, uint32_t* fail_step_out);

typedef struct { char internal[128]; } cssm_rccl_id;
int cssm_rccl_available(void);
const char* cssm_rccl_library(void);
int cssm_rccl_unique_id(cssm_rccl_id* id_out);
int cssm_rccl_comm_create(const cssm_rccl_id* id, int world, int rank, int device, void** comm_out);
void cssm_rccl_comm_destroy(void* comm);
int cssm_pf_shard_series_rccl(cssm_pf* pf, void* comm, int rank, int world, size_t s_begin, size_t s_end,
                              const uint8_t* weighted, int64_t cap, uint64_t* sums5_dev, uint64_t* all_sums5_dev,
                              double* send_buf_dev, double* recv_buf_dev, int single_collective);

typedef struct cssm_peer_handle {
  char ipc[64];
  uint64_t pid;
  uint64_t local_ptr;
  uint64_t bytes;
  int32_t device, has_ipc;
} cssm_peer_handle;
int cssm_pf_shard_peer_setup(cssm_pf* pf, int rank, int world, int64_t cap, cssm_peer_handle* mine_out);
int cssm_pf_shard_peer_connect(cssm_pf* pf, const cssm_peer_handle* all_handles, int world);
int cssm_pf_shard_peer_handshake(cssm_pf* pf, uint32_t token);
uint32_t cssm_pf_shard_peer_probe_stale(const cssm_pf* pf);
void cssm_pf_shard_peer_close(cssm_pf* pf);
int cssm_pf_shard_pack_peer(cssm_pf* pf, int rank, int world, int64_t cap);
int cssm_pf_shard_pack_rows_peer(cssm_pf* pf, int rank, int world, int64_t cap);
int cssm_pf_shard_peer_rows(cssm_pf* pf, uint64_t* rows_out, uint64_t* segments_out, uint64_t* beyond_out);
int64_t cssm_pf_shard_peer_debug(cssm_pf* pf, uint32_t* out, size_t nwords);
int cssm_pf_shard_adopt_peer(cssm_pf* pf, int rank, int world, int64_t cap);
int cssm_pf_shard_exchange_peer(cssm_pf* pf, int rank, int world, int64_t cap);
int cssm_pf_shard_series_peer(cssm_pf* pf, int rank, int world, size_t s_begin, size_t s_end, const uint8_t* weighted, int64_t cap);

int cssm_pmmh_run(cssm_pf* pf, const cssm_model_desc* desc, const double* theta0, size_t n_theta,
                  double delta, const double* t, const double* y, const uint8_t* has_obs, size_t T,
                  uint64_t seed, size_t n_iters, double* ll, double* theta, int32_t* accepted,
                  double* last_state);

typedef struct cssm_pfb cssm_pfb;
int cssm_pfb_create(const cssm_model_desc* desc, uint64_t n_particles, int n_chains, int device, cssm_pfb** out);
void cssm_pfb_destroy(cssm_pfb* b);
int cssm_pfb_num_chains(const cssm_pfb* b);
cssm_pf* cssm_pfb_chain(cssm_pfb* b, int k);
int cssm_pfb_filter(cssm_pfb* b, const cssm_model_desc* const* descs, const uint64_t* seeds, const double* t, const double* y,
                    const uint8_t* has_obs, size_t T, double* ll_out, double* path_out, int* rc_out);
int cssm_pmmh_run_batched(cssm_pfb* b, const cssm_model_desc* desc, const double* theta0, size_t n_theta, double delta, const double* t,
                          const double* y, const uint8_t* has_obs, size_t T, const uint64_t* seeds, size_t n_iters, double* ll, double* theta,
                          int32_t* accepted, double* last_state);
int cssm_pmmh_run_speculative(cssm_pfb* b, const cssm_model_desc* desc, const double* theta0, size_t n_theta, double delta, const double* t,
                              const double* y, const uint8_t* has_obs, size_t T, uint64_t seed, size_t n_iters, double* ll, double* theta,
                              int32_t* accepted, double* last_state);

int cssm_desc_flatten(const cssm_model_desc* desc, double* theta, size_t cap, size_t* n_theta);

int cssm_model_structure(const cssm_model_desc* desc, uint32_t* words_out, int32_t* d_out);

typedef struct cssm_fleet cssm_fleet;
#define CSSM_FLEET_MAX_N 4096

int cssm_fleet_create(const cssm_model_desc* desc, uint64_t n_particles, uint32_t n_series, int device, cssm_fleet** out);
void cssm_fleet_destroy(cssm_fleet* f);
uint32_t cssm_fleet_num_series(const cssm_fleet* f);
// ... 28 lines not shown
```

Measured before the change: 51.69 billion.

## Fuse offspring resampling with next-step propagation into one kernel launch

Adds a k_step_parents kernel that runs the systematic offspring/ancestor computation for step t and then, in the same block, propagates the particle range it just filled for step t+1. It accumulates per-unit weight sums as 48-bit limbs via atomics, so the next resample reads them directly. The host loop defers each resample and merges it with the following weighted propagate. This removes one launch and one full pass over ancestors and states per step. The cost is extra atomics, a second weight buffer, and a path limited to one specialised model (d=3, Poisson, a specific component word).

```diff
diff --git a/composablestatespacemodels_amd/csrc/cssm_device.hip.h b/composablestatespacemodels_amd/csrc/cssm_device.hip.h
--- a/composablestatespacemodels_amd/csrc/cssm_device.hip.h
+++ b/composablestatespacemodels_amd/csrc/cssm_device.hip.h
@@ -21,6 +21,7 @@
 #define CSSM_GRP_MAX 64
 #define CSSM_GRP_SMALL 32
 #define CSSM_GRP_LIMB 56
+#define CSSM_STEP_LIMB 48
 #define CSSM_GRP_MAX_UNIT (1u << 15)
 struct Scalars {
   unsigned long long maxslot[CSSM_MAXSETS * CSSM_MAXSLOTS * CSSM_SLOT_STRIDE];
diff --git a/composablestatespacemodels_amd/csrc/cssm_host.h b/composablestatespacemodels_amd/csrc/cssm_host.h
--- a/composablestatespacemodels_amd/csrc/cssm_host.h
+++ b/composablestatespacemodels_amd/csrc/cssm_host.h
@@ -28,6 +28,18 @@
   int obs_kind;
 };
 
+struct StepLaunch {
+  hipStream_t stream;
+  const double* logw_in; uint64_t n; Scalars* sc; const cssm_u128* unitP; const unsigned long long* ulimb_in; const StepRec* rec_t; uint32_t* anc;
+  uint32_t ntiles, nunits; int set_t; double* ll_t; int32_t* ess_t; uint32_t rec_idx; int force_exact; uint64_t seed;
+  cssm_u128* s2buf; uint32_t s2_stride; int s2_par; uint32_t gen;
+  const double* src; size_t stride; double* dst; double* logw_out; const StepRec* rec_n; ModelK mk; const double* logtab;
+  unsigned long long* ulimb_out; unsigned long long* ulimb_far; int set_n;
+};
+bool cssm_step_parents_has(const ModelK& mk, int d, int obs_kind);
+bool cssm_step_parents_launch(const StepLaunch& a, int d, int obs_kind);
+void cssm_offspring_limb_launch(const StepLaunch& a);
+
 bool cssm_rtc_launch(const PropLaunch& a, int kind, int D, int IT, int onev);
 
 #define CSSM_PROP_LAUNCHED_GRP 1
diff --git a/composablestatespacemodels_amd/csrc/cssm_internal.h b/composablestatespacemodels_amd/csrc/cssm_internal.h
--- a/composablestatespacemodels_amd/csrc/cssm_internal.h
+++ b/composablestatespacemodels_amd/csrc/cssm_internal.h
@@ -67,6 +67,10 @@
   int grp_layout = 0;
   bool last_ws = false;
   int opt_wave = 1;
+  int opt_one = 1;
+  double* logw2 = nullptr;
+  unsigned long long* ulimb = nullptr;
+  bool sums_limb = false;
   cssm_u128* tileW = nullptr;
   int resampler = CSSM_RESAMPLE_SYSTEMATIC;
   double* cum = nullptr;
diff --git a/composablestatespacemodels_amd/csrc/cssm_offspring.hip.h b/composablestatespacemodels_amd/csrc/cssm_offspring.hip.h
--- a/composablestatespacemodels_amd/csrc/cssm_offspring.hip.h
+++ b/composablestatespacemodels_amd/csrc/cssm_offspring.hip.h
@@ -148,7 +148,8 @@
 __device__ __forceinline__ void publish_observation(Scalars* __restrict__ sc, const StepRec* __restrict__ rec, const double gmax_dec, const double gmax,
                                                     const cssm_u128 tot, const cssm_u128 tot2, const bool p_pend, const cssm_u128 ptot2,
                                                     const int s2_par, const uint32_t nunits, const uint32_t rec_idx, const uint32_t gen,
-                                                    double* __restrict__ ll_t, int32_t* __restrict__ ess_t, const uint64_t n_global, const int slot_set) {
+                                                    double* __restrict__ ll_t, int32_t* __restrict__ ess_t, const uint64_t n_global, const int slot_set,
+                                                    const bool far_only = false, unsigned long long* __restrict__ ulimb_clear = nullptr, const uint32_t ulimb_n = 0u) {
   if (threadIdx.x == 0) {
     if (p_pend) {
       const int32_t pe = cssm_ess_of(sc->pend_S, ptot2);
@@ -168,11 +169,12 @@
       if (ll_t) ll_t[rec_idx] = sc->ll;
     }
   }
-  if (threadIdx.x < 2 * 2 * CSSM_GRP_MAX) {
+  if (ulimb_clear != nullptr) for (uint32_t q = threadIdx.x; q < ulimb_n; q += CSSM_BLOCK) ulimb_clear[q] = 0ull;
+  if (threadIdx.x < 2 * 2 * CSSM_GRP_MAX && (!far_only || threadIdx.x >= 2 * CSSM_GRP_MAX)) {
     const uint32_t tq2 = threadIdx.x;
     sc->grp[((size_t)((slot_set + 1 + (int)(tq2 / (2 * CSSM_GRP_MAX))) % CSSM_MAXSETS) * 2 * CSSM_GRP_MAX + tq2 % (2 * CSSM_GRP_MAX)) * CSSM_SLOT_STRIDE] = 0ull;
   }
-  if (threadIdx.x < 2 * CSSM_MAXSLOTS)
+  if (threadIdx.x < 2 * CSSM_MAXSLOTS && (!far_only || threadIdx.x >= CSSM_MAXSLOTS))
     sc->maxslot[((size_t)((slot_set + 1 + (int)(threadIdx.x / CSSM_MAXSLOTS)) % CSSM_MAXSETS) * CSSM_MAXSLOTS + threadIdx.x % CSSM_MAXSLOTS) * CSSM_SLOT_STRIDE] = 0ull;
 }
 
@@ -193,7 +195,9 @@
                                                           uint32_t slot_lo, uint32_t slot_hi, uint32_t all5_stride,
                                                           cssm_u128* __restrict__ s2buf = nullptr, uint32_t s2_stride = 0, int s2_par_arg = -1,
                                                           uint32_t gen = 0, const cssm_u128* __restrict__ unit_pre = nullptr, const uint32_t blk0 = 0u,
-                                                          const double* pre_in = nullptr, const SpecTotals* tt = nullptr, Mid* mid = nullptr) {
+                                                          const double* pre_in = nullptr, const SpecTotals* tt = nullptr, Mid* mid = nullptr,
+                                                          const unsigned long long* __restrict__ ulimb = nullptr, uint32_t* s_range = nullptr,
+                                                          const bool far_only = false, unsigned long long* __restrict__ ulimb_clear = nullptr) {
   const uint32_t bidx = blockIdx.x - blk0, nblk = gridDim.x - blk0;
   constexpr bool GRP = GRPL != 0;
   constexpr bool BIG = GRPL == 2;
@@ -249,7 +253,9 @@
         upre[0].lo = g[0]; upre[0].hi = g[(size_t)CSSM_GRP_MAX * CSSM_SLOT_STRIDE];
       } else {
         const uint32_t q = (grp_unit / CSSM_GRP_UNITS) * CSSM_GRP_UNITS + (l - (uint32_t)CSSM_GRP_SMALL);
-        if (q < nunits) {
+        if (q < nunits && ulimb != nullptr) {
+          upre[0].lo = ulimb[2 * (size_t)q]; upre[0].hi = ulimb[2 * (size_t)q + 1];
+        } else if (q < nunits) {
           upre[0] = unitP[(size_t)q * (uint32_t)split];
           if (!SELF) for (uint32_t sb = 1; sb < (uint32_t)split; ++sb) upre[0] = cssm_u128_add(upre[0], unitP[(size_t)q * (uint32_t)split + sb]);
         }
@@ -404,10 +410,11 @@
         static_assert(CSSM_GRP_SMALL == 32 && CSSM_GRP_UNITS == 32, "one wave holds the groups and one group's units");
         if (wid == wsum) {
           cssm_u128 v = upre[0];
-          if (lane < 32u) {
+          if (lane < 32u || ulimb != nullptr) {
+            const int L = (ulimb != nullptr) ? CSSM_STEP_LIMB : CSSM_GRP_LIMB;
             cssm_u128 x, y;
             x.lo = upre[0].lo; x.hi = 0ull;
-            y.lo = upre[0].hi << CSSM_GRP_LIMB; y.hi = upre[0].hi >> (64 - CSSM_GRP_LIMB);
+            y.lo = upre[0].hi << L; y.hi = upre[0].hi >> (64 - L);
             v = cssm_u128_add(x, y);
           }
           const cssm_u128 inc = wave_scan_u128(v, lane);
@@ -491,7 +498,8 @@
       if (!level_known()) return;
       cssm_u128 ptot2 = cssm_u128_zero();
       if (p_pend) ptot2 = block_sum_u128(pt2, s_r[2]);
-      publish_observation(sc, rec, gmax_dec, gmax, tot, tot2, p_pend != 0u, ptot2, s2_par, nunits, rec_idx, gen, ll_t, ess_t, n_global, slot_set);
+      publish_observation(sc, rec, gmax_dec, gmax, tot, tot2, p_pend != 0u, ptot2, s2_par, nunits, rec_idx, gen, ll_t, ess_t, n_global, slot_set,
+                          far_only, ulimb_clear, 2u * nunits);
       CSSM_STAMP(7);
       return;
     }
@@ -616,6 +624,10 @@
         if (CLIP) { wb = (wb < slot_lo) ? slot_lo : wb; we = (we > slot_hi) ? slot_hi : we; }
         we = (we > (uint32_t)n_global) ? (uint32_t)n_global : we;
         wb = (wb > we) ? we : wb;
+        if (s_range != nullptr) {
+          if (wid == 0 && lane == 0) s_range[0] = wb;
+          if (wid == CSSM_BLOCK / 64 - 1 && lane == 0) s_range[1] = we;
+        }
         fill_runs_wave<CSSM_OFF_SC1 != 0, CLIP>(prev, e, (uint32_t)i0, wb, we, anc, CLIP ? slot_lo : 0u, (uint32_t)(n - 1),
                                                 s_slot + wid * CSSM_WAVE_CHUNK);
       }
diff --git a/composablestatespacemodels_amd/csrc/cssm_pf.hip b/composablestatespacemodels_amd/csrc/cssm_pf.hip
--- a/composablestatespacemodels_amd/csrc/cssm_pf.hip
+++ b/composablestatespacemodels_amd/csrc/cssm_pf.hip
@@ -171,7 +171,7 @@
   (void)hipSetDevice(pf->device);
   if (pf->stream) (void)hipStreamSynchronize(pf->stream);
   cssm_peer_free(pf);
-  void* ptrs[] = {pf->sm_keys, pf->sm_partial, pf->sm_st, pf->sm_rec, pf->s2buf, pf->fineS, pf->fineS2, pf->state[0], pf->state[1], pf->logw, pf->endslot, pf->anc, pf->tileS, pf->tileS2, pf->tileP, pf->unitPre, pf->tileW, pf->sc,
+  void* ptrs[] = {pf->sm_keys, pf->sm_partial, pf->sm_st, pf->sm_rec, pf->s2buf, pf->fineS, pf->fineS2, pf->state[0], pf->state[1], pf->logw, pf->endslot, pf->anc, pf->tileS, pf->tileS2, pf->tileP, pf->unitPre, pf->tileW, pf->sc, pf->logw2, pf->ulimb,
                   pf->d_m0, pf->d_sd0, pf->d_logtab, pf->d_fsub, pf->cum, pf->d_recs, pf->d_ll_t, pf->d_ess_t, pf->d_path, pf->cand, pf->cand_end, pf->cand_idx, pf->d_bounds, pf->d_xch, pf->d_need};
   for (void* p : ptrs) if (p) (void)hipFree(p);
   if (pf->h_recs) (void)hipHostFree(pf->h_recs);
@@ -222,7 +222,7 @@
 static void fresh_host_state(cssm_pf* pf, double t0) {
   pf->cur = 0; pf->src = pf->state[0]; pf->src_stride = pf->stride; pf->src2 = nullptr; pf->anc_valid = false;
   pf->t = t0; pf->step = 0; pf->initialised = true; pf->wparity = 0;
-  pf->wmode = false; pf->sums_ready = false; pf->last_optimistic = false; pf->last_grp = false; pf->have_level = false;
+  pf->wmode = false; pf->sums_ready = false; pf->last_optimistic = false; pf->last_grp = false; pf->have_level = false; pf->sums_limb = false;
   pf->ess_host = (int32_t)(pf->n_global < 2147483647ull ? pf->n_global : 2147483647ull);
 }
 
@@ -384,7 +384,18 @@
   HIP_TRY(hipGetLastError());
   pf->cur ^= 1;
   pf->src = pf->state[pf->cur]; pf->src_stride = pf->stride; pf->anc_valid = false; pf->src2 = nullptr;
-  return CSSM_OK;
+  pf->sums_limb = false;
+  return CSSM_OK;
+}
+
+static void fill_step_resample(const cssm_pf* pf, StepLaunch& a, const StepRec* d_rec, double* ll_t, int32_t* ess_t, uint32_t rec_idx) {
+  const size_t us = 2 * (size_t)pf->nunits;
+  a.stream = pf->stream;
+  a.logw_in = pf->logw; a.n = pf->n; a.sc = pf->sc; a.unitP = pf->tileS;
+  a.ulimb_in = pf->sums_limb ? pf->ulimb + (size_t)pf->wparity * us : nullptr;
+  a.rec_t = d_rec; a.anc = pf->anc; a.ntiles = pf->ntiles; a.nunits = pf->nunits; a.set_t = pf->wparity;
+  a.ll_t = ll_t; a.ess_t = ess_t; a.rec_idx = rec_idx; a.force_exact = pf->opt_exact; a.seed = pf->seed;
+  a.s2buf = pf->s2buf; a.s2_stride = pf->s2_stride; a.s2_par = pf->s2_par; a.gen = pf->gen;
 }
 
 static int launch_resample(cssm_pf* pf, const StepRec* d_rec, double* ll_t = nullptr, int32_t* ess_t = nullptr, uint32_t rec_idx = 0, bool allow_grp = true) {
@@ -429,6 +440,11 @@
                         else if (lean_layout == 1 && RS == CSSM_RESAMPLE_SYSTEMATIC) \
                           hipLaunchKernelGGL((k_offspring_self<CSSM_RESAMPLE_SYSTEMATIC, 0, 1>), dim3(ogrid), dim3(CSSM_BLOCK), 0, pf->stream, OFF_ARGS); \
                         else hipLaunchKernelGGL((k_offspring_self<RS, 0>), dim3(ogrid), dim3(CSSM_BLOCK), 0, pf->stream, OFF_ARGS); } while (0)
+  if (optimistic && pf->sums_limb) {
+    StepLaunch a;
+    fill_step_resample(pf, a, d_rec, ll_t, ess_t, rec_idx);
+    cssm_offspring_limb_launch(a);
+  } else
   if (pf->resampler == CSSM_RESAMPLE_STRATIFIED) OFF_GO(CSSM_RESAMPLE_STRATIFIED);
   else if (pf->resampler == CSSM_RESAMPLE_MULTINOMIAL) OFF_GO(CSSM_RESAMPLE_MULTINOMIAL);
   else OFF_GO(CSSM_RESAMPLE_SYSTEMATIC);
@@ -447,6 +463,41 @@
   if (optimistic) pf->s2_par ^= 1;
   return CSSM_OK;
 }
+static bool one_launch_ok(const cssm_pf* pf) {
+  return pf->opt_one != 0 && !pf->sharded && pf->first == 0 && pf->n == pf->n_global && pf->resampler == CSSM_RESAMPLE_SYSTEMATIC &&
+         uses_sums_kernel(pf) && pf->obs_kind != CSSM_OBS_LGCP && pf->opt_spec == 1 && pf->opt_grp != 0 && pf->sup == 1u && pf->split == 1u &&
+         pf->nunits >= pf->grp_min_units && pf->nunits <= (uint32_t)(CSSM_GRP_SMALL * CSSM_GRP_UNITS) && large_geometry(pf) == GEO_LOOP &&
+         cssm_step_parents_has(pf->mk, pf->d, pf->obs_kind);
+}
+static bool one_launch_after_propagate(const cssm_pf* pf) {
+  return pf->last_optimistic && pf->last_grp && pf->grp_layout == 1 && !pf->last_ws;
+}
+static int launch_step_parents(cssm_pf* pf, const StepRec* rec_t, uint32_t idx_t, const StepRec* rec_n, double* ll_t, int32_t* ess_t) {
+  const size_t us = 2 * (size_t)pf->nunits;
+  if (!pf->logw2) {
+    if (hipMalloc(&pf->logw2, pf->stride * 8) != hipSuccess) return fail(CSSM_ENOMEM, "hipMalloc of the second weight buffer");
+    if (hipMalloc(&pf->ulimb, CSSM_MAXSETS * us * 8) != hipSuccess) return fail(CSSM_ENOMEM, "hipMalloc of the units' limb sums");
+  }
+  if (!pf->sums_limb) HIP_TRY(hipMemsetAsync(pf->ulimb, 0, CSSM_MAXSETS * us * 8, pf->stream));
+  StepLaunch a;
+  fill_step_resample(pf, a, rec_t, ll_t, ess_t, idx_t);
+  a.set_n = (pf->wparity + 1) % CSSM_MAXSETS;
+  a.src = pf->src; a.stride = pf->stride; a.dst = pf->state[pf->cur ^ 1]; a.logw_out = pf->logw2; a.rec_n = rec_n; a.mk = pf->mk; a.logtab = pf->d_logtab;
+  a.ulimb_out = pf->ulimb + (size_t)a.set_n * us;
+  a.ulimb_far = pf->ulimb + (size_t)((a.set_n + 1) % CSSM_MAXSETS) * us;
+  prof_begin(pf, CSSM_K_PROPAGATE);
+  const bool ok = cssm_step_parents_launch(a, pf->d, pf->obs_kind);
+  prof_end(pf);
+  if (!ok) return fail(CSSM_ESTATE, "no one-launch kernel for this model structure");
+  HIP_TRY(hipGetLastError());
+  pf->wparity = a.set_n; pf->wmode = true; pf->have_level = true; pf->s2_par ^= 1;
+  pf->last_optimistic = true; pf->last_grp = true; pf->grp_layout = 1; pf->last_ws = false;
+  pf->cur ^= 1; pf->src = pf->state[pf->cur]; pf->src_stride = pf->stride; pf->anc_valid = false; pf->src2 = nullptr;
+  std::swap(pf->logw, pf->logw2);
+  pf->sums_limb = true;
+  return CSSM_OK;
+}
+
 static int launch_step(cssm_pf* pf, const StepRec* d_rec, int weighted, uint32_t step_index, double* ll_t = nullptr, int32_t* ess_t = nullptr,
                        uint32_t rec_idx = 0, double* pick_out = nullptr, uint32_t pick_slot = 0) {
   pf->h_step_for_resample = step_index;
@@ -711,16 +762,30 @@
   if (pf->opt_events) HIP_TRY(hipEventRecord(pf->ev0, pf->stream));
   bool folded = false;
   size_t s_from = 0;
+  bool pending = false; size_t pend_s = 0;
+  auto flush = [&]() -> int {
+    if (!pending) return CSSM_OK;
+    pending = false;
+    return launch_resample(pf, pf->d_recs + pend_s, pf->d_ll_t, pf->d_ess_t, (uint32_t)pend_s);
+  };
   for (;;) {
     const bool may_hold = may_use_sums_kernel(pf);
+    const bool defer = path == nullptr && one_launch_ok(pf);
     for (size_t s = s_from; s < T; ++s) {
       const int weighted = pf->h_recs[s].has_obs;
       double* pick_out = (folded && s >= 1) ? pf->d_path + s * (size_t)d : nullptr;
       const uint32_t pick_slot = s >= 1 ? pf->h_recs[s - 1].pick : 0u;
       pf->h_step_for_resample = base + (uint32_t)s;
-      rc = cssm_launch_propagate(pf, pf->d_recs + s, pick_out, pick_slot);
+      if (pending && weighted) {
+        pending = false;
+        rc = launch_step_parents(pf, pf->d_recs + pend_s, (uint32_t)pend_s, pf->d_recs + s, pf->d_ll_t, pf->d_ess_t);
+      } else {
+        rc = flush();
+        if (!rc) rc = cssm_launch_propagate(pf, pf->d_recs + s, pick_out, pick_slot);
+      }
       if (!rc) {
-        if (weighted) rc = launch_resample(pf, pf->d_recs + s, pf->d_ll_t, pf->d_ess_t, (uint32_t)s);
+        if (weighted && defer && one_launch_after_propagate(pf)) { pending = true; pend_s = s; }
+        else if (weighted) rc = launch_resample(pf, pf->d_recs + s, pf->d_ll_t, pf->d_ess_t, (uint32_t)s);
         else hipLaunchKernelGGL(k_record, dim3(1), dim3(1), 0, pf->stream, pf->sc, pf->d_ll_t, pf->d_ess_t, (uint32_t)s);
       }
       if (rc) return rc;
@@ -731,6 +796,8 @@
                            (const uint32_t*)(pf->anc_valid ? pf->anc : nullptr), (uint64_t)pf->h_recs[s].pick, d,
                            pf->d_path + (s + 1) * (size_t)d);
     }
+    rc = flush();
+    if (rc) return rc;
     ph_enq = since(tp0);
     if (pf->opt_events) HIP_TRY(hipEventRecord(pf->ev1, pf->stream));
     HIP_TRY(hipGetLastError());
@@ -930,6 +997,12 @@
   if (option == CSSM_OPT_GROUP_SUMS) { pf->opt_grp = value ? 1 : 0; return CSSM_OK; }
   if (option == CSSM_OPT_WAVE_SUMS) { pf->opt_wave = value == 2 ? 2 : (value ? 1 : 0); return CSSM_OK; }
   if (option == CSSM_OPT_LOOP_EVENTS) { pf->opt_events = value ? 1 : 0; return CSSM_OK; }
+  if (option == CSSM_OPT_ONE_LAUNCH) {
+    if (value < 0 || value > 2) return fail(CSSM_EINVAL_ARG, "CSSM_OPT_ONE_LAUNCH takes 0, 1 or 2");
+    pf->opt_one = value;
+    if (value == 2 && !pf->sharded) { pf->opt_whole = 1; pf->split = 1u; }
+    return CSSM_OK;
+  }
   if (option == CSSM_OPT_FORECAST_CAP) {
     if (value < 0) return fail(CSSM_EINVAL_ARG, "the forecast key-buffer cap is a number of KiB >= 0");
     pf->forecast_cap = (size_t)value * 1024;
diff --git a/composablestatespacemodels_amd/csrc/cssm_propagate.hip.h b/composablestatespacemodels_amd/csrc/cssm_propagate.hip.h
--- a/composablestatespacemodels_amd/csrc/cssm_propagate.hip.h
+++ b/composablestatespacemodels_amd/csrc/cssm_propagate.hip.h
@@ -42,7 +42,8 @@
   bool bad;
 };
 
-template <int D, bool LGCP, int IT, int OBS, int SUMS, int ONE = 0, bool WR = false>
+struct NoTileEnd { __device__ __forceinline__ void operator()(uint32_t, cssm_u128&) const {} };
+template <int D, bool LGCP, int IT, int OBS, int SUMS, int ONE = 0, bool WR = false, bool LOWER = false, class TileEnd = NoTileEnd>
 __device__ __forceinline__ void propagate_range(
     const double* __restrict__ src, size_t src_stride, const uint32_t* __restrict__ anc,
     double* __restrict__ dst, size_t dst_stride, double* __restrict__ logw, uint64_t gid0,
@@ -51,7 +52,8 @@
     const uint32_t range_lo, const uint32_t n, int do_sums_arg,
     double* __restrict__ pick_out, uint32_t pick_slot, unsigned char* s_stage, PropAcc& acc,
     const double* __restrict__ fsub = nullptr, const unsigned long long* pre_jp = nullptr, const cssm_u32x4* pre_blk = nullptr,
-    const uint32_t step_now = 0u, const bool wr_on = false) {
+    const uint32_t step_now = 0u, const bool wr_on = false, const uint32_t range_first = 0u, const uint32_t tl_arg = 0u,
+    TileEnd* tile_end = nullptr) {
   const uint32_t step = (pre_blk != nullptr) ? step_now : rec->step;
   const int has_obs = rec->has_obs;
   const double dt = rec->dt;
@@ -65,7 +67,9 @@
   static_assert(!WR || ONE == 2, "wave ranges: the tile-after-tile instantiation");
   const bool wr = WR && wr_on;
   const uint32_t stride = (wr ? 64u : (uint32_t)CSSM_BLOCK) * IT;
-  const uint32_t tl = wr ? (threadIdx.x & 63u) : threadIdx.x;
+  const uint32_t tl = LOWER ? tl_arg : (wr ? (threadIdx.x & 63u) : threadIdx.x);
+  static_assert(!LOWER || (IT == 2 && ONE == 2 && !WR && SUMS == 1), "LOWER: the tile-after-tile pairs kernel with the fused sums");
+  auto above = [&](uint32_t i) { return !LOWER || i >= range_first; };
   constexpr bool STAGE = true;
   constexpr int ES = (IT * D <= 8) ? 16 : 8;
   constexpr int WAVE_STAGE = IT * D * 64 * ES;
@@ -80,6 +84,9 @@
         const ulonglong2 a = *reinterpret_cast<const ulonglong2*>(anc + i0);
         jp[0] = a.x; jp[NJ - 1] = a.y;
       } else if (IT == 2) {
+        if constexpr (LOWER) {
+          jp[0] = (i0 < n) ? __hip_atomic_load(reinterpret_cast<const unsigned long long*>(anc + i0), __ATOMIC_RELAXED, __HIP_MEMORY_SCOPE_AGENT) : 0ull;
+        } else
         jp[0] = *reinterpret_cast<const unsigned long long*>(anc + i0);
       } else {
         jp[0] = anc[i0];
@@ -94,7 +101,7 @@
 #pragma unroll
     for (int r = 0; r < IT; ++r) {
       const uint32_t v = (uint32_t)(jp[r / 2] >> (32 * (r & 1)));
-      j[r] = (i0 + r < n) ? v : n_last;
+      j[r] = (i0 + r < n && above(i0 + r)) ? v : n_last;
     }
   };
   auto ptr_of = [&](uint32_t j, int k) -> const double* {
@@ -206,7 +213,7 @@
   }
   for (; base < n; base += stride) {
     const uint32_t i0 = base + tl * IT;
-    const bool full = (i0 + IT <= n);
+    const bool full = (i0 + IT <= n) && above(i0);
     if (ONE == 2 && base + stride < n) load_idx(base + stride, jp);
     if (SUMS && pick_out != nullptr) {
 #pragma unroll
@@ -218,7 +225,7 @@
     }
     double lw[IT];
     auto account = [&](int r) {
-      if (weighted && i0 + r < n) {
+      if (weighted && i0 + r < n && above(i0 + r)) {
         if (lw[r] != lw[r]) { bad = true; lw[r] = -cssm_inf(); }
         tmax = (lw[r] > tmax) ? lw[r] : tmax;
         if (SUMS && do_sums) {
@@ -318,13 +325,14 @@
     } else {
 #pragma unroll
       for (int r = 0; r < IT; ++r) {
-        if (i0 + r < n) {
+        if (i0 + r < n && above(i0 + r)) {
 #pragma unroll
           for (int k = 0; k < D; ++k) dst[(size_t)k * dst_stride + i0 + r] = x[r][k];
           if (weighted && logw) logw[i0 + r] = lw[r];
         }
       }
     }
+    if constexpr (LOWER) (*tile_end)(i0, accS);
     if (ONE && base == range_lo) PSTAMP(4);
     if (ONE == 1) break;
     if (ONE == 2) {
diff --git a/composablestatespacemodels_amd/csrc/cssm_step.hip b/composablestatespacemodels_amd/csrc/cssm_step.hip
--- /dev/null
+++ b/composablestatespacemodels_amd/csrc/cssm_step.hip
@@ -0,0 +1,22 @@
+#include "cssm_host.h"
+#include "cssm_step_parents.hip.h"
+
+static constexpr uint32_t kStepW3 = 0x001A0636u;
+
+bool cssm_step_parents_has(const ModelK& mk, int d, int obs_kind) {
+  return d == 3 && mk.d == 3 && obs_kind == CSSM_OBS_POISSON && mk.comp[0] == kStepW3 && mk.comp[1] == 0u && mk.comp[2] == 0u;
+}
+
+bool cssm_step_parents_launch(const StepLaunch& a, int d, int obs_kind) {
+  if (!cssm_step_parents_has(a.mk, d, obs_kind)) return false;
+  static_assert(PropItems<3>::value == 2, "k_step_parents: one pair per thread");
+  k_step_parents<3, 2, CSSM_OBS_POISSON, kStepW3, 0u, 0u><<<dim3(a.nunits + 1u), dim3(CSSM_BLOCK), 0, a.stream>>>(
+      a.logw_in, a.n, a.sc, a.unitP, a.ulimb_in, a.rec_t, a.anc, a.ntiles, a.nunits, a.set_t, a.ll_t, a.ess_t, a.rec_idx, a.force_exact, a.seed,
+      a.s2buf, a.s2_stride, a.s2_par, a.gen, a.src, a.stride, a.dst, a.logw_out, a.rec_n, a.mk, a.logtab, a.ulimb_out, a.ulimb_far, a.set_n);
+  return true;
+}
+
+void cssm_offspring_limb_launch(const StepLaunch& a) {
+  k_offspring_limb<<<dim3(a.nunits + 1u), dim3(CSSM_BLOCK), 0, a.stream>>>(a.logw_in, a.n, a.sc, a.ulimb_in, a.rec_t, a.anc, a.ntiles, a.nunits, a.set_t,
+                                                                            a.ll_t, a.ess_t, a.rec_idx, a.force_exact, a.seed, a.s2buf, a.s2_stride, a.s2_par, a.gen);
+}
diff --git a/composablestatespacemodels_amd/csrc/cssm_step_parents.hip.h b/composablestatespacemodels_amd/csrc/cssm_step_parents.hip.h
--- /dev/null
+++ b/composablestatespacemodels_amd/csrc/cssm_step_parents.hip.h
@@ -0,0 +1,90 @@
+#pragma once
+
+#include "cssm_offspring.hip.h"
+#include "cssm_propagate.hip.h"
+
+#define CSSM_STEP_USLOTS 8
+
+__device__ __forceinline__ void step_sums_add(Scalars* __restrict__ sc, unsigned long long* __restrict__ ulimb, int set, uint32_t unit,
+                                              unsigned long long lo, unsigned long long hi) {
+  atomicAdd(&ulimb[2 * (size_t)unit], lo);
+  atomicAdd(&ulimb[2 * (size_t)unit + 1], hi);
+  unsigned long long* g = &sc->grp[((size_t)set * 2 * CSSM_GRP_MAX + unit / CSSM_GRP_UNITS) * CSSM_SLOT_STRIDE];
+  atomicAdd(g, lo);
+  atomicAdd(g + (size_t)CSSM_GRP_MAX * CSSM_SLOT_STRIDE, hi);
+}
+
+struct StepTileEnd {
+  unsigned long long* s_acc;
+  unsigned long long* ulimb; Scalars* sc; int set; uint32_t unit0, nunits;
+  __device__ __forceinline__ void operator()(uint32_t i0, cssm_u128& acc) const {
+    const cssm_u128 s = wave_sum_u128(acc);
+    acc = cssm_u128_zero();
+    const uint32_t unit = (uint32_t)__builtin_amdgcn_readfirstlane((int)i0) / (uint32_t)CSSM_TILE;
+    if ((threadIdx.x & 63u) == 0u && (s.lo | s.hi) != 0ull && unit < nunits) {
+      const unsigned long long lo = s.lo & ((1ull << CSSM_STEP_LIMB) - 1ull);
+      const unsigned long long hi = (s.lo >> CSSM_STEP_LIMB) | (s.hi << (64 - CSSM_STEP_LIMB));
+      const uint32_t k = unit - unit0;
+      if (k < (uint32_t)CSSM_STEP_USLOTS) { atomicAdd(&s_acc[2 * k], lo); atomicAdd(&s_acc[2 * k + 1], hi); }
+      else step_sums_add(sc, ulimb, set, unit, lo, hi);
+    }
+  }
+};
+
+template <int D, int IT, int OBS, uint32_t MKW, uint32_t MKW1, uint32_t MKW2>
+__global__ __launch_bounds__(CSSM_BLOCK, 4) void k_step_parents(
+    const double* __restrict__ logw_in, uint64_t n, Scalars* __restrict__ sc, const cssm_u128* __restrict__ unitP,
+    const unsigned long long* __restrict__ ulimb_in, const StepRec* __restrict__ rec_t, uint32_t* __restrict__ anc, uint32_t ntiles,
+    uint32_t nunits, int set_t, double* __restrict__ ll_t, int32_t* __restrict__ ess_t, uint32_t rec_idx, int force_exact, uint64_t seed,
+    cssm_u128* __restrict__ s2buf, uint32_t s2_stride, int s2_par, uint32_t gen,
+    const double* __restrict__ src, size_t stride, double* __restrict__ dst, double* __restrict__ logw_out, const StepRec* __restrict__ rec_n,
+    ModelK mk, const double* __restrict__ logtab, unsigned long long* __restrict__ ulimb_out, unsigned long long* __restrict__ ulimb_far,
+    int set_n) {
+  static_assert(IT == 2 && CSSM_BLOCK == 256, "pairs; three table entries per thread");
+  mk.comp[0] = MKW; mk.comp[1] = MKW1; mk.comp[2] = MKW2;
+  __shared__ uint32_t s_range[2];
+  __shared__ unsigned long long s_acc[2 * CSSM_STEP_USLOTS];
+  __shared__ double s_max[CSSM_BLOCK / 64];
+  const double tv = logtab[threadIdx.x], tv1 = logtab[256 + threadIdx.x], tv2 = logtab[512 + threadIdx.x];
+  if (threadIdx.x < 2u) s_range[threadIdx.x] = 0u;
+  if (threadIdx.x < 2u * CSSM_STEP_USLOTS) s_acc[threadIdx.x] = 0ull;
+  const double* tab = stage_log_table_finish(tv, tv1, tv2);
+  offspring_body<true, true, CSSM_RESAMPLE_SYSTEMATIC, 2, 1>(logw_in, n, sc, unitP, nullptr, rec_t, n, nullptr, anc, ntiles, 1u, nunits, 2, set_t, ll_t, ess_t,
+                                                             rec_idx, force_exact, nullptr, 0, 1, 1, seed, nullptr, nullptr, 1, nullptr, 0u, (uint32_t)n, 5u,
+                                                             s2buf, s2_stride, s2_par, gen, nullptr, 0u, nullptr, nullptr, (NoMid*)nullptr,
+                                                             ulimb_in, s_range, true, ulimb_far);
+  asm volatile("s_waitcnt vmcnt(0)" ::: "memory");
+  __syncthreads();
+  const uint32_t c0 = (uint32_t)__builtin_amdgcn_readfirstlane((int)s_range[0]), c1 = (uint32_t)__builtin_amdgcn_readfirstlane((int)s_range[1]);
+  if (c1 <= c0) return;
+  __shared__ __attribute__((aligned(16))) unsigned char s_stage[PropStage<D, IT>::bytes];
+  const uint32_t lo = c0 & ~(64u * IT - 1u);
+  const uint32_t tl = ((((threadIdx.x >> 6) + blockIdx.x) & (CSSM_BLOCK / 64 - 1u)) << 6) | (threadIdx.x & 63u);
+  StepTileEnd te{s_acc, ulimb_out, sc, set_n, lo / (uint32_t)CSSM_TILE, nunits};
+  PropAcc acc;
+  propagate_range<D, false, IT, OBS, 1, 2, false, true, StepTileEnd>(src, stride, anc, dst, stride, logw_out, 0ull, seed, rec_n, mk, nullptr, 0, 0u, tab,
+                                                                     lo, c1, 1, nullptr, 0u, s_stage, acc, nullptr, nullptr, nullptr, 0u, false, c0, tl, &te);
+  const double tmax = wave_max(acc.tmax);
+  if ((threadIdx.x & 63u) == 0u) s_max[threadIdx.x >> 6] = tmax;
+  if (__any(acc.bad) && (threadIdx.x & 63u) == 0u) atomicOr(&sc->err, 1u);
+  __syncthreads();
+  if (threadIdx.x < (uint32_t)CSSM_STEP_USLOTS) {
+    const unsigned long long a0 = s_acc[2 * threadIdx.x], a1 = s_acc[2 * threadIdx.x + 1];
+    if ((a0 | a1) != 0ull) step_sums_add(sc, ulimb_out, set_n, te.unit0 + threadIdx.x, a0, a1);
+  }
+  if (threadIdx.x == 0) {
+    double m = s_max[0];
+#pragma unroll
+    for (int w = 1; w < CSSM_BLOCK / 64; ++w) m = (s_max[w] > m) ? s_max[w] : m;
+    atomicMax(&sc->maxslot[((size_t)set_n * CSSM_MAXSLOTS + blockIdx.x % CSSM_MAXSLOTS) * CSSM_SLOT_STRIDE], (unsigned long long)cssm_order_key(m));
+  }
+}
+
+__global__ __attribute__((amdgpu_flat_work_group_size(CSSM_BLOCK, CSSM_BLOCK), amdgpu_waves_per_eu(CSSM_OFF_SELF_WAVES, 8))) void k_offspring_limb(
+    const double* __restrict__ logw, uint64_t n, Scalars* __restrict__ sc, const unsigned long long* __restrict__ ulimb, const StepRec* __restrict__ rec,
+    uint32_t* __restrict__ anc, uint32_t ntiles, uint32_t nunits, int slot_set, double* __restrict__ ll_t, int32_t* __restrict__ ess_t, uint32_t rec_idx,
+    int force_exact, uint64_t seed, cssm_u128* __restrict__ s2buf, uint32_t s2_stride, int s2_par, uint32_t gen) {
+  offspring_body<true, true, CSSM_RESAMPLE_SYSTEMATIC, 2, 1>(logw, n, sc, nullptr, nullptr, rec, n, nullptr, anc, ntiles, 1u, nunits, 2, slot_set, ll_t, ess_t, rec_idx,
+                                                             force_exact, nullptr, 0, 1, 1, seed, nullptr, nullptr, 1, nullptr, 0u, (uint32_t)n, 5u,
+                                                             s2buf, s2_stride, s2_par, gen, nullptr, 0u, nullptr, nullptr, (NoMid*)nullptr, ulimb);
+}
diff --git a/include/cssm_pf.h b/include/cssm_pf.h
--- a/include/cssm_pf.h
+++ b/include/cssm_pf.h
@@ -119,6 +119,7 @@
 #define CSSM_OPT_LOOP_EVENTS 9
 #define CSSM_OPT_WAVE_SUMS 10
 #define CSSM_OPT_FORECAST_CAP 11
+#define CSSM_OPT_ONE_LAUNCH 12
 int cssm_pf_set_option(cssm_pf* pf, int option, int value);
 int cssm_rtc_info(uint64_t* out4);
 
```

Result: slower. 44.32 billion (-14.3%).
